# ccalantzis/BRDF

Hardware: AMD Instinct MI355X
Metric: BRDF residual-evals/sec (1 M samples, Ward 3-param), whole job; rel-err vs CPU levmar in `parity` (higher is better)
Workload: dtype f64

## Files before the change

brdf_amd/_lib.py:

```python
from __future__ import annotations

import ctypes as C
import os

_HERE = os.path.dirname(os.path.abspath(__file__))
LIB_PATH = os.environ.get("BRDF_HIP_LIB") or os.path.join(_HERE, "libbrdf_hip.so")

D = C.POINTER(C.c_double)
F = C.POINTER(C.c_float)
I = C.POINTER(C.c_int)
MODEL_FUNC = C.CFUNCTYPE(None, D, D, C.c_int, C.c_int, C.c_void_p)


class ExtraData(C.Structure):
    _fields_ = [("angles", D), ("modelInfo", C.c_int)]


ABI = {
    "dlevmar_dif": (C.c_int, [C.c_void_p, D, D, C.c_int, C.c_int, C.c_int, D, D, D, D, C.c_void_p]),
    "dlevmar_bc_dif": (C.c_int, [C.c_void_p, D, D, C.c_int, C.c_int, D, D, D, C.c_int, D, D, D, D, C.c_void_p]),
    "dlevmar_der": (C.c_int, [C.c_void_p, C.c_void_p, D, D, C.c_int, C.c_int, C.c_int, D, D, D, D, C.c_void_p]),
    "dlevmar_bc_der": (C.c_int, [C.c_void_p, C.c_void_p, D, D, C.c_int, C.c_int, D, D, D, C.c_int, D, D, D, D, C.c_void_p]),
    "dlevmar_stddev": (C.c_double, [D, C.c_int, C.c_int]),
    "dlevmar_corcoef": (C.c_double, [D, C.c_int, C.c_int, C.c_int]),
    "dlevmar_R2": (C.c_double, [C.c_void_p, D, D, C.c_int, C.c_int, C.c_void_p]),
    "dAx_eq_b_LU_noLapack": (C.c_int, [D, D, D, C.c_int]),
    "slevmar_dif": (C.c_int, [C.c_void_p, F, F, C.c_int, C.c_int, C.c_int, F, F, F, F, C.c_void_p]),
    "slevmar_bc_dif": (C.c_int, [C.c_void_p, F, F, C.c_int, C.c_int, F, F, F, C.c_int, F, F, F, F, C.c_void_p]),
    "slevmar_der": (C.c_int, [C.c_void_p, C.c_void_p, F, F, C.c_int, C.c_int, C.c_int, F, F, F, F, C.c_void_p]),
    "slevmar_bc_der": (C.c_int, [C.c_void_p, C.c_void_p, F, F, C.c_int, C.c_int, F, F, F, C.c_int, F, F, F, F, C.c_void_p]),
    "slevmar_chkjac": (None, [C.c_void_p, C.c_void_p, F, C.c_int, C.c_int, C.c_void_p, F]),
    "slevmar_stddev": (C.c_float, [F, C.c_int, C.c_int]),
    "slevmar_corcoef": (C.c_float, [F, C.c_int, C.c_int, C.c_int]),
    "slevmar_R2": (C.c_float, [C.c_void_p, F, F, C.c_int, C.c_int, C.c_void_p]),
    "sAx_eq_b_LU_noLapack": (C.c_int, [F, F, F, C.c_int]),
    "brdf_hip_register_model": (C.c_int, [C.c_void_p]),
    "brdf_hip_unregister_model": (C.c_int, [C.c_void_p]),
    "BRDFFunc_hip": (None, [D, D, C.c_int, C.c_int, C.c_void_p]),
    "BRDFJac_hip": (None, [D, D, C.c_int, C.c_int, C.c_void_p]),
    "dlevmar_chkjac": (None, [C.c_void_p, C.c_void_p, D, C.c_int, C.c_int, C.c_void_p, D]),
    "brdf_hip_fit_dev": (C.c_int, [C.c_int, C.c_int, C.c_void_p, C.c_void_p, C.c_int, D, D, D, D, C.c_int, D, D, D,
                                   C.c_void_p]),
    "brdf_hip_fit_channels_dev": (C.c_int, [C.c_int, C.c_int, C.c_void_p, C.c_void_p, C.c_longlong, C.c_int, C.c_int, D, D, D, D, C.c_int, D,
                                            D, D, C.c_void_p]),
    "brdf_hip_last_channels_stamps": (C.c_int, [C.c_int, C.POINTER(C.c_longlong)]),
    "brdf_hip_last_channels_stats": (C.c_int, [C.c_int, C.POINTER(C.c_int), C.POINTER(C.c_longlong), C.POINTER(C.c_longlong), D]),
    "brdf_hip_fit_batch_dev": (C.c_int, [C.c_int, C.c_int, C.c_void_p, C.c_void_p, C.c_int, C.c_int, C.c_void_p, D, D,
                                         C.c_int, D, C.c_void_p, C.c_void_p, C.c_void_p]),
    "brdf_hip_fit_batch": (C.c_int, [C.c_int, C.c_int, D, D, C.c_int, C.c_int, D, D, D, C.c_int, D, D, I]),
    "brdf_hip_fit_batch_multi": (C.c_int, [C.c_int, C.c_int, D, D, C.c_int, C.c_int, D, D, D, C.c_int, D, D, I, I, C.c_int]),
    "brdf_hip_last_multi_stats": (C.c_int, [C.c_int, I, C.POINTER(C.c_longlong), C.POINTER(C.c_longlong), D]),
    "brdf_hip_fit_stats_batch_dev": (C.c_int, [C.c_int, C.c_int, C.c_void_p, C.c_void_p, C.c_int, C.c_int, C.c_void_p, D, C.c_void_p,
                                               C.c_void_p, C.c_void_p, C.c_void_p]),
    "brdf_hip_fit_stats_batch": (C.c_int, [C.c_int, C.c_int, D, D, C.c_int, C.c_int, D, D, D, D, I]),
    "brdf_hip_model_eval_dev": (C.c_int, [C.c_int, C.c_void_p, C.c_int, D, C.c_void_p, C.c_void_p]),
    "brdf_hip_synth_dev": (C.c_int, [C.c_int, C.c_ulonglong, C.c_longlong, C.c_int, C.c_int, C.c_void_p, C.c_void_p,
                                     C.c_void_p, C.c_void_p]),
    "brdf_hip_cosines_dev": (C.c_int, [C.c_void_p, C.c_void_p, C.c_void_p, C.c_void_p, C.c_longlong, D, C.c_int, D, C.c_int,
                                       C.c_void_p, C.c_void_p]),
    "brdf_hip_led_table": (None, [D]),
    "brdf_hip_fit_capture_dev": (C.c_int, [C.c_int, C.c_void_p, C.c_int, C.c_int, C.c_int, C.c_void_p, C.c_void_p, C.c_void_p,
                                           C.c_void_p, C.c_int, D, D, C.c_int, D, D, D, C.c_int, D, C.c_void_p, D,
                                           C.POINTER(C.c_longlong), C.c_void_p]),
    "brdf_hip_fit_capture_stats_dev": (C.c_int, [C.c_int, C.c_void_p, C.c_int, C.c_int, C.c_int, C.c_void_p, C.c_void_p, C.c_void_p,
                                                 C.c_void_p, C.c_int, D, D, C.c_int, D, D, D, C.c_int, D, C.c_void_p, D,
                                                 C.POINTER(C.c_longlong), C.c_void_p, C.c_void_p, C.c_void_p, C.c_void_p]),
    "brdf_hip_fit_capture_single_dev": (C.c_int, [C.c_int, C.c_void_p, C.c_int, C.c_int, C.c_int, C.c_void_p, C.c_void_p, C.c_void_p,
                                                  C.c_void_p, C.c_int, D, D, C.c_int, D, D, D, C.c_int, D, D, D,
                                                  C.POINTER(C.c_longlong), C.c_void_p]),
    "brdf_hip_device_count": (C.c_int, []),
    "brdf_hip_last_error": (C.c_char_p, []),
    "brdf_hip_last_fit_launches": (C.c_longlong, []),
    "brdf_hip_set_launch_timing": (None, [C.c_int]),
    "brdf_hip_last_fit_kernel_us": (C.c_double, []),
    "brdf_hip_last_channels_kernel_us": (C.c_double, []),
    "brdf_hip_last_fit_stamps": (C.c_int, [C.POINTER(C.c_longlong)]),
    "brdf_hip_last_fit_trace": (C.c_int, [C.POINTER(C.c_longlong), C.c_int]),
    "brdf_hip_last_fit_stats": (C.c_int, [C.POINTER(C.c_longlong), C.POINTER(C.c_longlong), C.POINTER(C.c_longlong),
                                          D]),
}


def load() -> C.CDLL:
    try:
        import torch
    except ImportError:
        pass
    if not os.path.exists(LIB_PATH):
        raise ImportError(
            f"{LIB_PATH} not found: build it with `python -c 'import __graft_entry__ as g; g.build()'` "
            "(or `make -C brdf_amd/csrc`). brdf_amd has no fallback path without its HIP library.")
    lib = C.CDLL(LIB_PATH, mode=C.RTLD_LOCAL)
    for name, (res, args) in ABI.items():
        try:
            fn = getattr(lib, name)
        except AttributeError as exc:
            raise ImportError(f"{LIB_PATH} does not export `{name}` declared in include/brdf_levmar.h") from exc
        fn.restype = res
        fn.argtypes = args
    return lib


lib = load()


def last_error() -> str:
    return (lib.brdf_hip_last_error() or b"").decode()
```

brdf_amd/csrc/capi.hip:

```cpp
#include <algorithm>
#include <cmath>
#include <cstdio>
#include <cstring>
#include <mutex>

#include <cfloat>
#include <vector>

#include "../../include/brdf_levmar.h"
#include "batch_fit.h"
#include "fit_host.h"
#include "fit_stats.h"

namespace brdf {
int generic_fit_run(int method, void (*func)(double *, double *, int, int, void *),
                    void (*jacf)(double *, double *, int, int, void *), double *p, double *x, int m, int n, double *lb,
                    double *ub, double *dscl, int itmax, double *opts, double *info, double *covar, void *adata);
int model_eval_run(int model, const double *d_angles, int n, const double *p, double *d_hx, hipStream_t stream);
int model_jac_run(int model, const double *d_angles, int n, const double *p, double *d_jac, hipStream_t stream);
int chkjac_err_run(const double *fvec, const double *fjac, const double *fvecp, const double *p, int m, int n, double *err);
int r2_run(const double *x, const double *hx, int n, double *r2);
int generic_fit_run_f(int method, void (*func)(float *, float *, int, int, void *), void (*jacf)(float *, float *, int, int, void *),
                      float *p, float *x, int m, int n, float *lb, float *ub, float *dscl, int itmax, float *opts, float *info,
                      float *covar, void *adata);
// ... 382 lines not shown

void BRDFFunc_hip(double *p, double *hx, int m, int n, void *adata) {
  const brdf_extra_data *ed = static_cast<const brdf_extra_data *>(adata);
  if (!p || !hx || !ed || !ed->angles || m != kM || n <= 0) {
    set_error("BRDFFunc_hip(): bad arguments");
    return;
  }
  if (ed->modelInfo < 0 || ed->modelInfo >= MODEL_COUNT) return;
  double *stage = g_stage.get(4 * (size_t)n);
  if (!stage) return;
  double *d_out = stage + 3 * (size_t)n;
  hipError_t e = upload_planes(stage, ed->angles, n, ed->modelInfo);
  if (e != hipSuccess) {
    set_error("BRDFFunc_hip(): host->device copy failed: %s", hipGetErrorString(e));
    return;
  }
  if (model_eval_run(ed->modelInfo, stage, n, p, d_out, nullptr) != 0) return;
  e = hipMemcpy(hx, d_out, sizeof(double) * n, hipMemcpyDeviceToHost);
  if (e != hipSuccess) set_error("BRDFFunc_hip(): device->host copy failed: %s", hipGetErrorString(e));
}

void BRDFJac_hip(double *p, double *jac, int m, int n, void *adata) {
  const brdf_extra_data *ed = static_cast<const brdf_extra_data *>(adata);
  if (!p || !jac || !ed || !ed->angles || m != kM || n <= 0) {
    set_error("BRDFJac_hip(): bad arguments");
    return;
  }
  if (ed->modelInfo < 0 || ed->modelInfo >= MODEL_COUNT) return;
  double *stage = g_stage.get(6 * (size_t)n);
  if (!stage) return;
  double *d_out = stage + 3 * (size_t)n;
  hipError_t e = upload_planes(stage, ed->angles, n, ed->modelInfo);
  if (e != hipSuccess) {
    set_error("BRDFJac_hip(): host->device copy failed: %s", hipGetErrorString(e));
    return;
  }
  if (model_jac_run(ed->modelInfo, stage, n, p, d_out, nullptr) != 0) return;
  e = hipMemcpy(jac, d_out, sizeof(double) * 3 * n, hipMemcpyDeviceToHost);
  if (e != hipSuccess) set_error("BRDFJac_hip(): device->host copy failed: %s", hipGetErrorString(e));
}

void dlevmar_chkjac(void (*func)(double *, double *, int, int, void *), void (*jacf)(double *, double *, int, int, void *),
                    double *p, int m, int n, void *adata, double *err) {
  if (!func || !jacf || !p || !err || m <= 0 || n <= 0) {
    set_error("dlevmar_chkjac(): bad arguments");
    return;
  }
  std::vector<double> fvec(n), fjac((size_t)n * m), pp(m), fvecp(n);
  const double eps = sqrt(DBL_EPSILON);
  (*func)(p, fvec.data(), m, n, adata);
  (*jacf)(p, fjac.data(), m, n, adata);
  for (int j = 0; j < m; ++j) {
    double temp = eps * fabs(p[j]);
    if (temp == 0.0) temp = eps;
    pp[j] = p[j] + temp;
  }
  (*func)(pp.data(), fvecp.data(), m, n, adata);
  (void)chkjac_err_run(fvec.data(), fjac.data(), fvecp.data(), p, m, n, err);
}

int brdf_hip_fit_dev(int method, int model, const double *d_angles, const double *d_x, int n, double *p,
                     const double *lb, const double *ub, const double *dscl, int itmax, const double *opts,
                     double *info, double *covar, void *stream) {
  StreamFitArgs a;
  a.method = (method == BRDF_METHOD_BC_DER) ? 1 : (method == BRDF_METHOD_DER ? 2 : method);
  a.analytic = (method == BRDF_METHOD_BC_DER || method == BRDF_METHOD_DER) ? 1 : 0;
  a.model = model;
  a.d_angles = d_angles;
  a.d_x = d_x;
  a.n = n;
  a.p = p;
  a.lb = lb;
  a.ub = ub;
  a.dscl = dscl;
  a.itmax = itmax;
  a.opts = opts;
  a.info = info;
  a.covar = covar;
  a.stream = static_cast<hipStream_t>(stream);
  return stream_fit_run(a);
}

int brdf_hip_fit_channels_dev(int method, int model, const double *d_angles, const double *d_x, long long x_stride, int n, int channels,
                              double *p, const double *lb, const double *ub, const double *dscl, int itmax, const double *opts,
                              double *info, double *covar, void *stream) {
  if (!d_angles || !d_x || !p || n <= 0 || channels < 1 || channels > 16 || (channels > 1 && x_stride < n)) {
    set_error("brdf_hip_fit_channels_dev(): bad arguments");
    return LM_ERROR;
  }
  if (method < 0 || method > 3 || model < 0 || model >= MODEL_COUNT) {
    set_error("brdf_hip_fit_channels_dev(): unknown method %d or model %d", method, model);
    return LM_ERROR;
  }
  return channels_fit_run(method, model, d_angles, d_x, x_stride, n, channels, p, lb, ub, dscl, itmax, opts, info, covar,
                          static_cast<hipStream_t>(stream));
}

int brdf_hip_last_channels_stamps(int channel, long long *out8) {
  const FitStats st = channels_last_stats(channel);
  for (int i = 0; i < 8; ++i) out8[i] = st.stamps[i];
  return 0;
}

int brdf_hip_last_channels_stats(int channel, int *shared_launch, long long *passes, long long *jac_passes, double *device_us) {
  const FitStats st = channels_last_stats(channel);
  if (shared_launch) *shared_launch = channels_last_shared();
  if (passes) *passes = st.passes;
  if (jac_passes) *jac_passes = st.jac_passes;
  if (device_us) *device_us = st.device_us;
  return 0;
}

int brdf_hip_fit_batch_dev(int method, int model, const double *d_angles, const double *d_x, int S, int n,
                           double *d_p, const double *lb, const double *ub, int itmax, const double *opts,
                           double *d_info, int *d_ret, void *stream) {
  BatchFitArgs a;
  a.method = method;
  a.model = model;
  a.d_angles = d_angles;
  a.d_x = d_x;
  a.S = S;
  a.n = n;
  a.d_p = d_p;
  a.lb = lb;
  a.ub = ub;
  a.itmax = itmax;
  a.opts = opts;
  a.d_info = d_info;
  a.d_ret = d_ret;
  a.stream = static_cast<hipStream_t>(stream);
  return batch_fit_enqueue(a);
}

int brdf_hip_fit_batch(int method, int model, const double *angles, const double *x, int S, int n, double *p,
                       const double *lb, const double *ub, int itmax, const double *opts, double *info, int *ret) {
  if (!angles || !x || !p || S <= 0 || n <= 0) {
    set_error("brdf_hip_fit_batch(): bad arguments");
    return LM_ERROR;
  }
  const size_t sn = (size_t)S * n;
  DevBuf d_angles, d_x, d_p, d_info, d_ret;
  if (d_angles.alloc(3 * sn) || d_x.alloc(sn) || d_p.alloc(3 * (size_t)S) || d_info.alloc(10 * (size_t)S) ||
      d_ret.alloc(((size_t)S + 1) / 2 + 1))
    return LM_ERROR;
  hipError_t e = hipMemcpy(d_angles.ptr, angles, sizeof(double) * 3 * sn, hipMemcpyHostToDevice);
  if (e == hipSuccess) e = hipMemcpy(d_x.ptr, x, sizeof(double) * sn, hipMemcpyHostToDevice);
  if (e == hipSuccess) e = hipMemcpy(d_p.ptr, p, sizeof(double) * 3 * S, hipMemcpyHostToDevice);
  if (e != hipSuccess) {
    set_error("brdf_hip_fit_batch(): host->device copy failed: %s", hipGetErrorString(e));
    return LM_ERROR;
  }
  int *d_ret_i = reinterpret_cast<int *>(d_ret.ptr);
  if (brdf_hip_fit_batch_dev(method, model, d_angles.ptr, d_x.ptr, S, n, d_p.ptr, lb, ub, itmax, opts, d_info.ptr,
                             d_ret_i, nullptr) != 0)
    return LM_ERROR;
  e = hipDeviceSynchronize();
  if (e == hipSuccess) e = hipMemcpy(p, d_p.ptr, sizeof(double) * 3 * S, hipMemcpyDeviceToHost);
  if (e == hipSuccess && info) e = hipMemcpy(info, d_info.ptr, sizeof(double) * 10 * S, hipMemcpyDeviceToHost);
  int *host_ret = ret;
  int *tmp = nullptr;
  if (!host_ret) host_ret = tmp = new int[S];
  if (e == hipSuccess) e = hipMemcpy(host_ret, d_ret_i, sizeof(int) * S, hipMemcpyDeviceToHost);
  int bad = 0;
  if (e == hipSuccess)
    for (int s = 0; s < S; ++s) bad += host_ret[s] < 0;
  delete[] tmp;
  if (e != hipSuccess) {
    set_error("brdf_hip_fit_batch(): %s", hipGetErrorString(e));
    return LM_ERROR;
  }
  return bad;
}

int brdf_hip_fit_stats_batch_dev(int method, int model, const double *d_angles, const double *d_x, int S, int n,
                                 const double *d_p, const double *opts, double *d_covar, double *d_stats, int *d_rank,
                                 void *stream) {
  FitStatsArgs a;
  a.method = method;
  a.model = model;
  a.d_angles = d_angles;
  a.d_x = d_x;
  a.S = S;
  a.n = n;
  a.d_p = d_p;
  a.opts = opts;
  a.d_covar = d_covar;
  a.d_stats = d_stats;
  a.d_rank = d_rank;
  a.stream = static_cast<hipStream_t>(stream);
  return fit_stats_enqueue(a, "brdf_hip_fit_stats_batch_dev");
}

int brdf_hip_fit_stats_batch(int method, int model, const double *angles, const double *x, int S, int n, const double *p,
                             const double *opts, double *covar, double *stats, int *rank) {
  static const char *who = "brdf_hip_fit_stats_batch";
  FitStatsArgs a;
  a.method = method;
  a.model = model;
  a.d_angles = angles;
  a.d_x = x;
  a.S = S;
  a.n = n;
  a.d_p = p;
  a.opts = opts;
  a.d_covar = covar;
  a.d_stats = stats;
  a.d_rank = rank;
  if (fit_stats_check(a, who) != 0) return LM_ERROR;
  const size_t sn = (size_t)S * n;
  DevBuf d_angles, d_x, d_p, d_covar, d_stats, d_rank;
  if (d_angles.alloc(3 * sn) || d_x.alloc(sn) || d_p.alloc(3 * (size_t)S) || (covar && d_covar.alloc(9 * (size_t)S)) ||
      (stats && d_stats.alloc(BRDF_STATS_SZ * (size_t)S)) || (rank && d_rank.alloc(((size_t)S + 1) / 2 + 1)))
    return LM_ERROR;
  hipError_t e = hipMemcpy(d_angles.ptr, angles, sizeof(double) * 3 * sn, hipMemcpyHostToDevice);
  if (e == hipSuccess) e = hipMemcpy(d_x.ptr, x, sizeof(double) * sn, hipMemcpyHostToDevice);
  if (e == hipSuccess) e = hipMemcpy(d_p.ptr, p, sizeof(double) * 3 * S, hipMemcpyHostToDevice);
  if (e != hipSuccess) {
    set_error("%s(): host->device copy failed: %s", who, hipGetErrorString(e));
    return LM_ERROR;
  }
  a.d_angles = d_angles.ptr;
  a.d_x = d_x.ptr;
  a.d_p = d_p.ptr;
  a.d_covar = d_covar.ptr;
  a.d_stats = d_stats.ptr;
  a.d_rank = reinterpret_cast<int *>(d_rank.ptr);
  if (fit_stats_enqueue(a, who) != 0) return LM_ERROR;
  e = hipStreamSynchronize(nullptr);
  if (e == hipSuccess && covar) e = hipMemcpy(covar, d_covar.ptr, sizeof(double) * 9 * S, hipMemcpyDeviceToHost);
  if (e == hipSuccess && stats) e = hipMemcpy(stats, d_stats.ptr, sizeof(double) * BRDF_STATS_SZ * S, hipMemcpyDeviceToHost);
  if (e == hipSuccess && rank) e = hipMemcpy(rank, d_rank.ptr, sizeof(int) * S, hipMemcpyDeviceToHost);
  if (e != hipSuccess) {
    set_error("%s(): %s", who, hipGetErrorString(e));
    return LM_ERROR;
  }
  return 0;
}

int brdf_hip_model_eval_dev(int model, const double *d_angles, int n, const double *p, double *d_hx, void *stream) {
  return model_eval_run(model, d_angles, n, p, d_hx, static_cast<hipStream_t>(stream));
}

int brdf_hip_synth_dev(int model, unsigned long long seed, long long first, int count, int n,
                       const double *d_truth, double *d_angles, double *d_x, void *stream) {
  return synth_enqueue(model, seed, first, count, n, d_truth, d_angles, d_x, static_cast<hipStream_t>(stream));
}

int brdf_hip_cosines_dev(const double *d_vertices, const int *d_faces, const double *d_face_normals, const int *d_surfels,
                         long long S, const double *leds, int L, const double *view_origin, int rv_mode, double *d_angles,
                         void *stream) {
  return cosines_run(d_vertices, d_faces, d_face_normals, d_surfels, S, leds, L, view_origin, rv_mode, d_angles,
                     static_cast<hipStream_t>(stream));
}

void brdf_hip_led_table(double *leds16x3) { led_table(leds16x3); }

int brdf_hip_fit_capture_dev(int model, const unsigned char *d_images, int L, int H, int W, const int *d_pixel_map,
                             const double *d_vertices, const int *d_faces, const double *d_face_normals, int nf,
                             const double *leds, const double *view_origin, int rv_mode, const double *p0, const double *lb,
                             const double *ub, int itmax, const double *opts, double *d_brdf_surfaces, double *avg,
                             long long *n_pixels, void *stream) {
  return capture_fit_run(model, d_images, L, H, W, d_pixel_map, d_vertices, d_faces, d_face_normals, nf, leds, view_origin,
                         rv_mode, p0, lb, ub, itmax, opts, d_brdf_surfaces, avg, n_pixels, static_cast<hipStream_t>(stream));
}

int brdf_hip_fit_capture_stats_dev(int model, const unsigned char *d_images, int L, int H, int W, const int *d_pixel_map,
                                   const double *d_vertices, const int *d_faces, const double *d_face_normals, int nf,
                                   const double *leds, const double *view_origin, int rv_mode, const double *p0,
                                   const double *lb, const double *ub, int itmax, const double *opts, double *d_brdf_surfaces,
                                   double *avg, long long *n_pixels, void *stream, double *d_surface_covar,
                                   double *d_surface_stats, int *d_surface_rank) {
  return capture_fit_run(model, d_images, L, H, W, d_pixel_map, d_vertices, d_faces, d_face_normals, nf, leds, view_origin,
                         rv_mode, p0, lb, ub, itmax, opts, d_brdf_surfaces, avg, n_pixels, static_cast<hipStream_t>(stream),
                         d_surface_covar, d_surface_stats, d_surface_rank);
}

int brdf_hip_fit_capture_single_dev(int model, const unsigned char *d_images, int L, int H, int W, const int *d_pixel_map,
                                    const double *d_vertices, const int *d_faces, const double *d_face_normals, int nf,
                                    const double *leds, const double *view_origin, int rv_mode, const double *p0,
                                    const double *lb, const double *ub, int itmax, const double *opts, double *single_brdf,
                                    double *info, long long *n_faces_used, void *stream) {
  return capture_fit_single_run(model, d_images, L, H, W, d_pixel_map, d_vertices, d_faces, d_face_normals, nf, leds, view_origin,
                                rv_mode, p0, lb, ub, itmax, opts, single_brdf, info, n_faces_used, static_cast<hipStream_t>(stream));
}

int brdf_hip_device_count(void) {
  int c = 0;
  if (hipGetDeviceCount(&c) != hipSuccess) return 0;
  return c;
}

const char *brdf_hip_last_error(void) { return get_error(); }

int brdf_hip_last_fit_stats(long long *passes, long long *jac_passes, long long *eval_passes, double *device_us) {
  const FitStats s = stream_fit_last_stats();
  if (passes) *passes = s.passes;
  if (jac_passes) *jac_passes = s.jac_passes;
  if (eval_passes) *eval_passes = s.eval_passes;
  if (device_us) *device_us = s.device_us;
  return 0;
}

long long brdf_hip_last_fit_launches(void) { return stream_fit_last_stats().launches; }

void brdf_hip_set_launch_timing(int on) { set_launch_timing(on != 0); }
double brdf_hip_last_fit_kernel_us(void) { return stream_fit_last_stats().kernel_us; }
double brdf_hip_last_channels_kernel_us(void) { return channels_last_shared() ? channels_last_stats(0).kernel_us : -1.0; }

int brdf_hip_last_fit_trace(long long *out, int max_rows) { return resident_fit_last_trace(out, max_rows); }

int brdf_hip_last_fit_stamps(long long *out8) {
  const FitStats s = stream_fit_last_stats();
  for (int k = 0; k < 8; ++k) out8[k] = s.stamps[k];
  return 0;
}

}
```

brdf_amd/csrc/fit_host.hip:

```cpp
#include <algorithm>
#include <cstdio>
#include <cstdlib>

#include "fit_host.h"

namespace brdf {

void set_bad_input_error(const char *who, int bad_input, int n, int m) {
  switch (bad_input) {
  case 1: set_error("%s(): cannot solve a problem with fewer measurements [%d] than unknowns [%d]", who, n, m); break;
  case 2: set_error("%s(): at least one lower bound exceeds the upper one", who); break;
  default: set_error("%s(): scaling constants should be positive", who); break;
  }
}

void warn_start_projected(int i, double from, double to) {
  fprintf(stderr, "Warning: component %d of starting point not feasible in dlevmar_bc_dif()! [%g projected to %g]\n", i, from, to);
}

int start_fit_machine(MachineUnion &m, int method, const double *p, int n, const double *lb, const double *ub, const double *dscl, int itmax,
                      const double *opts, bool want_covar, bool analytic, bool fast) {
  if (method == 0) {
    m.dif.start(p, n, itmax, opts, want_covar, 1, dif_chain_candidates());
    if (m.dif.h.req.kind != RQ_DONE) return 0;
    set_bad_input_error("dlevmar_dif", 1, n, kM);
    return kLmError;
  }
  if (method == 2) {
    m.der.start(p, n, itmax, opts, want_covar);
    if (m.der.h.req.kind != RQ_DONE) return 0;
    set_bad_input_error("dlevmar_der", 1, n, kM);
    return kLmError;
  }
  BcMachine<kM> &bc = m.bc;
  bc.start(p, n, lb, ub, dscl, itmax, opts, want_covar, pg_candidates(), bc_spec_jac_enabled() ? 1 : 0);
  bc.c.analytic_jac = analytic ? 1 : 0;
  if (bc.h.req.kind == RQ_DONE) {
    set_bad_input_error("dlevmar_bc_dif", bc.c.bad_input, n, kM);
    return kLmError;
  }
  if (fast || !brdf_fast_path_enabled())
    for (int i = 0; i < kM; ++i)
      if (bc.c.infeasible_mask & (1 << i)) warn_start_projected(i, bc.c.p_start[i], bc.h.p[i]);
  return 0;
}

void mailbox_to_caller(const Mailbox &mb, double *p, double *info, double *covar, FitStats *stats) {
  for (int i = 0; i < kM; ++i) p[i] = mb.p[i];
  if (info)
    for (int i = 0; i < kInfoSz; ++i) info[i] = mb.info[i];
  if (covar)
    for (int i = 0; i < kM * kM; ++i) covar[i] = mb.covar[i];
  stats->passes = mb.passes;
  stats->jac_passes = mb.n_jac;
  stats->eval_passes = mb.n_eval;
  stats->device_us = (double)(mb.t_last - mb.t_first) / 100.0;
  for (int k = 0; k < 8; ++k) stats->stamps[k] = mb.stamps[k];
}

ExchangeKnobs exchange_knobs(int max_replicas, long long default_spin_ticks) {
  ExchangeKnobs k{max_replicas, default_spin_ticks, -1};
  if (const char *e = getenv("BRDF_HIP_RESIDENT_REPLICAS")) k.replicas = std::min(max_replicas, std::max(1, atoi(e)));
  if (const char *e = getenv("BRDF_HIP_RESIDENT_SPIN_MS")) k.spin_ticks = std::max(1LL, atoll(e)) * 100000LL;
  if (const char *e = getenv("BRDF_HIP_RESIDENT_SABOTAGE")) k.sabotage_epoch = atoi(e);
  return k;
}

bool kernel_fits_a_cu(const void *kernel, int threads, std::atomic<int> &cached) {
  int v = cached.load(std::memory_order_relaxed);
  if (v == 0) {
    int per_cu = 0;
    if (hipOccupancyMaxActiveBlocksPerMultiprocessor(&per_cu, kernel, threads, 0) != hipSuccess) per_cu = 0;
    v = per_cu + 1;
    cached.store(v, std::memory_order_relaxed);
  }
  return v > 1;
}

void ResidentWorkspace::release() {
  if (d_block || h_mbox) {
    int cur = -1;
    (void)hipGetDevice(&cur);
    if (device >= 0 && cur != device) (void)hipSetDevice(device);
    (void)hipDeviceSynchronize();
    if (d_block) (void)hipFree(d_block);
    if (h_mbox) (void)hipHostFree(h_mbox);
    if (cur >= 0 && cur != device) (void)hipSetDevice(cur);
  }
  d_block = nullptr;
  h_mbox = d_mbox = nullptr;
  device = -1;
}

int ResidentWorkspace::allocate(size_t bytes, int mailboxes) {
  hipDeviceProp_t prop;
  HIP_OK(hipGetDeviceProperties(&prop, device));
  cus = prop.multiProcessorCount;
  HIP_OK(hipMalloc(&d_block, bytes));
  HIP_OK(hipMemset(d_block, 0, bytes));
  HIP_OK(hipHostMalloc(&h_mbox, sizeof(Mailbox) * (size_t)mailboxes, hipHostMallocMapped | hipHostMallocCoherent));
  HIP_OK(hipHostGetDevicePointer((void **)&d_mbox, h_mbox, 0));
  block_bytes = bytes;
  n_mbox = mailboxes;
  return 0;
}

int ResidentWorkspace::ensure(int dev, size_t bytes, int mailboxes) {
  if (ready(dev)) return 0;
  release();
  device = dev;
  const int r = allocate(bytes, mailboxes);
  if (r != 0) release();
  return r;
}

int ResidentWorkspace::zero_tables(hipStream_t stream) {
  HIP_OK(hipMemsetAsync(d_block, 0, block_bytes, stream));
  return 0;
}

void ResidentWorkspace::launch_unavailable() {
  backoff = std::min(1024, std::max(8, backoff * 2));
  skip = backoff;
  if (const char *e = getenv("BRDF_HIP_RESIDENT_BACKOFF")) skip = std::max(0, atoi(e));
}

int ResidentWorkspace::wait_for_mailboxes(int K, hipStream_t stream, bool *done) {
  auto all_done = [&] {
    for (int k = 0; k < K; ++k)
      if (!*(volatile int *)&h_mbox[k].done) return false;
    return true;
  };
  for (unsigned spins = 0; !all_done(); ++spins)
    if ((spins & 0x3FFu) == 0x3FFu && hipStreamQuery(stream) != hipErrorNotReady) break;
  __atomic_thread_fence(__ATOMIC_ACQUIRE);
  if (!all_done()) {
    HIP_OK(hipStreamSynchronize(stream));
    __atomic_thread_fence(__ATOMIC_ACQUIRE);
  }
  *done = all_done();
  return 0;
}

}
```

brdf_amd/csrc/lm_machine.h:

```cpp
#pragma once

#include <float.h>
#include <math.h>

#if defined(__HIPCC__)
#define LM_HD __host__ __device__ __forceinline__
#else
#define LM_HD inline
#endif

namespace brdf {

constexpr double kEpsilon = 1E-12;
constexpr double kOneThird = 0.3333333334;
constexpr int kLsItMax = 150;
constexpr double kLsPow = 2.1;
constexpr double kInitMu = 1E-03;
#ifndef LM_STAMP
#define LM_STAMP(i) do {} while (0)
#endif

#ifndef LM_PHASE_ENTER
#define LM_PHASE_ENTER(X) true
#endif
#define LM_PHASE(X) if ((ONE_LANE ? lm_uniform(ph) : ph) == X && LM_PHASE_ENTER(X)) do
#define LM_PHASE_END while (0);
#define LM_GATE(X)                                    \
  if (GATED && !heavy && ph == X) {                   \
    req.kind = RQ_YIELD;                              \
    { h.phase = ph; return; }                         \
  }

constexpr double kStopThresh = 1E-17;
constexpr double kDiffDelta = 1E-06;
constexpr int kInfoSz = 10;
constexpr int kLmError = -1;

enum ReqKind : int {
  RQ_DONE = 0,
  RQ_EVAL = 1,
  RQ_SCALED = 2,
  RQ_JAC = 3,
  RQ_DIF_INIT = 4,
  RQ_DIF_JAC = 5,
  RQ_DIF_TRIAL = 6,
  RQ_DIF_UPDATE = 7,
  RQ_EVAL_MULTI = 8,
  RQ_YIELD = 9
};

constexpr int kMaxCand = 8;

template <class Real>
struct LmLimits;
template <>
struct LmLimits<double> {
  static LM_HD double eps() { return DBL_EPSILON; }
  static LM_HD double max() { return DBL_MAX; }
};
template <>
struct LmLimits<float> {
  static LM_HD float eps() { return FLT_EPSILON; }
  static LM_HD float max() { return FLT_MAX; }
};

template <int M, class Real = double>
struct Request {
  int kind;
  int central;
  int sel_hx;
  int sel_j;
  int aux;
  Real p[M];
  Real d[M];
  Real q[M];
  Real dp[M];
  Real dp_l2;
  Real scal;
  int nk;
  int pad_;
  Real pk[kMaxCand][M];
};

template <int M>
struct SumLayout {
  static constexpr int NL = M * (M + 1) / 2;
  static constexpr int JAC = NL + M + 1;
  static constexpr int DIF_JAC = NL + M;
  static constexpr int DIF_TRIAL = 1 + NL + 2 * M;
  static constexpr int MAX = DIF_TRIAL > JAC ? DIF_TRIAL : JAC;
};

LM_HD int lm_uniform(int v) {
#if defined(__HIP_DEVICE_COMPILE__)
  return __builtin_amdgcn_readfirstlane(v);
#else
  return v;
#endif
}

#if defined(__HIP_DEVICE_COMPILE__)
__device__ __forceinline__ double lm_read_lane(double v, int lane) {
  const int lo = __builtin_amdgcn_readlane(__double2loint(v), lane);
  const int hi = __builtin_amdgcn_readlane(__double2hiint(v), lane);
  return __hiloint2double(hi, lo);
}
__device__ __forceinline__ float lm_read_lane(float v, int lane) {
  return __int_as_float(__builtin_amdgcn_readlane(__float_as_int(v), lane));
}
#endif

template <class Real>
LM_HD Real lm_abs(Real v) { return (v >= Real(0.0)) ? v : -v; }
template <class Real>
LM_HD bool lm_finite(Real v) { return (v - v) == Real(0.0); }

template <int M, class Real>
LM_HD int lu_solve(const Real *A, const Real *B, Real *x) {
  constexpr int kUnrollLu = M <= 8 ? 64 : 1;
  Real a[M * M], scale[M];
  int perm[M];
#pragma unroll kUnrollLu
  for (int i = 0; i < M * M; ++i) a[i] = A[i];
#pragma unroll kUnrollLu
  for (int i = 0; i < M; ++i) x[i] = B[i];
#pragma unroll kUnrollLu
  for (int i = 0; i < M; ++i) {
    Real big = Real(0.0);
#pragma unroll kUnrollLu
    for (int j = 0; j < M; ++j) {
      const Real t = lm_abs(a[i * M + j]);
      if (t > big) big = t;
    }
    if (big == Real(0.0)) return 0;
    scale[i] = Real(1.0) / big;
  }
#pragma unroll kUnrollLu
  for (int j = 0; j < M; ++j) {
    int pivot = j;
    Real big = Real(0.0);
#pragma unroll kUnrollLu
    for (int i = 0; i < j; ++i) {
      Real s = a[i * M + j];
#pragma unroll kUnrollLu
      for (int k = 0; k < i; ++k) s -= a[i * M + k] * a[k * M + j];
      a[i * M + j] = s;
    }
#pragma unroll kUnrollLu
    for (int i = j; i < M; ++i) {
      Real s = a[i * M + j];
#pragma unroll kUnrollLu
      for (int k = 0; k < j; ++k) s -= a[i * M + k] * a[k * M + j];
      a[i * M + j] = s;
      const Real t = scale[i] * lm_abs(s);
      if (t >= big) {
        big = t;
        pivot = i;
      }
    }
#pragma unroll kUnrollLu
    for (int r = j + 1; r < M; ++r) {
      if (pivot == r) {
#pragma unroll kUnrollLu
        for (int k = 0; k < M; ++k) {
          const Real t = a[r * M + k];
          a[r * M + k] = a[j * M + k];
          a[j * M + k] = t;
        }
        scale[r] = scale[j];
      }
    }
    perm[j] = pivot;
    if (a[j * M + j] == Real(0.0)) a[j * M + j] = LmLimits<Real>::eps();
    if (j != M - 1) {
      const Real t = Real(1.0) / a[j * M + j];
#pragma unroll kUnrollLu
      for (int i = j + 1; i < M; ++i) a[i * M + j] *= t;
    }
  }
  int first = 0;
#pragma unroll kUnrollLu
  for (int i = 0; i < M; ++i) {
    Real s = x[i];
#pragma unroll kUnrollLu
    for (int r = i + 1; r < M; ++r) {
      if (perm[i] == r) {
        s = x[r];
        x[r] = x[i];
      }
    }
    if (first != 0) {
#pragma unroll kUnrollLu
      for (int jj = 0; jj < i; ++jj)
        if (jj >= first - 1) s -= a[i * M + jj] * x[jj];
    } else if (s != Real(0.0)) {
      first = i + 1;
    }
    x[i] = s;
  }
#pragma unroll kUnrollLu
  for (int i = M - 1; i >= 0; --i) {
    Real s = x[i];
#pragma unroll kUnrollLu
    for (int j = i + 1; j < M; ++j) s -= a[i * M + j] * x[j];
    x[i] = s / a[i * M + i];
  }
  return 1;
}

template <int M, class Real>
LM_HD int lu_covar(const Real *JtJ, Real *C, Real sumsq, int n) {
  for (int l = 0; l < M; ++l) {
    Real rhs[M], col[M];
    for (int i = 0; i < M; ++i) rhs[i] = (i == l) ? Real(1.0) : Real(0.0);
    if (!lu_solve<M>(JtJ, rhs, col)) return 0;
    for (int i = 0; i < M; ++i) C[i * M + l] = col[i];
  }
  const Real fact = sumsq / (Real)(n - M);
  for (int i = 0; i < M * M; ++i) C[i] *= fact;
  return M;
}

template <int M, class Real>
LM_HD void fd_steps(const Real *p, Real delta, Real *d) {
  for (int j = 0; j < M; ++j) {
    Real s = Real(1E-04) * p[j];
    s = lm_abs(s);
    if (s < delta) s = delta;
    d[j] = s;
  }
}

template <int M, class Real>
LM_HD void unpack_lower(const Real *s, Real *jtj) {
  int c = 0;
  for (int i = 0; i < M; ++i)
    for (int j = 0; j <= i; ++j, ++c) {
      jtj[i * M + j] = s[c];
      jtj[j * M + i] = s[c];
    }
}

template <class Real = double>
struct FitOptionsT {
  Real tau, eps1, eps2, eps2sq, eps3, delta;
  int forward;
};

template <class Real>
LM_HD FitOptionsT<Real> make_options(const Real *opts) {
  FitOptionsT<Real> o;
  if (opts) {
    o.tau = opts[0];
    o.eps1 = opts[1];
    o.eps2 = opts[2];
    o.eps2sq = opts[2] * opts[2];
    o.eps3 = opts[3];
    o.delta = opts[4];
  } else {
    o.tau = Real(kInitMu);
    o.eps1 = Real(kStopThresh);
    o.eps2 = Real(kStopThresh);
    o.eps2sq = Real(kStopThresh) * Real(kStopThresh);
    o.eps3 = Real(kStopThresh);
    o.delta = Real(kDiffDelta);
  }
  o.forward = 1;
  if (o.delta < Real(0.0)) {
    o.delta = -o.delta;
    o.forward = 0;
  }
  return o;
}

template <int M, class Real = double>
struct DifMachine {
  enum Phase : int { D_INIT_EVAL = 1, D_ITER_TOP, D_AFTER_JAC, D_GRADIENT, D_SOLVE, D_AFTER_TRIAL, D_AFTER_UPDATE, D_DECIDE, D_REJECT, D_AFTER_MULTI, D_FINISH, D_DONE };
  struct Cold {
    FitOptionsT<Real> o;
    int itmax, n, want_covar, refresh;
    int speculative;
    int multi;
    Real info[kInfoSz], covar[M * M];
    int ret;
  };
  struct CoreInts {
    int phase, k, stop, nu, nfev, njap, nlss, updjac, updp, newjac;
    int sel_hx, sel_j, accepted;
    int chain, single, mcnt;
  };
  struct CoreReals {
    Real p[M], mu, p_e2, jte_inf, p_l2, dp_l2, pdp_e2;
    Real jtj[M * M], jte[M], dp[M];
  };
  struct Core : CoreInts, CoreReals {};
  struct Cool {
    Real init_e2, diag[M], pdp[M];
    Real spec_jtj[M * M], spec_jte[M];
    Real ml2[kMaxCand];
  };
  struct Hot : Core {
    Cool cool;
    Request<M, Real> req;
  };
  static LM_HD void uniform_ints(CoreInts &h) {
    h.phase = lm_uniform(h.phase);
    h.k = lm_uniform(h.k);
    h.stop = lm_uniform(h.stop);
    h.nu = lm_uniform(h.nu);
    h.nfev = lm_uniform(h.nfev);
    h.njap = lm_uniform(h.njap);
    h.nlss = lm_uniform(h.nlss);
    h.updjac = lm_uniform(h.updjac);
    h.updp = lm_uniform(h.updp);
    h.newjac = lm_uniform(h.newjac);
    h.sel_hx = lm_uniform(h.sel_hx);
    h.sel_j = lm_uniform(h.sel_j);
    h.accepted = lm_uniform(h.accepted);
    h.chain = lm_uniform(h.chain);
    h.single = lm_uniform(h.single);
    h.mcnt = lm_uniform(h.mcnt);
  }
  Cold c;
  Hot h;

  LM_HD void start(const Real *p0, int n_, int itmax_, const Real *opts, int want_covar_, int speculative_ = 1, int multi_ = 1) {
    Request<M, Real> &req = h.req;
    Cool &cool = h.cool;
    c.o = make_options(opts);
    c.speculative = speculative_;
    c.multi = (multi_ < 1 || !speculative_) ? 1 : ((multi_ > kMaxCand) ? kMaxCand : multi_);
    h.chain = h.single = h.mcnt = 0;
    for (int j = 0; j < kMaxCand; ++j) cool.ml2[j] = Real(0.0);
    h.accepted = 0;
    c.itmax = itmax_;
    c.n = n_;
    c.want_covar = want_covar_;
    h.k = 0;
    h.stop = 0;
    h.nfev = h.njap = h.nlss = 0;
    h.updjac = 0;
    h.updp = 1;
    h.newjac = 0;
    c.refresh = (M >= 10) ? M : 10;
    h.sel_hx = h.sel_j = 0;
    h.mu = h.jte_inf = h.p_l2 = Real(0.0);
    h.p_e2 = cool.init_e2 = h.pdp_e2 = Real(0.0);
    h.dp_l2 = LmLimits<Real>::max();
    c.ret = kLmError;
    for (int i = 0; i < M; ++i) {
      h.p[i] = p0[i];
      h.jte[i] = cool.diag[i] = h.dp[i] = cool.pdp[i] = Real(0.0);
      cool.spec_jte[i] = Real(0.0);
    }
    for (int i = 0; i < M * M; ++i) h.jtj[i] = cool.spec_jtj[i] = c.covar[i] = Real(0.0);
    for (int i = 0; i < kInfoSz; ++i) c.info[i] = Real(0.0);
    clear_req(h, req);
    if (c.n < M) {
      h.phase = D_DONE;
      req.kind = RQ_DONE;
      return;
    }
    req.kind = RQ_DIF_INIT;
    for (int i = 0; i < M; ++i) req.p[i] = h.p[i];
    h.phase = D_INIT_EVAL;
  }

  static LM_HD void clear_req(const CoreInts &h, Request<M, Real> &req) {
    req.kind = RQ_DONE;
    req.central = 0;
    req.sel_hx = h.sel_hx;
    req.sel_j = h.sel_j;
    req.aux = 0;
    req.dp_l2 = Real(0.0);
    req.scal = Real(1.0);
    req.nk = 0;
    for (int i = 0; i < M; ++i) req.p[i] = req.d[i] = req.q[i] = req.dp[i] = Real(0.0);
  }

  static LM_HD void gradient_stats(CoreReals &h, Cool &cool) {
    h.p_l2 = h.jte_inf = Real(0.0);
    for (int i = 0; i < M; ++i) {
      const Real t = lm_abs(h.jte[i]);
      if (h.jte_inf < t) h.jte_inf = t;
      cool.diag[i] = h.jtj[i * M + i];
      h.p_l2 += h.p[i] * h.p[i];
    }
  }

  template <bool ONE_LANE = false, bool MULTI = false>
  LM_HD void step(const Real *s, Real maxabs) { run<ONE_LANE, MULTI>(c, h, h.cool, h.req, s, maxabs); }

  template <bool ONE_LANE, bool MULTI = false>
  static LM_HD void run(Cold &c, Core &h, Cool &cool, Request<M, Real> &req, const Real *s, Real maxabs) {
    run<ONE_LANE, MULTI>(c, static_cast<CoreInts &>(h), static_cast<CoreReals &>(h), cool, req, s, maxabs);
  }
  template <bool ONE_LANE, bool MULTI = false>
  static LM_HD void run(Cold &c, CoreInts &hi, CoreReals &h, Cool &cool, Request<M, Real> &req, const Real *s, Real ) {
    int ph = ONE_LANE ? lm_uniform(hi.phase) : hi.phase;
    LM_STAMP(0);
    for (;;) {
      if (ONE_LANE) ph = lm_uniform(ph);
      if (ph <= 0 || ph >= D_DONE) {
        req.kind = RQ_DONE;
        { hi.phase = ph; return; }
      }
      LM_PHASE(D_INIT_EVAL) {
        hi.nfev = 1;
        h.p_e2 = s[0];
        cool.init_e2 = h.p_e2;
        if (!lm_finite(h.p_e2)) hi.stop = 7;
        hi.nu = 20;
        ph = D_ITER_TOP;
        break;
      } LM_PHASE_END

      LM_PHASE(D_AFTER_JAC) {
        unpack_lower<M>(s, h.jtj);
        for (int i = 0; i < M; ++i) h.jte[i] = s[SumLayout<M>::NL + i];
        hi.newjac = 0;
        gradient_stats(h, cool);
        ph = D_SOLVE;
        break;
      } LM_PHASE_END

      LM_PHASE(D_AFTER_TRIAL) {
        h.pdp_e2 = s[0];
        if (!lm_finite(h.pdp_e2)) {
          hi.stop = 7;
          ph = D_FINISH;
          break;
        }
        const Real dF = h.p_e2 - h.pdp_e2;
        const bool updated = (hi.updp || dF > 0);
        if (MULTI) hi.chain = updated ? 0 : hi.chain + 1;
        Real dL = Real(0.0);
        for (int i = 0; i < M; ++i) dL += h.dp[i] * (h.mu * h.dp[i] + h.jte[i]);
        hi.accepted = (dL > Real(0.0) && dF > Real(0.0)) ? 1 : 0;
        if (hi.accepted) {
          Real t = (Real(2.0) * dF / dL - Real(1.0));
          t = Real(1.0) - t * t * t;
          h.mu = h.mu * ((t >= Real(kOneThird)) ? t : Real(kOneThird));
        }
        if (updated) {
          ++hi.updjac;
          hi.newjac = 1;
          if (c.speculative) {
            hi.sel_j ^= 1;
            unpack_lower<M>(s + 1, cool.spec_jtj);
            const Real *g = s + 1 + SumLayout<M>::NL + (hi.accepted ? 0 : M);
            for (int i = 0; i < M; ++i) cool.spec_jte[i] = g[i];
          } else {
            clear_req(hi, req);
            req.kind = RQ_DIF_UPDATE;
            req.aux = hi.accepted;
            for (int i = 0; i < M; ++i) {
              req.p[i] = h.p[i];
              req.q[i] = cool.pdp[i];
              req.dp[i] = h.dp[i];
            }
            req.dp_l2 = h.dp_l2;
            ph = D_AFTER_UPDATE;
            { hi.phase = ph; return; }
          }
        }
        LM_STAMP(1);
        ph = D_DECIDE;
        break;
      } LM_PHASE_END

      LM_PHASE(D_AFTER_UPDATE) {
        unpack_lower<M>(s, cool.spec_jtj);
        for (int i = 0; i < M; ++i) cool.spec_jte[i] = s[SumLayout<M>::NL + i];
        ph = D_DECIDE;
        break;
      } LM_PHASE_END

      if constexpr (MULTI)
      LM_PHASE(D_AFTER_MULTI) {
        const int cnt = hi.mcnt;
        int next = D_ITER_TOP;
        for (int j = 0; j < kMaxCand; ++j) {
          if (j >= cnt || !(hi.k < c.itmax)) break;
          const Real e2 = s[j];
          if (lm_finite(e2) && h.p_e2 - e2 > Real(0.0)) {
            hi.single = 1;
            break;
          }
          ++hi.nlss;
          ++hi.nfev;
          h.pdp_e2 = e2;
          h.dp_l2 = cool.ml2[j];
          if (!lm_finite(e2)) {
            hi.stop = 7;
            next = D_FINISH;
            break;
          }
          ++hi.chain;
          h.mu *= hi.nu;
          const int nu2 = (int)((unsigned)hi.nu << 1);
          if (nu2 <= hi.nu) {
            hi.stop = 5;
            next = D_FINISH;
            break;
          }
          hi.nu = nu2;
          ++hi.k;
        }
        ph = next;
        break;
      } LM_PHASE_END

      LM_PHASE(D_DECIDE) {
        if (hi.accepted) {
          hi.nu = 2;
          for (int i = 0; i < M; ++i) h.p[i] = cool.pdp[i];
          if (c.speculative) hi.sel_hx ^= 1;
          h.p_e2 = h.pdp_e2;
          hi.updp = 1;
          ++hi.k;
          ph = D_ITER_TOP;
          break;
        }
        ph = D_REJECT;
        break;
      } LM_PHASE_END

      LM_PHASE(D_REJECT) {
        h.mu *= hi.nu;
        const int nu2 = (int)((unsigned)hi.nu << 1);
        if (nu2 <= hi.nu) {
          hi.stop = 5;
          ph = D_FINISH;
          break;
        }
        hi.nu = nu2;
        for (int i = 0; i < M; ++i) h.jtj[i * M + i] = cool.diag[i];
        ++hi.k;
        ph = D_ITER_TOP;
        break;
      } LM_PHASE_END

      LM_PHASE(D_ITER_TOP) {
        if (!(hi.k < c.itmax && !hi.stop)) {
          ph = D_FINISH;
          break;
        }
        if (h.p_e2 <= c.o.eps3) {
          hi.stop = 6;
          ph = D_FINISH;
          break;
        }
        if ((hi.updp && hi.nu > 16) || hi.updjac == c.refresh) {
          clear_req(hi, req);
          req.kind = RQ_DIF_JAC;
          req.central = !c.o.forward;
          for (int i = 0; i < M; ++i) req.p[i] = h.p[i];
          fd_steps<M>(h.p, c.o.delta, req.d);
          ++hi.njap;
          hi.nfev += c.o.forward ? M : 2 * M;
          hi.nu = 2;
          hi.updjac = 0;
          hi.updp = 0;
          hi.newjac = 1;
          if (MULTI) hi.chain = 0;
          ph = D_AFTER_JAC;
          { hi.phase = ph; return; }
        }
        ph = D_GRADIENT;
        break;
      } LM_PHASE_END

      LM_PHASE(D_GRADIENT) {
        LM_STAMP(5);
        if (hi.newjac) {
          hi.newjac = 0;
          for (int i = 0; i < M * M; ++i) h.jtj[i] = cool.spec_jtj[i];
          for (int i = 0; i < M; ++i) h.jte[i] = cool.spec_jte[i];
          gradient_stats(h, cool);
        }
        ph = D_SOLVE;
        break;
      } LM_PHASE_END

      LM_PHASE(D_SOLVE) {
        LM_STAMP(2);
        if (h.jte_inf <= c.o.eps1) {
          h.dp_l2 = Real(0.0);
          hi.stop = 1;
          ph = D_FINISH;
          break;
        }
        if (hi.k == 0) {
          Real t = -LmLimits<Real>::max();
          for (int i = 0; i < M; ++i)
            if (cool.diag[i] > t) t = cool.diag[i];
          h.mu = c.o.tau * t;
        }
        if (MULTI && c.multi > 1 && hi.updp == 0 && hi.chain >= 1 && !hi.single) {
          Real A[M * M], b[M], pc[M];
          for (int i = 0; i < M * M; ++i) A[i] = h.jtj[i];
          for (int i = 0; i < M; ++i) {
            b[i] = h.jte[i];
            pc[i] = h.p[i];
          }
          Real mu = h.mu;
          int nu = hi.nu, kk = hi.k, cnt = 0;
          const Real pl2 = h.p_l2;
#if defined(__HIP_DEVICE_COMPILE__)
          if (ONE_LANE) {
            const int myj = (int)(__lane_id() & (kMaxCand - 1));
            Real my_mu = mu;
            int limit = 0;
            for (int j = 0; j < kMaxCand; ++j) {
              if (j >= c.multi || !(kk < c.itmax)) break;
              if (j == myj) my_mu = mu;
              limit = j + 1;
              mu *= nu;
              const int nu2 = (int)((unsigned)nu << 1);
              if (nu2 <= nu) break;
              nu = nu2;
              ++kk;
            }
            Real dpj[M], q[M], l2 = Real(0.0);
            for (int i = 0; i < M; ++i) A[i * M + i] = cool.diag[i] + my_mu;
            bool ok = lu_solve<M>(A, b, dpj) != 0;
            for (int i = 0; i < M; ++i) {
              q[i] = pc[i] + dpj[i];
              l2 += dpj[i] * dpj[i];
            }
            ok = ok && !(l2 <= c.o.eps2sq * pl2 || l2 >= (pl2 + c.o.eps2) / (Real(kEpsilon) * Real(kEpsilon)));
            const unsigned good = (unsigned)__builtin_amdgcn_ballot_w64(ok) & 0xFFu;
            for (int j = 0; j < kMaxCand; ++j) {
              if (j >= limit || !(good >> j & 1u)) break;
              for (int i = 0; i < M; ++i) req.pk[j][i] = lm_read_lane(q[i], j);
              cool.ml2[j] = lm_read_lane(l2, j);
              ++cnt;
            }
          } else
#endif
          for (int j = 0; j < kMaxCand; ++j) {
            if (j >= c.multi || !(kk < c.itmax)) break;
            Real dpj[M];
            for (int i = 0; i < M; ++i) A[i * M + i] = cool.diag[i] + mu;
            if (!lu_solve<M>(A, b, dpj)) break;
            Real l2 = Real(0.0);
            for (int i = 0; i < M; ++i) {
              req.pk[j][i] = pc[i] + dpj[i];
              l2 += dpj[i] * dpj[i];
            }
            if (l2 <= c.o.eps2sq * pl2 || l2 >= (pl2 + c.o.eps2) / (Real(kEpsilon) * Real(kEpsilon))) break;
            cool.ml2[j] = l2;
            ++cnt;
            mu *= nu;
            const int nu2 = (int)((unsigned)nu << 1);
            if (nu2 <= nu) break;
            nu = nu2;
            ++kk;
          }
          if (cnt >= 2) {
            hi.mcnt = cnt;
            req.kind = RQ_EVAL_MULTI;
            req.nk = cnt;
            req.scal = Real(1.0);
            ph = D_AFTER_MULTI;
            { hi.phase = ph; return; }
          }
        }
        if (MULTI) hi.single = 0;
        for (int i = 0; i < M; ++i) h.jtj[i * M + i] += h.mu;
        const int solved = lu_solve<M>(h.jtj, h.jte, h.dp);
        LM_STAMP(3);
        ++hi.nlss;
        if (!solved) {
          ph = D_REJECT;
          break;
        }
        h.dp_l2 = Real(0.0);
        for (int i = 0; i < M; ++i) {
          const Real t = h.dp[i];
          cool.pdp[i] = h.p[i] + t;
          h.dp_l2 += t * t;
        }
        if (h.dp_l2 <= c.o.eps2sq * h.p_l2) {
          hi.stop = 2;
          ph = D_FINISH;
          break;
        }
        if (h.dp_l2 >= (h.p_l2 + c.o.eps2) / (Real(kEpsilon) * Real(kEpsilon))) {
          hi.stop = 4;
          ph = D_FINISH;
          break;
        }
        clear_req(hi, req);
        req.kind = RQ_DIF_TRIAL;
        for (int i = 0; i < M; ++i) {
          req.p[i] = h.p[i];
          req.q[i] = cool.pdp[i];
          req.dp[i] = h.dp[i];
        }
        req.dp_l2 = h.dp_l2;
        ++hi.nfev;
        ph = D_AFTER_TRIAL;
        LM_STAMP(4);
        { hi.phase = ph; return; }
      } LM_PHASE_END

      LM_PHASE(D_FINISH) {
        if (hi.k >= c.itmax) hi.stop = 3;
        for (int i = 0; i < M; ++i) h.jtj[i * M + i] = cool.diag[i];
        c.info[0] = cool.init_e2;
        c.info[1] = h.p_e2;
        c.info[2] = h.jte_inf;
        c.info[3] = h.dp_l2;
        Real t = -LmLimits<Real>::max();
        for (int i = 0; i < M; ++i)
          if (t < h.jtj[i * M + i]) t = h.jtj[i * M + i];
        c.info[4] = h.mu / t;
        c.info[5] = (Real)hi.k;
        c.info[6] = (Real)hi.stop;
        c.info[7] = (Real)hi.nfev;
        c.info[8] = (Real)hi.njap;
        c.info[9] = (Real)hi.nlss;
        if (c.want_covar) lu_covar<M>(h.jtj, c.covar, h.p_e2, c.n);
        c.ret = (hi.stop != 4 && hi.stop != 7) ? hi.k : kLmError;
        clear_req(hi, req);
        ph = D_DONE;
        { hi.phase = ph; return; }
      } LM_PHASE_END
    }
  }
};

template <int M, class Real = double>
struct BcMachine {
  enum Phase : int {
    B_INIT_EVAL = 1, B_ITER_TOP, B_AFTER_JAC, B_SOLVE, B_AFTER_LM_EVAL, B_AFTER_LM_NORM, B_LM_JUDGE, B_LS_PROLOGUE,
    B_LS_ISSUE, B_LS_EVAL, B_PG_BEGIN, B_PG_ISSUE, B_PG_EVAL, B_PG_NORM, B_PG_JUDGE, B_PG_MULTI, B_COMMIT,
    B_END_ITER, B_FINISH, B_DONE
  };
  struct Cold {
    FitOptionsT<Real> o;
    int itmax, n, want_covar;
    int has_lb, has_ub, has_dscl;
    Real lb[M], ub[M], dscl[M];
    int infeasible_mask, bad_input;
    int bad_config;
    int analytic_jac;
    int multi;
    int spec_jac;
    Real p_start[M];
    Real info[kInfoSz], covar[M * M];
    int ret;
  };
  struct Core {
    int phase, k, stop, nu, nfev, njev, nlss, gprev;
    int spec_state;
    Real p[M], mu, p_e2, jte_inf, p_l2, dp_l2, pdp_e2;
    Real jtj[M * M], jte[M], dp[M], pdp[M];
    Real t, gdp;
    int ls_first, ls_left;
    int pg_n, pg_single;
  };
  struct Cool {
    Real init_e2, keep_max, diag[M], t0;
    Real sj[SumLayout<M>::JAC];
    Real ls_f0, ls_lambda, ls_plmbda, ls_pfpls, ls_tlmbda, ls_rmnlmb, ls_slp;
  };
  struct Hot : Core {
    Cool cool;
    Request<M, Real> req;
  };
  static LM_HD void uniform_ints(Core &h) {
    h.phase = lm_uniform(h.phase);
    h.k = lm_uniform(h.k);
    h.stop = lm_uniform(h.stop);
    h.nu = lm_uniform(h.nu);
    h.nfev = lm_uniform(h.nfev);
    h.njev = lm_uniform(h.njev);
    h.nlss = lm_uniform(h.nlss);
    h.gprev = lm_uniform(h.gprev);
    h.spec_state = lm_uniform(h.spec_state);
    h.ls_first = lm_uniform(h.ls_first);
    h.ls_left = lm_uniform(h.ls_left);
    h.pg_n = lm_uniform(h.pg_n);
    h.pg_single = lm_uniform(h.pg_single);
  }
  Cold c;
  Hot h;

  LM_HD static Real median3(Real a, Real b, Real c) {
    return (a >= b) ? ((c >= a) ? a : ((c <= b) ? b : c)) : ((c >= b) ? b : ((c <= a) ? a : c));
  }
  static LM_HD void project(const Cold &c, Real *v) {
    const int has_lb = c.has_lb, has_ub = c.has_ub;
    if (!has_lb && !has_ub) return;
    Real lo[M], hi[M];
    for (int i = 0; i < M; ++i) {
      lo[i] = c.lb[i];
      hi[i] = c.ub[i];
    }
    for (int i = M; i-- > 0;) {
      if (has_lb && has_ub)
        v[i] = median3(lo[i], v[i], hi[i]);
      else if (has_ub) {
        if (v[i] > hi[i]) v[i] = hi[i];
      } else {
        if (v[i] < lo[i]) v[i] = lo[i];
      }
    }
  }
  static LM_HD void clear_req(const Core &h, Request<M, Real> &req) {
    req.kind = RQ_DONE;
    req.central = 0;
    req.sel_hx = req.sel_j = req.aux = 0;
    req.dp_l2 = Real(0.0);
    req.scal = Real(1.0);
    for (int i = 0; i < M; ++i) req.p[i] = req.d[i] = req.q[i] = req.dp[i] = Real(0.0);
  }
  static LM_HD void request_eval(const Cold &c, Core &h, Request<M, Real> &req, const Real *v, int kind = RQ_EVAL) {
    req.kind = kind;
    req.scal = Real(1.0);
    if (c.has_dscl) {
      for (int i = 0; i < M; ++i) req.p[i] = v[i] * c.dscl[i];
    } else {
      for (int i = 0; i < M; ++i) req.p[i] = v[i];
    }
    ++h.nfev;
  }
  static LM_HD void request_eval_jac(const Cold &c, Core &h, Request<M, Real> &req, const Real *v) {
    req.kind = RQ_JAC;
    req.scal = Real(1.0);
    req.central = !c.o.forward;
    for (int i = 0; i < M; ++i) req.p[i] = v[i];
    fd_steps<M>(req.p, c.o.delta, req.d);
    ++h.nfev;
    h.spec_state = 1;
  }

  LM_HD void configure(int n_, const Real *lb_, const Real *ub_, const Real *dscl_, int itmax_, const Real *opts,
                       int want_covar_, int multi_ = 1, int spec_jac_ = 0) {
    c.multi = (multi_ < 1) ? 1 : ((multi_ > kMaxCand) ? kMaxCand : multi_);
    c.o = make_options(opts);
    if (opts) {
      c.o.forward = (opts[4] >= Real(0.0));
      c.o.delta = lm_abs(opts[4]);
    }
    c.itmax = itmax_;
    c.n = n_;
    c.want_covar = want_covar_;
    c.has_lb = lb_ != nullptr;
    c.has_ub = ub_ != nullptr;
    c.has_dscl = dscl_ != nullptr;
    c.analytic_jac = 0;
    c.spec_jac = (spec_jac_ && !c.has_dscl) ? 1 : 0;
    for (int i = 0; i < M; ++i) {
      c.lb[i] = c.has_lb ? lb_[i] : -LmLimits<Real>::max();
      c.ub[i] = c.has_ub ? ub_[i] : LmLimits<Real>::max();
      c.dscl[i] = c.has_dscl ? dscl_[i] : Real(1.0);
    }
    c.bad_config = 0;
    if (c.n < M) {
      c.bad_config = 1;
      return;
    }
    if (c.has_lb && c.has_ub)
      for (int i = 0; i < M; ++i)
        if (c.lb[i] > c.ub[i]) {
          c.bad_config = 2;
          return;
        }
    if (c.has_dscl)
      for (int i = M; i-- > 0;)
        if (c.dscl[i] <= Real(0.0)) {
          c.bad_config = 3;
          return;
        }
  }
  LM_HD void begin(const Real *p0) {
    Request<M, Real> &req = h.req;
    Cool &cool = h.cool;
    h.pg_n = h.pg_single = 0;
    h.spec_state = 0;
    h.k = 0;
    h.stop = 0;
    h.nu = 2;
    h.nfev = h.njev = h.nlss = 0;
    h.gprev = 0;
    c.infeasible_mask = 0;
    c.bad_input = c.bad_config;
    h.mu = h.jte_inf = h.p_l2 = h.t = cool.t0 = h.gdp = Real(0.0);
    h.p_e2 = cool.init_e2 = h.pdp_e2 = cool.keep_max = Real(0.0);
    h.dp_l2 = LmLimits<Real>::max();
    cool.ls_f0 = cool.ls_lambda = cool.ls_plmbda = cool.ls_pfpls = cool.ls_tlmbda = cool.ls_rmnlmb = cool.ls_slp = Real(0.0);
    h.ls_first = 1;
    h.ls_left = 0;
    c.ret = kLmError;
    for (int i = 0; i < M; ++i) {
      h.p[i] = p0[i];
      h.jte[i] = cool.diag[i] = h.dp[i] = h.pdp[i] = Real(0.0);
    }
    for (int i = 0; i < M * M; ++i) h.jtj[i] = c.covar[i] = Real(0.0);
    for (int i = 0; i < SumLayout<M>::JAC; ++i) cool.sj[i] = Real(0.0);
    for (int i = 0; i < kInfoSz; ++i) c.info[i] = Real(0.0);
    clear_req(h, req);
    h.phase = B_DONE;
    if (c.bad_input) return;
    for (int i = 0; i < M; ++i) c.p_start[i] = h.p[i];
    project(c, h.p);
    for (int i = 0; i < M; ++i)
      if (c.p_start[i] != h.p[i]) c.infeasible_mask |= (1 << i);
    clear_req(h, req);
    req.kind = RQ_EVAL;
    for (int i = 0; i < M; ++i) req.p[i] = h.p[i];
    if (c.spec_jac) {
      request_eval_jac(c, h, req, h.p);
      h.nfev = 0;
    }
    h.phase = B_INIT_EVAL;
  }
  LM_HD void start(const Real *p0, int n_, const Real *lb_, const Real *ub_, const Real *dscl_,
                   int itmax_, const Real *opts, int want_covar_, int multi_ = 1, int spec_jac_ = 0) {
    configure(n_, lb_, ub_, dscl_, itmax_, opts, want_covar_, multi_, spec_jac_);
    begin(p0);
  }

  template <bool SPECJ = false>
  static LM_HD void accept_trial(Core &h) {
    for (int i = 0; i < M; ++i) h.p[i] = h.pdp[i];
    h.p_e2 = h.pdp_e2;
    if (SPECJ) h.spec_state = (h.spec_state == 1) ? 2 : 0;
  }
  template <bool SPECJ>
  static LM_HD Real candidate_e2(Core &h, Cool &cool, const Real *s) {
    if (SPECJ && h.spec_state == 1) {
      for (int i = 0; i < SumLayout<M>::JAC; ++i) cool.sj[i] = s[i];
      return s[SumLayout<M>::JAC - 1];
    }
    return s[0];
  }

  template <bool ONE_LANE = false, bool MULTI = true, bool GATED = false, bool SPECJ = false>
  LM_HD void step(const Real *s, Real maxabs, bool heavy = true) { run<ONE_LANE, MULTI, GATED, SPECJ>(c, h, h.cool, h.req, s, maxabs, heavy); }

  template <bool ONE_LANE, bool MULTI, bool GATED, bool SPECJ = false>
  static LM_HD void run(Cold &c, Core &h, Cool &cool, Request<M, Real> &req, const Real *s, Real maxabs, bool heavy) {
    constexpr Real alpha = Real(1e-4), beta = Real(0.9), gamma = Real(0.99995), rho = Real(1e-8), tming = Real(1e-18), tini = Real(1.0);
    int ph = ONE_LANE ? lm_uniform(h.phase) : h.phase;
    for (;;) {
      (void)LM_PHASE_ENTER(29);
      if (ONE_LANE) ph = lm_uniform(ph);
      if (ph <= 0 || ph >= B_DONE) {
        req.kind = RQ_DONE;
        { h.phase = ph; return; }
      }
      LM_PHASE(B_INIT_EVAL) {
        h.nfev = 1;
        h.p_e2 = candidate_e2<SPECJ>(h, cool, s);
        if (SPECJ && h.spec_state == 1) h.spec_state = 2;
        cool.init_e2 = h.p_e2;
        if (!lm_finite(h.p_e2)) h.stop = 7;
        if (c.has_dscl)
          for (int i = M; i-- > 0;) {
            h.p[i] /= c.dscl[i];
            if (c.has_ub && c.ub[i] != LmLimits<Real>::max()) c.ub[i] = c.ub[i] / c.dscl[i];
            if (c.has_lb && c.lb[i] != -LmLimits<Real>::max()) c.lb[i] = c.lb[i] / c.dscl[i];
          }
        ph = B_ITER_TOP;
        break;
      } LM_PHASE_END

      LM_GATE(B_AFTER_JAC)
      if (!GATED || heavy)
      LM_PHASE(B_AFTER_JAC) {
        const Real *sv = s;
        if (SPECJ && h.spec_state == 3) sv = cool.sj;
        if (SPECJ) h.spec_state = 0;
        unpack_lower<M>(sv, h.jtj);
        for (int i = 0; i < M; ++i) h.jte[i] = sv[SumLayout<M>::NL + i];
        if (c.has_dscl) {
          for (int i = 0; i < M; ++i) {
            h.jte[i] *= c.dscl[i];
            for (int j = 0; j < M; ++j) h.jtj[i * M + j] *= c.dscl[i] * c.dscl[j];
          }
        }
        int nactive = 0, satisfied = 0;
        h.p_l2 = h.jte_inf = Real(0.0);
        for (int i = 0; i < M; ++i) {
          if (c.has_ub && h.p[i] == c.ub[i]) {
            ++nactive;
            if (h.jte[i] > Real(0.0)) ++satisfied;
          } else if (c.has_lb && h.p[i] == c.lb[i]) {
            ++nactive;
            if (h.jte[i] < Real(0.0)) ++satisfied;
          } else {
            const Real a = lm_abs(h.jte[i]);
            if (h.jte_inf < a) h.jte_inf = a;
// ... 750 lines not shown
```

brdf_amd/csrc/resident_fit.hip:

```cpp
#include <algorithm>
#include <atomic>
#include <cstdio>
#include <cstdlib>
#include <cstring>

#include "resident_fit_impl.h"
#include "fit_host.h"

namespace brdf {

#ifndef BRDF_DEV_WARD_ONLY
ResidentKernels resident_kernels_00(), resident_kernels_01(), resident_kernels_02();
ResidentKernels resident_kernels_10(), resident_kernels_11(), resident_kernels_12();
#endif
ResidentKernels resident_kernels_20(), resident_kernels_21(), resident_kernels_22();

namespace {

ResidentKernels (*const kKernels[MODEL_COUNT][3])() = {
#ifndef BRDF_DEV_WARD_ONLY
    {resident_kernels_00, resident_kernels_01, resident_kernels_02},
    {resident_kernels_10, resident_kernels_11, resident_kernels_12},
#else
    {nullptr, nullptr, nullptr},
    {nullptr, nullptr, nullptr},
#endif
    {resident_kernels_20, resident_kernels_21, resident_kernels_22},
};
std::atomic<int> g_fits_a_cu[MODEL_COUNT][3][2];

struct RWorkspace : ResidentWorkspace {
  static constexpr size_t kMachineBytes = 4096;
  static constexpr size_t off_rows = sizeof(ResidentCtl) + kMachineBytes;
  static constexpr size_t rows_bytes = sizeof(u64) * (kRowsGranules + kGroupsGranules);
  static constexpr size_t trace_bytes = sizeof(long long) * 8 * kRowStride;
  long long h_trace[8 * (kRowStride + 1)] = {0};
  unsigned tag_base = 0;
  FitStats stats{};
  int ensure(int dev) {
    if (ready(dev)) return 0;
    tag_base = 0;
    return ResidentWorkspace::ensure(dev, off_rows + rows_bytes + trace_bytes, 1);
  }
};
thread_local RWorkspace g_rws;

int resident_attempt(const ResidentKernels &k, bool fast, const StreamFitArgs &a, RWorkspace &ws, bool *retry_exact, bool *unavailable) {
  *retry_exact = *unavailable = false;
  const int G = (int)std::min<long long>(ws.cus, std::max<long long>(1, ((long long)a.n + 1023) / 1024));
  MachineUnion scratch;
  if (start_fit_machine(scratch, a.method, a.p, a.n, a.lb, a.ub, a.dscl, a.itmax, a.opts, a.covar != nullptr, a.analytic != 0, fast) != 0)
    return kLmError;
  ws.clear_mailboxes();
  if (ws.tag_base > 0xF0000000u) {
    if (ws.zero_tables(a.stream) != 0) return kLmError;
    ws.tag_base = 0;
  }

  ResidentCtx c;
  c.c0 = a.d_angles;
  c.c1 = a.d_angles + a.n;
  c.c2 = a.d_angles + 2 * (size_t)a.n;
  c.x = a.d_x;
  c.ctl = reinterpret_cast<ResidentCtl *>(ws.d_block);
  c.rows = reinterpret_cast<u64 *>(ws.d_block + RWorkspace::off_rows);
  c.groups = c.rows + kRowsGranules;
  c.launch_id = ws.tag_base + 1u;
  for (int i = 0; i < kM; ++i) {
    c.p0[i] = a.p[i];
    c.lb[i] = a.lb ? a.lb[i] : 0.0;
    c.ub[i] = a.ub ? a.ub[i] : 0.0;
    c.dscl[i] = a.dscl ? a.dscl[i] : 1.0;
  }
  for (int i = 0; i < 5; ++i) c.opts[i] = a.opts ? a.opts[i] : 0.0;
  c.itmax = a.itmax;
  c.has_opts = a.opts != nullptr;
  c.has_lb = a.method == 1 && a.lb != nullptr;
  c.has_ub = a.method == 1 && a.ub != nullptr;
  c.has_dscl = a.method == 1 && a.dscl != nullptr;
  c.want_covar = a.covar != nullptr;
  c.multi = pg_candidates();
  c.chain = dif_chain_candidates();
  c.spec_jac = bc_spec_jac_enabled() ? 1 : 0;
  c.analytic = a.analytic ? 1 : 0;
  c.mbox = ws.d_mbox;
  c.n = a.n;
  c.tag_base = ws.tag_base;
  const ExchangeKnobs knobs = exchange_knobs(kReplicas, kSpinBudgetTicks);
  c.spin_ticks = knobs.spin_ticks;
  c.sabotage_epoch = knobs.sabotage_epoch;
  c.replicas = knobs.replicas;
  c.trace = nullptr;
  c.trace_epoch = -1;
#ifdef BRDF_STAMPS
  c.trace = reinterpret_cast<long long *>(ws.d_block + RWorkspace::off_rows + RWorkspace::rows_bytes);
  c.trace_epoch = 20;
  if (const char *e = getenv("BRDF_HIP_RESIDENT_TRACE_EPOCH")) c.trace_epoch = atoi(e);
#endif

  const ResidentKernelFn kernel = k.single[fast ? kFastPath : kExactPath];
  if (!kernel_fits_a_cu((const void *)kernel, kRThreads, g_fits_a_cu[a.model][a.method][fast ? kFastPath : kExactPath])) {
    *unavailable = true;
    return 0;
  }
  ws.timer.before(a.stream);
  hipLaunchKernelGGL(kernel, dim3(G), dim3(kRThreads), 0, a.stream, c, BatchCtx{});
  HIP_OK(hipGetLastError());
  ws.timer.after(a.stream);
  bool done = false;
  if (ws.wait_for_mailboxes(1, a.stream, &done) != 0) return kLmError;
  if (!done) {
    (void)ws.zero_tables(a.stream);
    ws.tag_base = 0;
    *unavailable = true;
    return 0;
  }
  const Mailbox &mb = *ws.h_mbox;
  ws.tag_base += (unsigned)mb.passes + 2u;
#ifdef BRDF_STAMPS
  (void)hipMemcpy(ws.h_trace, c.trace, RWorkspace::trace_bytes, hipMemcpyDeviceToHost);
  k.take_lm_stamps(ws.h_trace + 8 * kRowStride);
#endif
  if (fast && mb.domain_bad) {
    *retry_exact = true;
    return 0;
  }
  mailbox_to_caller(mb, a.p, a.info, a.covar, &ws.stats);
  ws.stats.launches = 1;
  ws.stats.kernel_us = ws.timer.elapsed_us();
  return mb.ret;
}

int resident_run(const ResidentKernels &k, const StreamFitArgs &a, RWorkspace &ws, bool *unavailable) {
  bool retry = false;
  double keep[kM];
  for (int i = 0; i < kM; ++i) keep[i] = a.p[i];
  if (brdf_fast_path_enabled() || !k.single[kExactPath]) {
    const int ret = resident_attempt(k, true, a, ws, &retry, unavailable);
    if (!retry || *unavailable) return ret;
    for (int i = 0; i < kM; ++i) a.p[i] = keep[i];
  }
  return k.single[kExactPath] ? resident_attempt(k, false, a, ws, &retry, unavailable) : kLmError;
}

}

FitStats resident_fit_last_stats() { return g_rws.stats; }
int resident_fit_last_trace(long long *out, int max_rows) {
  const int rows = std::min(max_rows, kRowStride + 1);
  memcpy(out, g_rws.h_trace, sizeof(long long) * 8 * (size_t)rows);
  return rows;
}

int resident_batch_enqueue(int model, int method, bool fast, const BatchCtx &c, hipStream_t stream) {
  if (!kKernels[model][method]) {
    set_error("resident kernels of model %d / method %d are not in this build", model, method);
    return kLmError;
  }
  const ResidentKernels k = kKernels[model][method]();
  const dim3 grid(c.S), block(kRThreads);
  const ResidentCtx none{};
  if (fast) {
    hipLaunchKernelGGL(k.batched[kFastPath], grid, block, 0, stream, none, c);
    HIP_OK(hipGetLastError());
  }
  if (k.batched[kExactPath]) {
    hipLaunchKernelGGL(k.batched[kExactPath], grid, block, 0, stream, none, c);
    HIP_OK(hipGetLastError());
  }
  return 0;
}

bool resident_fit_try(const StreamFitArgs &a, int *ret) {
  const char *e = getenv("BRDF_HIP_RESIDENT");
  if (e && e[0] == '0') return false;
  int dev = 0;
  if (!kKernels[a.model][a.method] || hipGetDevice(&dev) != hipSuccess) return false;
  RWorkspace &ws = g_rws;
  if (ws.ensure(dev) != 0) return false;
  if ((long long)a.n > (long long)ws.cus * kRTile || ws.cus > kRowStride) return false;
  if (ws.step_aside()) return false;
  bool unavailable = false;
  const int r = resident_run(kKernels[a.model][a.method](), a, ws, &unavailable);
  if (unavailable) {
    static std::atomic<bool> warned{false};
    if (!warned.exchange(true))
      fprintf(stderr, "libbrdf_hip: resident single-launch path unavailable (grid not co-resident?); using the launch chain\n");
    ws.launch_unavailable();
    return false;
  }
  ws.launch_succeeded();
  *ret = r;
  return true;
}

}
```

brdf_amd/csrc/resident_fit_impl.h:

```cpp
#pragma once
#include <type_traits>

#if defined(BRDF_STAMPS)
#include <hip/hip_runtime.h>
static __device__ long long g_rlm_stamps[8];
static __device__ long long g_rlm_last;
#endif
#if defined(BRDF_STAMPS) && defined(__HIP_DEVICE_COMPILE__)
#define LM_STAMP(i) do { if (blockIdx.x == 0) { const long long now_ = clock64(); if ((i) != 0) g_rlm_stamps[i] += now_ - g_rlm_last; g_rlm_last = now_; } } while (0)
#endif
#include "batch_fit.h"
#include "stream_fit.h"

namespace brdf {

constexpr int kRThreads = 512;
constexpr int kRSpt = 8;
constexpr int kRTile = kRThreads * kRSpt;
constexpr int kRCap = kRTile;
constexpr int kRowWords = 2 * kSlots;
constexpr int kRowStride = 256;
constexpr int kRedCols = kRThreads / 4;
constexpr long long kSpinBudgetTicks = 200000000LL;

typedef unsigned long long u64;

struct ResidentCtl {
  unsigned abort;
  unsigned domain_bad;
  unsigned pad[30];
};

struct ResidentCtx {
  const double *c0, *c1, *c2, *x;
  u64 *rows;
  u64 *groups;
  ResidentCtl *ctl;
  unsigned launch_id;
  double p0[kM], opts[5], lb[kM], ub[kM], dscl[kM];
  int itmax, has_opts, has_lb, has_ub, has_dscl, want_covar, multi, analytic;
  int chain;
  int spec_jac;
  Mailbox *mbox;
  int n;
  unsigned tag_base;
  long long spin_ticks;
  int sabotage_epoch;
  int replicas;
  long long *trace;
  int trace_epoch;
};

template <int METHOD>
using RMachine = typename std::conditional<METHOD == 0, DifMachine<kM>, typename std::conditional<METHOD == 1, BcMachine<kM>, DerMachine<kM>>::type>::type;

__device__ __forceinline__ double read_lane(double v, int lane) {
  const int lo = __builtin_amdgcn_readlane(__double2loint(v), lane);
  const int hi = __builtin_amdgcn_readlane(__double2hiint(v), lane);
  return __hiloint2double(hi, lo);
}

__device__ __forceinline__ void acc_normal_eq_fma(const double *j, double e, double *jtj6, double *jte3) {
  jtj6[0] = fma(j[0], j[0], jtj6[0]);
  jtj6[1] = fma(j[0], j[1], jtj6[1]);
  jtj6[2] = fma(j[1], j[1], jtj6[2]);
  jtj6[3] = fma(j[0], j[2], jtj6[3]);
  jtj6[4] = fma(j[1], j[2], jtj6[4]);
  jtj6[5] = fma(j[2], j[2], jtj6[5]);
  jte3[0] = fma(j[0], e, jte3[0]);
  jte3[1] = fma(j[1], e, jte3[1]);
  jte3[2] = fma(j[2], e, jte3[2]);
}
__device__ __forceinline__ double div_by(double x, double d, double r) {
  const double q = x * r;
  return fma(fma(-q, d, x), r, q);
}

#ifdef BRDF_STAMPS
#define RSTAMP(i) do { const long long now_ = clock64(); st_[i] += now_ - last_; last_ = now_; } while (0)
#define RTRACE(ctx_, epoch_, slot_, val_) do { if ((ctx_).trace && (int)(epoch_) == (ctx_).trace_epoch && (threadIdx.x & 63) == 0) (ctx_).trace[blockIdx.x * 8 + (slot_)] = (long long)(val_); } while (0)
#else
#define RSTAMP(i) do {} while (0)
#define RTRACE(ctx_, epoch_, slot_, val_) do {} while (0)
#endif

constexpr int kFc0 = 0, kFx = 1, kFq1 = 2, kFq2 = 3, kFhx = 4, kFwrk = 5, kFtb = 6;
template <int METHOD>
constexpr int sample_fields() { return METHOD == 0 ? 7 : 4; }

template <int METHOD>
struct RegSamples {
  static constexpr bool kUnrolled = true;
  double v[sample_fields<METHOD>()][kRSpt];
  __device__ __forceinline__ double get(int f, int k) const { return v[f][k]; }
  __device__ __forceinline__ void set(int f, int k, double x) { v[f][k] = x; }
};
template <int METHOD>
struct LdsSamples {
  static constexpr bool kUnrolled = false;
  double *base;
  __device__ __forceinline__ double get(int f, int k) const { return base[(f * kRSpt + k) * kWave]; }
  __device__ __forceinline__ void set(int f, int k, double x) { base[(f * kRSpt + k) * kWave] = x; }
};

template <bool UNROLLED, class F>
__device__ __forceinline__ void for_samples(int nk, F &&f) {
  if constexpr (UNROLLED) {
#pragma unroll
    for (int k = 0; k < kRSpt; ++k)
      if (k < nk) f(k);
  } else {
#pragma unroll 2
    for (int k = 0; k < nk; ++k) f(k);
  }
}

template <int NS, bool MAX = true>
__device__ __forceinline__ void worker_reduce(const double *acc, double mx, double *buf, double *out, long long *st_, long long &last_) {
  const int lane = threadIdx.x & (kWave - 1);
  const int wave = threadIdx.x >> 6;
  double v[NS + 1];
#pragma unroll
  for (int k = 0; k < NS; ++k) {
    double t = acc[k];
    t = t + dpp_move<0x111, 0xf, 0xf>(t, 0.0);
    t = t + dpp_move<0x112, 0xf, 0xf>(t, 0.0);
    v[k] = t;
  }
  if constexpr (MAX) {
    double t = mx;
    t = fmax(t, dpp_move<0x111, 0xf, 0xf>(t, 0.0));
    t = fmax(t, dpp_move<0x112, 0xf, 0xf>(t, 0.0));
    v[NS] = t;
  }
  constexpr int NV = NS + (MAX ? 1 : 0);
  if ((threadIdx.x & 3) == 3) {
#pragma unroll
    for (int k = 0; k < NV; ++k) buf[k * kRedCols + (threadIdx.x >> 2)] = v[k];
  }
  __syncthreads();
  RSTAMP(6);
  {
    constexpr int NW = kRThreads / kWave;
    const int k0 = wave, k1 = wave + NW;
    const bool has0 = k0 < NV, has1 = k1 < NV;
    double s0 = 0.0, s1 = 0.0;
    if (has0) {
      const double *src = buf + k0 * kRedCols;
      s0 = (k0 < NS || !MAX) ? src[lane] + src[lane + kWave] : fmax(src[lane], src[lane + kWave]);
    }
    if (has1) {
      const double *src = buf + k1 * kRedCols;
      s1 = (k1 < NS || !MAX) ? src[lane] + src[lane + kWave] : fmax(src[lane], src[lane + kWave]);
    }
    const bool max0 = MAX && has0 && k0 == NS, max1 = MAX && has1 && k1 == NS;
    if (!max0 && !max1) {
      wave_reduce2_to_last<OpSum, OpSum>(s0, s1);
    } else if (max1) {
      wave_reduce2_to_last<OpSum, OpMax>(s0, s1);
    } else {
      wave_reduce2_to_last<OpMax, OpSum>(s0, s1);
    }
    if (lane == kWave - 1) {
      if (has0) out[max0 ? kSums : k0] = s0;
      if (has1) out[max1 ? kSums : k1] = s1;
    }
  }
  __syncthreads();
}

constexpr int kGroup = 16;
constexpr int kMaxGroups = 16;
constexpr int kReplicas = 8;
constexpr size_t kBlockGranules = (size_t)kRowWords * kGroup;
constexpr size_t kRowsGranules = 2 * (size_t)kMaxGroups * kBlockGranules;
constexpr size_t kGroupsGranules = 2 * (size_t)kReplicas * kBlockGranules;

typedef unsigned int u32x4 __attribute__((ext_vector_type(4)));
constexpr int kCacheSc1 = 16;
__device__ __forceinline__ __amdgpu_buffer_rsrc_t table_rsrc(const u64 *p, size_t granules) {
  return __builtin_amdgcn_make_buffer_rsrc(const_cast<u64 *>(p), 0, (int)(granules * sizeof(u64)), 0x00027000);
}
__device__ __forceinline__ void put_cell(__amdgpu_buffer_rsrc_t t, unsigned cell, unsigned tag, double v) {
  const u32x4 d = {(unsigned)__double2loint(v), tag, (unsigned)__double2hiint(v), tag};
  __builtin_amdgcn_raw_buffer_store_b128(d, t, (int)(cell * 16u), 0, kCacheSc1);
}

template <int NS, bool MAX = true>
__device__ __forceinline__ constexpr bool slot_used(int v) { return v < NS || (MAX && v == kSums); }

template <int NS, bool MAX = true, class Ctx>
__device__ __forceinline__ bool gather_block(const Ctx &ctx, __amdgpu_buffer_rsrc_t t, unsigned first, unsigned tag, int ncols,
                                             double (&val)[4], unsigned *polls) {
  const int lane = threadIdx.x & (kWave - 1);
  const int col = lane & 15, r = lane >> 4;
  const long long t0 = (long long)wall_clock64();
  for (unsigned spins = 0;; ++spins) {
    u32x4 d[4];
    bool ready = true;
#pragma unroll
    for (int j = 0; j < 4; ++j) {
      d[j] = u32x4{0u, tag, 0u, tag};
      if ((4 * j < NS) || (MAX && 4 * j <= kSums && kSums < 4 * j + 4)) {
        const int v = 4 * j + r;
        if (slot_used<NS, MAX>(v) && col < ncols) d[j] = __builtin_amdgcn_raw_buffer_load_b128(t, (int)((first + v * kGroup + col) * 16u), 0, kCacheSc1);
      }
    }
#pragma unroll
    for (int j = 0; j < 4; ++j) ready = ready && d[j].y == tag && d[j].w == tag;
    if (__all(ready)) {
#pragma unroll
      for (int j = 0; j < 4; ++j) val[j] = __hiloint2double((int)d[j].z, (int)d[j].x);
      *polls = spins;
      return true;
    }
    if ((spins & 63u) == 63u) {
      if (__hip_atomic_load(&ctx.ctl->abort, __ATOMIC_RELAXED, __HIP_MEMORY_SCOPE_AGENT) == ctx.launch_id ||
          (long long)wall_clock64() - t0 > ctx.spin_ticks) {
        __hip_atomic_store(&ctx.ctl->abort, ctx.launch_id, __ATOMIC_RELAXED, __HIP_MEMORY_SCOPE_AGENT);
        return false;
      }
    }
    __builtin_amdgcn_s_sleep(1);
  }
}

template <int NS, bool MAX>
__device__ __forceinline__ void fold_block(double (&val)[4]) {
  const int r = (int)(threadIdx.x & (kWave - 1)) >> 4;
  double mx = 0.0;
  if constexpr (MAX) mx = row_reduce_to_last<OpMax>(val[kSums / 4]);
#pragma unroll
  for (int j = 0; j < 4; ++j)
    if ((4 * j < NS) || (MAX && j == kSums / 4)) val[j] = row_reduce_to_last<OpSum>(val[j]);
  if (MAX && r == (kSums & 3)) val[kSums / 4] = mx;
}

template <int NS, bool MAX = true, class Ctx>
__device__ __forceinline__ bool control_exchange(const Ctx &ctx, unsigned epoch, double *sums, int *s_abort,
                                                 long long *st_, long long &last_) {
  const int lane = threadIdx.x & (kWave - 1);
  const int col = lane & 15, r = lane >> 4;
  const int G = gridDim.x;
  const int grp = blockIdx.x / kGroup, ngrp = (G + kGroup - 1) / kGroup;
  const int members = min(kGroup, G - grp * kGroup);
  const int leader = grp * kGroup + (grp & 7) % members;
  const unsigned tag = ctx.tag_base + epoch + 1u;
  constexpr unsigned kBlockCells = kSlots * kGroup;
  const __amdgpu_buffer_rsrc_t rows = table_rsrc(ctx.rows, kRowsGranules), groups = table_rsrc(ctx.groups, kGroupsGranules);
  const unsigned my_rows = ((epoch & 1u) * kMaxGroups + grp) * kBlockCells;
  const unsigned my_groups = (epoch & 1u) * kReplicas * kBlockCells;
  const bool withhold = (int)epoch == ctx.sabotage_epoch && blockIdx.x == gridDim.x - 1;
  if (slot_used<NS, MAX>(lane) && lane <= kSums && !withhold) put_cell(rows, my_rows + lane * kGroup + blockIdx.x % kGroup, tag, sums[lane]);

  double val[4];
  unsigned polls = 0;
  if ((int)blockIdx.x == leader) {
    if (!gather_block<NS, MAX>(ctx, rows, my_rows, tag, members, val, &polls)) {
      *s_abort = 1;
      return false;
    }
#ifndef BRDF_TRACE_WORKERS
    RTRACE(ctx, epoch, 6, polls + 1);
#endif
    fold_block<NS, MAX>(val);
#pragma unroll
    for (int j = 0; j < 4; ++j) {
      const double t = dpp_move<0x15F, 0xf, 0xf>(val[j], 0.0);
      const int v = 4 * j + r;
      if (slot_used<NS, MAX>(v) && col < ctx.replicas) put_cell(groups, my_groups + col * kBlockCells + v * kGroup + grp, tag, t);
    }
  }
  RSTAMP(2);
  RTRACE(ctx, epoch, 3, wall_clock64());
  if (!gather_block<NS, MAX>(ctx, groups, my_groups + (blockIdx.x % ctx.replicas) * kBlockCells, tag, ngrp, val, &polls)) {
    *s_abort = 1;
    return false;
  }
  fold_block<NS, MAX>(val);
#pragma unroll
  for (int j = 0; j < 4; ++j) {
    const int v = 4 * j + r;
    if (slot_used<NS, MAX>(v) && col == kGroup - 1) sums[v] = val[j];
  }
  __builtin_amdgcn_fence(__ATOMIC_RELEASE, "wavefront");
  __builtin_amdgcn_wave_barrier();
  RSTAMP(3);
  RTRACE(ctx, epoch, 4, wall_clock64());
#ifndef BRDF_TRACE_WORKERS
  RTRACE(ctx, epoch, 7, polls);
#endif
  return true;
}

template <int MODEL>
__device__ __forceinline__ void build_uniforms_wave(PassUniforms<MODEL> &u, const Request<kM> &r, bool need_base, bool analytic_jac) {
  using Mdl = BrdfModel<MODEL>;
  const int lane = (int)(threadIdx.x & (kWave - 1));
  if (r.kind == RQ_EVAL_MULTI) {
    u.ncand = r.nk;
    u.analytic = analytic_jac ? 1 : 0;
    if (lane < kMaxCand && lane < r.nk) {
      const double pk[kM] = {r.pk[lane][0], r.pk[lane][1], r.pk[lane][2]};
      u.lk[lane] = Mdl::lin(pk);
      u.nk[lane] = Mdl::nl(pk);
    }
    return;
  }
  if ((r.kind == RQ_JAC && !analytic_jac) || r.kind == RQ_DIF_JAC) {
    u.ncand = 0;
    u.analytic = 0;
    u.central = r.central;
    u.scal = r.scal;
    u.dp_l2 = r.dp_l2;
#pragma unroll
    for (int j = 0; j < kM; ++j) u.dp[j] = r.dp[j];
    if (lane < 1 + 2 * kM) {
      const int j = lane == 0 ? 0 : (lane - 1) % kM;
      const bool plus = lane >= 1 && lane <= kM, minus = lane > kM;
      double pp[kM];
#pragma unroll
      for (int i = 0; i < kM; ++i) {
        pp[i] = r.p[i];
        if (i == j && plus) pp[i] = r.p[i] + r.d[i];
        if (i == j && minus) pp[i] = r.p[i] - r.d[i];
      }
      const Lin l = Mdl::lin(pp);
      const Nl nn = Mdl::nl(pp);
      if (lane == 0) {
        u.l0 = l;
        u.n0 = nn;
      } else if (plus) {
        u.lp[j] = l;
        if (j == kM - 1) u.np2 = nn;
        double dj = r.d[0];
#pragma unroll
        for (int i = 1; i < kM; ++i)
          if (i == j) dj = r.d[i];
        u.dinv[j] = (r.central ? 0.5 : 1.0) / dj;
      } else {
        u.lm[j] = l;
        if (j == kM - 1) u.nm2 = nn;
      }
    }
    return;
  }
  u.build(r, need_base, analytic_jac);
}

template <int MODEL, int METHOD, bool FAST, class Store>
__device__ __forceinline__ void sweep_pass(int kind, const PassUniforms<MODEL> &u, Store &st, double *jl, int tid, int nk, int nfull, unsigned okm,
                                           bool pend, const double *dpp, double *acc, double &mx) {
  constexpr bool U = Store::kUnrolled;
  constexpr bool W2 = BrdfModel<MODEL>::prep_planes == 2;
  auto prep = [&](int k) { return Prep{st.get(kFq1, k), W2 ? st.get(kFq2, k) : 0.0}; };
  auto dead = [&](int k) { return k >= nfull && !(okm >> k & 1u); };
  switch (kind) {
  case RQ_EVAL:
    if constexpr (METHOD != 0) {
      const EvalUniforms eu{scalar_copy(u.l0), scalar_copy(u.n0), 1.0};
      for_samples<U>(nk, [&](int k) {
        const double f = model_value<MODEL, FAST>(eu, st.get(kFc0, k), prep(k));
        double e = st.get(kFx, k) - f;
        if (dead(k)) e = 0.0;
        acc[0] = fma(e, e, acc[0]);
        mx = fmax(mx, fabs(e));
      });
    }
    break;
  case RQ_SCALED:
    if constexpr (METHOD != 0) {
      const EvalUniforms eu{scalar_copy(u.l0), scalar_copy(u.n0), scalar_copy(u.scal)};
      for_samples<U>(nk, [&](int k) {
        const double f = model_value<MODEL, FAST>(eu, st.get(kFc0, k), prep(k));
        double t = (st.get(kFx, k) - f) / eu.scal;
        if (dead(k)) t = 0.0;
        acc[0] = fma(t, t, acc[0]);
      });
    }
    break;
  case RQ_EVAL_MULTI:
    if constexpr (METHOD != 2) {
      if (u.ncand == kMaxCand) {
        if constexpr (METHOD == 0) {
          for_samples<U>(nk, [&](int k) {
            const double c0 = st.get(kFc0, k), x = st.get(kFx, k);
            const Prep q = prep(k);
            const bool d = dead(k);
#pragma unroll
            for (int j0 = 0; j0 < kMaxCand; j0 += 4) {
              double e[4];
#pragma unroll
              for (int j = 0; j < 4; ++j) e[j] = x - model_value_k<MODEL, FAST>(u, j0 + j, c0, q);
#pragma unroll
              for (int j = 0; j < 4; ++j) {
                if (d) e[j] = 0.0;
                acc[j0 + j] = fma(e[j], e[j], acc[j0 + j]);
              }
            }
          });
          break;
        }
#pragma unroll
        for (int j0 = 0; j0 < kMaxCand; j0 += 4) {
          Lin l4[4];
          Nl n4[4];
#pragma unroll
          for (int j = 0; j < 4; ++j) {
            l4[j] = scalar_copy(u.lk[j0 + j]);
            n4[j] = scalar_copy(u.nk[j0 + j]);
          }
          for_samples<U>(nk, [&](int k) {
            const double c0 = st.get(kFc0, k), x = st.get(kFx, k);
            const Prep q = prep(k);
            const bool d = dead(k);
            double e[4];
#pragma unroll
            for (int j = 0; j < 4; ++j) e[j] = x - BrdfModel<MODEL>::combine(l4[j], c0, BrdfModel<MODEL>::template shape<FAST>(n4[j], c0, q));
#pragma unroll
            for (int j = 0; j < 4; ++j) {
              if (d) e[j] = 0.0;
              acc[j0 + j] = fma(e[j], e[j], acc[j0 + j]);
            }
          });
        }
        break;
      }
      for_samples<U>(nk, [&](int k) {
        const double c0 = st.get(kFc0, k), x = st.get(kFx, k);
        const Prep q = prep(k);
#pragma unroll
        for (int j = 0; j < kMaxCand; ++j)
          if (j < u.ncand) {
            double e = x - model_value_k<MODEL, FAST>(u, j, c0, q);
            if (dead(k)) e = 0.0;
            acc[j] = fma(e, e, acc[j]);
          }
      });
    }
    break;
  case RQ_JAC:
    if constexpr (METHOD != 0) {
      auto jac = [&](auto jk) {
        constexpr int JK = decltype(jk)::value;
        JacUniforms ju;
        ju.l0 = scalar_copy(u.l0);
        ju.n0 = scalar_copy(u.n0);
        ju.analytic = JK == 2;
        ju.central = JK == 1;
        if (JK == 2) {
          ju.an[0] = scalar_copy(u.an[0]);
          ju.an[1] = scalar_copy(u.an[1]);
        } else {
#pragma unroll
          for (int j = 0; j < kM; ++j) {
            ju.lp[j] = scalar_copy(u.lp[j]);
            ju.dinv[j] = scalar_copy(u.dinv[j]);
            if (JK == 1) ju.lm[j] = scalar_copy(u.lm[j]);
          }
          ju.np2 = scalar_copy(u.np2);
          if (JK == 1) ju.nm2 = scalar_copy(u.nm2);
        }
        for_samples<U>(nk, [&](int k) {
          double f0 = 0.0, j[kM];
          if (JK == 2)
            model_an_row<MODEL, FAST>(ju, st.get(kFc0, k), prep(k), f0, j);
          else if (JK == 1)
            model_fd_row_t<MODEL, FAST, true>(ju, st.get(kFc0, k), prep(k), true, f0, 0.0, false, j);
          else
            model_fd_row_t<MODEL, FAST, false>(ju, st.get(kFc0, k), prep(k), true, f0, 0.0, false, j);
          double e = st.get(kFx, k) - f0;
          if (dead(k)) e = j[0] = j[1] = j[2] = 0.0;
          acc_normal_eq_fma(j, e, acc, acc + kNL);
          acc[kNL + kM] = fma(e, e, acc[kNL + kM]);
        });
      };
      if (u.analytic)
        jac(std::integral_constant<int, 2>{});
      else if (u.central)
        jac(std::integral_constant<int, 1>{});
      else
        jac(std::integral_constant<int, 0>{});
    }
    break;
  case RQ_DIF_INIT:
    if constexpr (METHOD == 0) {
      for_samples<U>(nk, [&](int k) {
        const double h = model_value<MODEL, FAST>(u, st.get(kFc0, k), prep(k));
        st.set(kFhx, k, h);
        double e = st.get(kFx, k) - h;
        if (dead(k)) e = 0.0;
        acc[0] = fma(e, e, acc[0]);
      });
    }
    break;
  case RQ_DIF_JAC:
    if constexpr (METHOD == 0) {
      for_samples<U>(nk, [&](int k) {
        const int s = k * kRThreads + tid;
        const double h = st.get(kFhx, k);
        double f0 = 0.0, j[kM];
        model_fd_row<MODEL, FAST>(u, st.get(kFc0, k), prep(k), false, f0, h, true, j);
        double e = st.get(kFx, k) - h;
        if (dead(k)) e = j[0] = j[1] = j[2] = 0.0;
        jl[s] = j[0];
        jl[kRCap + s] = j[1];
        jl[2 * kRCap + s] = j[2];
        acc_normal_eq_fma(j, e, acc, acc + kNL);
      });
    }
    break;
  case RQ_DIF_TRIAL:
    if constexpr (METHOD == 0) {
      struct TrialUniforms {
        Lin lq;
        Nl nq;
        double dp[kM], dp_l2;
      };
      TrialUniforms tu;
      tu.lq = scalar_copy(u.lq);
      tu.nq = scalar_copy(u.nq);
#pragma unroll
      for (int j = 0; j < kM; ++j) tu.dp[j] = scalar_copy(u.dp[j]);
      tu.dp_l2 = scalar_copy(u.dp_l2);
      const double dpp_s[kM] = {scalar_copy(dpp[0]), scalar_copy(dpp[1]), scalar_copy(dpp[2])};
      const TrialUniforms &u = tu;
      const double *dpp = dpp_s;
      const double rinv = 1.0 / u.dp_l2;
      auto value_q = [&](int k) { return model_value_q<MODEL, FAST>(u, st.get(kFc0, k), prep(k)); };
      auto body = [&](int k, const double w) {
        const int s = k * kRThreads + tid;
        const double h = st.get(kFhx, k), x = st.get(kFx, k);
        double jo[kM] = {jl[s], jl[kRCap + s], jl[2 * kRCap + s]};
        if (pend) {
          const double tp = st.get(kFtb, k);
#pragma unroll
          for (int j = 0; j < kM; ++j) jo[j] = fma(tp, dpp[j], jo[j]);
          jl[s] = jo[0];
          jl[kRCap + s] = jo[1];
          jl[2 * kRCap + s] = jo[2];
        }
        double t = jo[0] * u.dp[0], jn[kM];
        t = fma(jo[1], u.dp[1], t);
        t = fma(jo[2], u.dp[2], t);
        t = div_by(w - h - t, u.dp_l2, rinv);
#pragma unroll
        for (int j = 0; j < kM; ++j) jn[j] = fma(t, u.dp[j], jo[j]);
        double en = x - w, eo = x - h;
        if (dead(k)) en = eo = jn[0] = jn[1] = jn[2] = t = 0.0;
        st.set(kFwrk, k, w);
        st.set(kFtb, k, t);
        acc[0] = fma(en, en, acc[0]);
#pragma unroll
        for (int j = 0; j < kM; ++j) acc[1 + j] = fma(jo[j], t, acc[1 + j]);
        acc[1 + kM] = fma(t, t, acc[1 + kM]);
#pragma unroll
        for (int j = 0; j < kM; ++j) acc[2 + kM + j] = fma(jn[j], en, acc[2 + kM + j]);
        acc[2 + 2 * kM] = fma(t, eo, acc[2 + 2 * kM]);
      };
      for_samples<U>(nk, [&](int k) { body(k, value_q(k)); });
    }
    break;
  default: break;
  }
}

template <int METHOD>
__device__ __forceinline__ void reduce_pass(int kind, const double *acc, double mx, double *red, double *sums, long long *st_, long long &last_) {
  if constexpr (METHOD == 0) {
    switch (kind) {
    case RQ_DIF_JAC: worker_reduce<SumLayout<kM>::DIF_JAC, false>(acc, mx, red, sums, st_, last_); break;
    case RQ_DIF_TRIAL: worker_reduce<kTrialSums, false>(acc, mx, red, sums, st_, last_); break;
    case RQ_EVAL_MULTI: worker_reduce<kMaxCand, false>(acc, mx, red, sums, st_, last_); break;
    default: worker_reduce<1, false>(acc, mx, red, sums, st_, last_); break;
    }
  } else {
    switch (kind) {
    case RQ_JAC: worker_reduce<SumLayout<kM>::JAC, false>(acc, mx, red, sums, st_, last_); break;
    case RQ_EVAL_MULTI: worker_reduce<kMaxCand, false>(acc, mx, red, sums, st_, last_); break;
    default: worker_reduce<1, METHOD == 1>(acc, mx, red, sums, st_, last_); break;
    }
  }
}

template <int MODEL, int METHOD, bool FAST, bool BATCHED>
__global__ __launch_bounds__(kRThreads) void resident_fit_kernel(ResidentCtx ctx, BatchCtx bctx) {
  using Machine = RMachine<METHOD>;
  using Mdl = BrdfModel<MODEL>;
  constexpr int NF = sample_fields<METHOD>();
  constexpr bool kControlFromLds = (METHOD == 0) || (METHOD == 1 && !BATCHED);
  static_assert(sizeof(Machine) % 4 == 0, "machine copied as dwords");
  __shared__ Machine sm;
  __shared__ PassUniforms<MODEL> su;
  __shared__ double red[kSlots * kRedCols];
  __shared__ double sums[kSlots];
  __shared__ double dp_prev[kM + 1];
  __shared__ int s_abort, s_bad;
  __shared__ double cst[kControlFromLds ? NF * kRSpt * kWave : 2];
  constexpr int kJl = (METHOD == 0) ? 3 * kRCap : 2;
  __shared__ double jl[kJl];

  const int tid = threadIdx.x;
  const int wave = __builtin_amdgcn_readfirstlane((int)threadIdx.x >> 6);
  const int G = BATCHED ? 1 : (int)gridDim.x;
  const int n = BATCHED ? bctx.n : ctx.n;
  const int fit = blockIdx.x;
  if constexpr (BATCHED && !FAST) {
    if (bctx.flags[fit] != kNeedsExact) return;
  }

  if (wave == 0) {
    double p0[kM], opts[5], lb[kM], ub[kM], dscl[kM];
    int itmax, has_opts, has_lb, has_ub, has_dscl = 0, want_covar = 0, multi, analytic, chain, spec_jac;
    if constexpr (BATCHED) {
#pragma unroll
      for (int i = 0; i < kM; ++i) {
        p0[i] = bctx.p[(size_t)fit * kM + i];
        lb[i] = bctx.lb[i];
        ub[i] = bctx.ub[i];
        dscl[i] = 1.0;
      }
#pragma unroll
      for (int i = 0; i < 5; ++i) opts[i] = bctx.opts[i];
      itmax = bctx.itmax, has_opts = bctx.has_opts, has_lb = bctx.has_lb, has_ub = bctx.has_ub, multi = bctx.multi, analytic = bctx.analytic;
      chain = bctx.chain, spec_jac = bctx.spec_jac;
    } else {
#pragma unroll
      for (int i = 0; i < kM; ++i) {
        p0[i] = ctx.p0[i];
        lb[i] = ctx.lb[i];
        ub[i] = ctx.ub[i];
        dscl[i] = ctx.dscl[i];
      }
#pragma unroll
      for (int i = 0; i < 5; ++i) opts[i] = ctx.opts[i];
      itmax = ctx.itmax, has_opts = ctx.has_opts, has_lb = ctx.has_lb, has_ub = ctx.has_ub, has_dscl = ctx.has_dscl;
      want_covar = ctx.want_covar, multi = ctx.multi, analytic = ctx.analytic, chain = ctx.chain, spec_jac = ctx.spec_jac;
    }
    const double *po = has_opts ? opts : nullptr;
    if constexpr (METHOD == 0) {
      sm.start(p0, n, itmax, po, want_covar, 1, chain);
    } else if constexpr (METHOD == 1) {
      sm.start(p0, n, has_lb ? lb : nullptr, has_ub ? ub : nullptr, has_dscl ? dscl : nullptr, itmax, po, want_covar, multi, BATCHED ? 0 : spec_jac);
      sm.c.analytic_jac = analytic;
    } else {
      sm.start(p0, n, itmax, po, want_covar);
    }
    (void)analytic, (void)chain, (void)spec_jac;
  }
  if (tid == 0) s_abort = s_bad = 0;
  if (tid <= kM) dp_prev[tid] = 0.0;
  __syncthreads();
  if (wave == 0) {
    if constexpr (METHOD == 1)
      su.build(sm.h.req, true, sm.c.analytic_jac != 0);
    else
      su.build(sm.h.req, true, METHOD == 2);
  }

  int vb = BATCHED ? 0 : (int)blockIdx.x;
  if (!BATCHED && (G & 7) == 0) vb = (blockIdx.x & 7) * (G >> 3) + (blockIdx.x >> 3);
  const int tile = (n + G - 1) / G;
  const int begin = vb * tile;
  const int end = min(n, begin + tile);
  const double *pc0 = BATCHED ? bctx.angles + (size_t)fit * 3 * n : ctx.c0;
  const double *pc1 = BATCHED ? pc0 + n : ctx.c1;
  const double *pc2 = BATCHED ? pc0 + 2 * (size_t)n : ctx.c2;
  const double *px = BATCHED ? bctx.x + (size_t)fit * n : ctx.x;
  const int nk = (tile + kRThreads - 1) / kRThreads;
  const int nfull = max(end - begin, 0) / kRThreads;
  RegSamples<METHOD> rs;
  LdsSamples<METHOD> ls{cst + (tid & (kWave - 1))};
  unsigned okm = 0;
  {
    bool bad = false;
#pragma unroll
    for (int k = 0; k < kRSpt; ++k) {
      const int i = begin + tid + k * kRThreads;
      const bool ok = i < end;
      okm |= ok ? (1u << k) : 0u;
      const int ii = ok ? i : begin;
      const double r0 = pc0[ii];
      const double r1 = Mdl::uses_c1 ? pc1[ii] : 0.0;
      const double r2 = Mdl::uses_c2 ? pc2[ii] : 0.0;
      const Prep q = Mdl::template prepare<FAST>(r0, r1, r2);
      rs.v[kFc0][k] = r0;
      rs.v[kFx][k] = px[ii];
      rs.v[kFq1][k] = q.q1;
      rs.v[kFq2][k] = q.q2;
      if constexpr (METHOD == 0) rs.v[kFhx][k] = rs.v[kFwrk][k] = rs.v[kFtb][k] = 0.0;
      if (FAST && ok && !Mdl::domain_ok(r0, r1, r2)) bad = true;
    }
    if constexpr (BATCHED) {
      if (FAST && bad) s_bad = 1;
    } else {
      if (FAST && bad) __hip_atomic_store(&ctx.ctl->domain_bad, ctx.launch_id, __ATOMIC_RELAXED, __HIP_MEMORY_SCOPE_AGENT);
    }
    if (kControlFromLds && wave == 0) {
#pragma unroll
      for (int f = 0; f < NF; ++f)
#pragma unroll
        for (int k = 0; k < kRSpt; ++k) ls.set(f, k, rs.v[f][k]);
    }
  }
  __syncthreads();

  int cur_sel_hx = 0, cur_sel_j = 0;
  auto decisions = [&](auto &st, bool &pend) {
    pend = false;
    if constexpr (METHOD == 0) {
      pend = sm.h.req.sel_j != cur_sel_j;
      if (pend && sm.h.req.kind != RQ_DIF_TRIAL) pend = false;
      cur_sel_j = sm.h.req.sel_j;
      if (sm.h.req.sel_hx != cur_sel_hx) {
        for_samples<std::remove_reference<decltype(st)>::type::kUnrolled>(nk, [&](int k) { st.set(kFhx, k, st.get(kFwrk, k)); });
        cur_sel_hx = sm.h.req.sel_hx;
      }
    }
  };

  if (wave == 0) {
    long long st_[8] = {0, 0, 0, 0, 0, 0, 0, 0};
    long long last_ = clock64();
    long long n_jac = 0;
    typename Machine::Cold cold0;
    typename std::conditional<METHOD == 0, typename DifMachine<kM>::CoreInts, int>::type ints_regs{};
    if constexpr (METHOD == 0) {
      cold0.itmax = lm_uniform(sm.c.itmax);
      cold0.n = lm_uniform(sm.c.n);
      cold0.want_covar = lm_uniform(sm.c.want_covar);
      cold0.refresh = lm_uniform(sm.c.refresh);
      cold0.speculative = lm_uniform(sm.c.speculative);
      cold0.multi = lm_uniform(sm.c.multi);
      cold0.o.forward = lm_uniform(sm.c.o.forward);
      cold0.o.tau = scalar_copy(sm.c.o.tau);
      cold0.o.eps1 = scalar_copy(sm.c.o.eps1);
      cold0.o.eps2 = scalar_copy(sm.c.o.eps2);
      cold0.o.eps2sq = scalar_copy(sm.c.o.eps2sq);
      cold0.o.eps3 = scalar_copy(sm.c.o.eps3);
      cold0.o.delta = scalar_copy(sm.c.o.delta);
      ints_regs = sm.h;
      Machine::uniform_ints(ints_regs);
    }
    (void)cold0, (void)ints_regs;
    const long long t_first = (long long)wall_clock64();
    unsigned epoch = 0;
    for (;; ++epoch) {
      const int kind = sm.h.req.kind;
      if (kind == RQ_DONE) break;
      if (kind == RQ_JAC || kind == RQ_DIF_JAC) ++n_jac;
      RTRACE(ctx, epoch, 0, wall_clock64());
      {
        bool pend;
        double acc[kSums];
#pragma unroll
        for (int k = 0; k < kSums; ++k) acc[k] = 0.0;
        double mx = 0.0;
        const double dpp[kM] = {dp_prev[0], dp_prev[1], dp_prev[2]};
        if constexpr (kControlFromLds) {
          decisions(ls, pend);
          sweep_pass<MODEL, METHOD, FAST>(kind, su, ls, jl, tid, nk, nfull, okm, pend, dpp, acc, mx);
        } else {
          decisions(rs, pend);
          sweep_pass<MODEL, METHOD, FAST>(kind, su, rs, jl, tid, nk, nfull, okm, pend, dpp, acc, mx);
        }
        RSTAMP(5);
        RTRACE(ctx, epoch, 1, wall_clock64());
        reduce_pass<METHOD>(kind, acc, mx, red, sums, st_, last_);
      }
      RSTAMP(1);
      RTRACE(ctx, epoch, 2, wall_clock64());
      bool alive = true;
      if constexpr (BATCHED && FAST) {
        if (epoch == 0) {
          if (s_bad) {
            if (tid == 0) bctx.flags[fit] = kNeedsExact;
            s_abort = 1;
            alive = false;
          } else if (tid == 0) {
            bctx.flags[fit] = 0;
          }
        }
      }
      if constexpr (!BATCHED) {
       if (gridDim.x > 1) {
        if constexpr (METHOD == 0) {
          switch (kind) {
          case RQ_DIF_JAC: alive = control_exchange<SumLayout<kM>::DIF_JAC, false>(ctx, epoch, sums, &s_abort, st_, last_); break;
          case RQ_DIF_TRIAL: alive = control_exchange<kTrialSums, false>(ctx, epoch, sums, &s_abort, st_, last_); break;
          case RQ_EVAL_MULTI: alive = control_exchange<kMaxCand, false>(ctx, epoch, sums, &s_abort, st_, last_); break;
          default: alive = control_exchange<1, false>(ctx, epoch, sums, &s_abort, st_, last_); break;
          }
        } else {
          switch (kind) {
          case RQ_JAC: alive = control_exchange<SumLayout<kM>::JAC, false>(ctx, epoch, sums, &s_abort, st_, last_); break;
          case RQ_EVAL_MULTI: alive = control_exchange<kMaxCand, false>(ctx, epoch, sums, &s_abort, st_, last_); break;
          default: alive = control_exchange<1, METHOD == 1>(ctx, epoch, sums, &s_abort, st_, last_); break;
          }
        }
       }
      }
      if (!alive) {
        __syncthreads();
        return;
      }
      if (kind == RQ_DIF_TRIAL) {
        if constexpr (METHOD == 0) {
          expand_trial_sums(static_cast<const typename Machine::Core &>(sm.h), sm.h.cool, su.dp, sums);
        }
#pragma unroll
        for (int j = 0; j < kM; ++j) dp_prev[j] = su.dp[j];
        dp_prev[kM] = su.dp_l2;
      }
      {
        if constexpr (METHOD == 0) {
          typename Machine::Cold cc;
          cc.itmax = cold0.itmax, cc.n = cold0.n, cc.want_covar = cold0.want_covar, cc.refresh = cold0.refresh;
          cc.speculative = cold0.speculative, cc.multi = cold0.multi, cc.o = cold0.o;
          for (int i = 0; i < kInfoSz; ++i) cc.info[i] = 0.0;
          for (int i = 0; i < kM * kM; ++i) cc.covar[i] = 0.0;
          cc.ret = kLmError;
          Machine::template run<true, true>(cc, ints_regs, static_cast<typename Machine::CoreReals &>(sm.h), sm.h.cool, sm.h.req, sums, sums[kSums]);
          Machine::uniform_ints(ints_regs);
          if (sm.h.req.kind == RQ_DONE) {
            for (int i = 0; i < kInfoSz; ++i) sm.c.info[i] = cc.info[i];
            for (int i = 0; i < kM * kM; ++i) sm.c.covar[i] = cc.covar[i];
            sm.c.ret = cc.ret;
          }
        } else
        if constexpr (METHOD == 1)
          sm.template step<true, true, false, !BATCHED>(sums, sums[kSums]);
        else
          sm.template step<true>(sums, sums[kSums]);
      }
      RSTAMP(7);
      if (sm.h.req.kind != RQ_DONE) {
        if constexpr (METHOD == 1 && !BATCHED)
          build_uniforms_wave(su, sm.h.req, false, sm.c.analytic_jac != 0);
        else if constexpr (METHOD == 1)
          su.build(sm.h.req, false, sm.c.analytic_jac != 0);
        else
          su.build(sm.h.req, false, METHOD == 2);
      }
      RTRACE(ctx, epoch, 5, wall_clock64());
      __syncthreads();
      RSTAMP(4);
    }
    if constexpr (BATCHED) {
      if (tid == 0) {
        double *po = bctx.p + (size_t)fit * kM;
        for (int i = 0; i < kM; ++i) po[i] = sm.h.p[i];
        if (bctx.info)
          for (int i = 0; i < kInfoSz; ++i) bctx.info[(size_t)fit * kInfoSz + i] = sm.c.info[i];
        if (bctx.ret) bctx.ret[fit] = sm.c.ret;
      }
      return;
    }
    if (blockIdx.x == 0 && tid == 0) {
      Mailbox *mb = ctx.mbox;
      mb->ret = sm.c.ret;
      mb->passes = (int)epoch;
      if constexpr (METHOD == 1)
        mb->infeasible_mask = sm.c.infeasible_mask;
      else
        mb->infeasible_mask = 0;
      mb->domain_bad = __hip_atomic_load(&ctx.ctl->domain_bad, __ATOMIC_RELAXED, __HIP_MEMORY_SCOPE_AGENT) == ctx.launch_id ? 1 : 0;
      mb->n_jac = n_jac;
      mb->n_eval = (long long)epoch - n_jac;
      mb->t_first = t_first;
      mb->t_last = (long long)wall_clock64();
      for (int k = 0; k < 8; ++k) mb->stamps[k] = st_[k];
      for (int i = 0; i < kM; ++i) mb->p[i] = sm.h.p[i];
      for (int i = 0; i < kInfoSz; ++i) mb->info[i] = sm.c.info[i];
      for (int i = 0; i < kM * kM; ++i) mb->covar[i] = sm.c.covar[i];
      __threadfence_system();
      __hip_atomic_store(&mb->done, 1, __ATOMIC_RELEASE, __HIP_MEMORY_SCOPE_SYSTEM);
    }
    return;
  }

  long long wst_[8] = {0, 0, 0, 0, 0, 0, 0, 0}, wlast_ = 0;
#ifdef BRDF_TRACE_WORKERS
  unsigned wepoch = 0;
#endif
  for (;;) {
    const int kind = sm.h.req.kind;
    if (kind == RQ_DONE) break;
    bool pend;
    decisions(rs, pend);
    double acc[kSums];
#pragma unroll
    for (int k = 0; k < kSums; ++k) acc[k] = 0.0;
    double mx = 0.0;
    const double dpp[kM] = {dp_prev[0], dp_prev[1], dp_prev[2]};
    sweep_pass<MODEL, METHOD, FAST>(kind, su, rs, jl, tid, nk, nfull, okm, pend, dpp, acc, mx);
#ifdef BRDF_TRACE_WORKERS
    if constexpr (!BATCHED) {
      if (wave == 4) RTRACE(ctx, wepoch, 6, wall_clock64());
      if (wave == 7) RTRACE(ctx, wepoch, 7, wall_clock64());
      ++wepoch;
    }
#endif
    reduce_pass<METHOD>(kind, acc, mx, red, sums, wst_, wlast_);
    __syncthreads();
    if (s_abort) return;
  }
}

using ResidentKernelFn = void (*)(ResidentCtx, BatchCtx);
constexpr int kFastPath = 0, kExactPath = 1;
struct ResidentKernels {
  ResidentKernelFn single[2], batched[2];
#ifdef BRDF_STAMPS
  void (*take_lm_stamps)(long long *out8);
#endif
};

template <int MODEL, int METHOD, bool FAST, bool BATCHED>
constexpr ResidentKernelFn resident_kernel() {
  if constexpr (FAST || MODEL != MODEL_WARD)
    return resident_fit_kernel<MODEL, METHOD, FAST, BATCHED>;
  else
    return nullptr;
}

#ifdef BRDF_STAMPS
static void take_lm_stamps(long long *out8) {
  const long long zero[8] = {0, 0, 0, 0, 0, 0, 0, 0};
  (void)hipMemcpyFromSymbol(out8, HIP_SYMBOL(g_rlm_stamps), sizeof zero);
  (void)hipMemcpyToSymbol(HIP_SYMBOL(g_rlm_stamps), zero, sizeof zero);
}
#define BRDF_RESIDENT_STAMPS_ENTRY , take_lm_stamps
#else
#define BRDF_RESIDENT_STAMPS_ENTRY
#endif

#define BRDF_RESIDENT_INSTANCE(MODEL_, METHOD_, NAME_)                                                                      \
  ResidentKernels resident_kernels_##NAME_() {                                                                              \
    return {{resident_kernel<MODEL_, METHOD_, true, false>(), resident_kernel<MODEL_, METHOD_, false, false>()},            \
            {resident_kernel<MODEL_, METHOD_, true, true>(), resident_kernel<MODEL_, METHOD_, false, true>()} BRDF_RESIDENT_STAMPS_ENTRY}; \
  }

}
```

brdf_amd/csrc/stream_fit.h:

```cpp
#pragma once

#include "device_common.h"

namespace brdf {

constexpr int kStreamThreads = 512;
constexpr int kStreamMaxBlocks = 512;
constexpr int kStreamGridCap = 256;
constexpr int kStreamWavesPerSimd = 2;

union MachineUnion {
  DifMachine<kM> dif;
  BcMachine<kM> bc;
  DerMachine<kM> der;
  __host__ __device__ MachineUnion() {}
};

struct Mailbox {
  int done;
  int ret;
  int passes;
  int infeasible_mask;
  long long t_first, t_last;
  long long n_jac, n_eval;
  double p[kM];
  double info[kInfoSz];
  double covar[kM * kM];
  int progress;
  int domain_bad;
  long long stamps[8];
};

struct StreamCtx {
  const double *c0, *c1, *c2, *x;
  double *prep[2];
  double *jac[2];
  double *partials;
  Mailbox *mbox;
  int n, nb, method, model;
  int done;
  int domain_bad;
  long long t_first;
  long long n_jac, n_eval;
  long long stamps[8];
#ifdef BRDF_STAMPS
  int dbg[4096 * 4];
#endif
  MachineUnion m[2];
};

struct StreamFitArgs {
  int method, model;
  int analytic = 0;
  const double *d_angles, *d_x;
  int n;
  double *p;
  const double *lb, *ub, *dscl;
  int itmax;
  const double *opts;
  double *info, *covar;
  hipStream_t stream;
};
int stream_fit_run(const StreamFitArgs &a);

struct FitStats {
  long long passes, jac_passes, eval_passes;
  long long launches;
  double device_us;
  double kernel_us;
  long long stamps[8];
};
FitStats stream_fit_last_stats();
bool launch_timing_enabled();
void set_launch_timing(bool on);
struct LaunchTimer {
  hipEvent_t e0 = nullptr, e1 = nullptr;
  int device = -1;
  bool armed = false;
  void drop() {
    if (e0) (void)hipEventDestroy(e0);
    if (e1) (void)hipEventDestroy(e1);
    e0 = e1 = nullptr;
  }
  ~LaunchTimer() { drop(); }
  void before(hipStream_t s) {
    armed = false;
    if (!launch_timing_enabled()) return;
    int dev = -1;
    if (hipGetDevice(&dev) != hipSuccess) return;
    if (dev != device) {
      drop();
      device = dev;
    }
    if (!e0 && (hipEventCreate(&e0) != hipSuccess || hipEventCreate(&e1) != hipSuccess)) {
      drop();
      return;
    }
    armed = hipEventRecord(e0, s) == hipSuccess;
  }
  void after(hipStream_t s) {
    if (armed) armed = hipEventRecord(e1, s) == hipSuccess;
  }
  double elapsed_us() {
    float ms = 0.0f;
    if (!armed || hipEventSynchronize(e1) != hipSuccess || hipEventElapsedTime(&ms, e0, e1) != hipSuccess) return -1.0;
    return 1e3 * (double)ms;
  }
};

bool resident_fit_try(const StreamFitArgs &a, int *ret);
FitStats resident_fit_last_stats();
int resident_fit_last_trace(long long *out, int max_rows);

int channels_fit_run(int method, int model, const double *d_angles, const double *d_x, long long x_stride, int n, int K, double *p,
                     const double *lb, const double *ub, const double *dscl, int itmax, const double *opts, double *info, double *covar,
                     hipStream_t stream);
int channels_last_shared();
FitStats channels_last_stats(int c);

int capture_fit_single_run(int model, const unsigned char *d_images, int L, int H, int W, const int *d_pixel_map,
                           const double *d_vertices, const int *d_faces, const double *d_normals, int nf, const double *leds,
                           const double *view, int rv_mode, const double *p0, const double *lb, const double *ub, int itmax,
                           const double *opts, double *single_brdf, double *info, long long *n_faces_used, hipStream_t stream);
int cosines_run(const double *d_vertices, const int *d_faces, const double *d_normals, const int *d_surfels, long long S,
                const double *leds, int L, const double *view, int rv_mode, double *d_angles, hipStream_t stream);
void led_table(double *out16x3);
int capture_fit_run(int model, const unsigned char *d_images, int L, int H, int W, const int *d_pixel_map,
                    const double *d_vertices, const int *d_faces, const double *d_normals, int nf, const double *leds,
                    const double *view, int rv_mode, const double *p0, const double *lb, const double *ub, int itmax,
                    const double *opts, double *d_brdf_surfaces, double *avg, long long *n_pixels, hipStream_t stream,
                    double *d_surface_covar = nullptr, double *d_surface_stats = nullptr, int *d_surface_rank = nullptr);

bool brdf_fast_path_enabled();
int pg_candidates();
int dif_chain_candidates();
bool bc_spec_jac_enabled();
void set_error(const char *fmt, ...);
const char *get_error();

}
```

brdf_amd/csrc/stream_fit.hip:

```cpp
#include <chrono>
#include <cstdarg>
#include <cstdio>
#include <atomic>
#include <cstdlib>
#include <cstring>
#include <type_traits>

#if defined(BRDF_STAMPS)
#include <hip/hip_runtime.h>
__device__ long long g_lm_stamps[8];
__device__ long long g_lm_last;
#endif
#if defined(BRDF_STAMPS) && defined(__HIP_DEVICE_COMPILE__)
#define LM_STAMP(i) do { if (blockIdx.x == 0) { const long long now_ = clock64(); if ((i) != 0) g_lm_stamps[i] += now_ - g_lm_last; g_lm_last = now_; } } while (0)
#endif
#include "fit_host.h"

namespace brdf {

template <int METHOD>
using MachineOf = typename std::conditional<METHOD == 0, DifMachine<kM>, typename std::conditional<METHOD == 1, BcMachine<kM>, DerMachine<kM>>::type>::type;

template <int METHOD>
__device__ __forceinline__ MachineOf<METHOD> *machine_slot(StreamCtx *ctx, int which) {
// ... 250 lines not shown
    {
      auto rows = [&](auto jk) {
        constexpr int JK = decltype(jk)::value;
#pragma unroll
        for (int k = 0; k < 4; ++k) {
          double f0 = 0.0, j[kM];
          if (JK == 2)
            model_an_row<MODEL, FAST>(u, s0[k], pq[k], f0, j);
          else if (JK == 1)
            model_fd_row_t<MODEL, FAST, true>(u, s0[k], pq[k], true, f0, 0.0, false, j);
          else
            model_fd_row_t<MODEL, FAST, false>(u, s0[k], pq[k], true, f0, 0.0, false, j);
          double e = sx[k] - f0;
          if (!ok[k]) e = j[0] = j[1] = j[2] = 0.0;
          acc_normal_eq(j, e, acc, acc + kNL);
          acc[kNL + kM] += e * e;
        }
      };
      if (u.analytic)
        rows(std::integral_constant<int, 2>{});
      else if (u.central)
        rows(std::integral_constant<int, 1>{});
      else
        rows(std::integral_constant<int, 0>{});
    }
    SWEEP_END
    STAMP();
    block_reduce<SumLayout<kM>::JAC, kStreamThreads>(acc, mx, red, sums);
    break;
  case RQ_DIF_INIT: {
    SWEEP_BEGIN(4)
#pragma unroll
    for (int k = 0; k < 4; ++k) {
      const double f = model_value<MODEL, FAST>(u, s0[k], pq[k]);
      const double e = ok[k] ? sx[k] - f : 0.0;
      acc[0] += e * e;
    }
    SWEEP_END
    STAMP();
    block_reduce<1, kStreamThreads>(acc, mx, red, sums);
    break;
  }
  case RQ_DIF_JAC: {
    double *__restrict__ jb = ctx->jac[sm.h.req.sel_j];
    SWEEP_BEGIN(4)
#pragma unroll
    for (int k = 0; k < 4; ++k) {
      double f0 = 0.0, j[kM];
      model_fd_row<MODEL, FAST>(u, s0[k], pq[k], true, f0, 0.0, false, j);
      double e = sx[k] - f0;
      if (ok[k]) {
        jb[idx[k]] = j[0];
        jb[(size_t)n + idx[k]] = j[1];
        jb[2 * (size_t)n + idx[k]] = j[2];
      } else {
        e = j[0] = j[1] = j[2] = 0.0;
      }
      acc_normal_eq(j, e, acc, acc + kNL);
    }
    SWEEP_END
    STAMP();
    block_reduce<SumLayout<kM>::DIF_JAC, kStreamThreads>(acc, mx, red, sums);
    break;
  }
  case RQ_DIF_TRIAL: {
    const double *__restrict__ jo = ctx->jac[sm.h.req.sel_j];
    double *__restrict__ jn = ctx->jac[sm.h.req.sel_j ^ 1];
    SWEEP_BEGIN(4)
    double h[4], jold[4][kM];
#pragma unroll
    for (int k = 0; k < 4; ++k) {
      jold[k][0] = jo[idx[k]];
      jold[k][1] = jo[(size_t)n + idx[k]];
      jold[k][2] = jo[2 * (size_t)n + idx[k]];
    }
#pragma unroll
    for (int k = 0; k < 4; ++k) {
      const double w = model_value_q<MODEL, FAST>(u, s0[k], pq[k]);
      h[k] = model_value<MODEL, FAST>(u, s0[k], pq[k]);
      double j[kM];
      broyden_row(jold[k], w, h[k], u.dp, u.dp_l2, j);
      double en = sx[k] - w, eo = sx[k] - h[k];
      if (ok[k]) {
        jn[idx[k]] = j[0];
        jn[(size_t)n + idx[k]] = j[1];
        jn[2 * (size_t)n + idx[k]] = j[2];
      } else {
        en = eo = j[0] = j[1] = j[2] = 0.0;
      }
      acc[0] += en * en;
      acc_normal_eq(j, en, acc + 1, acc + 1 + kNL);
      acc[1 + kNL + kM + 0] += j[0] * eo;
      acc[1 + kNL + kM + 1] += j[1] * eo;
      acc[1 + kNL + kM + 2] += j[2] * eo;
    }
    SWEEP_END
    STAMP();
    block_reduce<SumLayout<kM>::DIF_TRIAL, kStreamThreads>(acc, mx, red, sums);
    break;
  }
  default: return;
  }
#undef SWEEP_BEGIN
#undef SWEEP_END

  if (tid < kSlots) outp[tid * kStreamMaxBlocks + blockIdx.x] = sums[tid];
  STAMP();
#ifdef BRDF_STAMPS
  if (blockIdx.x == 0 && tid == 0 && pass > 0 && sti_ == 8)
    for (int k = 0; k < 7; ++k) ctx->stamps[k] += st_[k + 1] - st_[k];
#endif
}

template <int MODEL>
__global__ __launch_bounds__(256) void model_eval_kernel(const double *__restrict__ c0, const double *__restrict__ c1,
                                                         const double *__restrict__ c2, int n, Request<kM> r,
                                                         double *__restrict__ hx) {
  using Mdl = BrdfModel<MODEL>;
  PassUniforms<MODEL> u;
  u.build(r);
  for (int i = blockIdx.x * blockDim.x + threadIdx.x; i < n; i += gridDim.x * blockDim.x)
    hx[i] = model_value<MODEL, false>(u, c0[i], Mdl::template prepare<false>(c0[i], Mdl::uses_c1 ? c1[i] : 0.0, Mdl::uses_c2 ? c2[i] : 0.0));
}

template <int MODEL>
__global__ __launch_bounds__(256) void model_jac_kernel(const double *__restrict__ c0, const double *__restrict__ c1,
                                                        const double *__restrict__ c2, int n, Request<kM> r,
                                                        double *__restrict__ jac) {
  using Mdl = BrdfModel<MODEL>;
  PassUniforms<MODEL> u;
  u.build(r, true, true);
  for (int i = blockIdx.x * blockDim.x + threadIdx.x; i < n; i += gridDim.x * blockDim.x) {
    double f0, j[kM];
    model_an_row<MODEL, false>(u, c0[i], Mdl::template prepare<false>(c0[i], Mdl::uses_c1 ? c1[i] : 0.0, Mdl::uses_c2 ? c2[i] : 0.0), f0, j);
    jac[3 * (size_t)i] = j[0];
    jac[3 * (size_t)i + 1] = j[1];
    jac[3 * (size_t)i + 2] = j[2];
  }
}

static thread_local char g_err[512] = "";
void set_error(const char *fmt, ...) {
  va_list ap;
  va_start(ap, fmt);
  vsnprintf(g_err, sizeof g_err, fmt, ap);
  va_end(ap);
  fprintf(stderr, "libbrdf_hip: %s\n", g_err);
}
const char *get_error() { return g_err; }

namespace {

struct Workspace {
  int device = -1;
  StreamCtx *d_ctx = nullptr;
  StreamCtx *h_ctx = nullptr;
  Mailbox *h_mbox = nullptr;
  Mailbox *d_mbox = nullptr;
  double *d_partials = nullptr;
  double *d_dif = nullptr;
  size_t dif_cap = 0;
  hipStream_t last_stream = nullptr;
  bool used = false;
  FitStats stats{};

  int ensure(int dev) {
    if (device == dev && d_ctx) return 0;
    release();
    device = dev;
    HIP_OK(hipMalloc(&d_ctx, sizeof(StreamCtx)));
    HIP_OK(hipHostMalloc(&h_ctx, sizeof(StreamCtx), hipHostMallocDefault));
    HIP_OK(hipHostMalloc(&h_mbox, sizeof(Mailbox), hipHostMallocMapped | hipHostMallocCoherent));
    HIP_OK(hipHostGetDevicePointer((void **)&d_mbox, h_mbox, 0));
    HIP_OK(hipMalloc(&d_partials, sizeof(double) * 2 * kSlots * kStreamMaxBlocks));
    HIP_OK(hipMemset(d_partials, 0, sizeof(double) * 2 * kSlots * kStreamMaxBlocks));
    return 0;
  }
  int ensure_dif(size_t n) {
    if (dif_cap >= n) return 0;
    if (d_dif) (void)hipFree(d_dif);
    d_dif = nullptr;
    dif_cap = 0;
    HIP_OK(hipMalloc(&d_dif, sizeof(double) * 8 * n));
    dif_cap = n;
    return 0;
  }
  void release() {
    if (d_ctx) (void)hipFree(d_ctx);
    if (h_ctx) (void)hipHostFree(h_ctx);
    if (h_mbox) (void)hipHostFree(h_mbox);
    if (d_partials) (void)hipFree(d_partials);
    if (d_dif) (void)hipFree(d_dif);
    d_ctx = nullptr;
    h_ctx = nullptr;
    h_mbox = nullptr;
    d_mbox = nullptr;
    d_partials = nullptr;
    d_dif = nullptr;
    dif_cap = 0;
  }
  ~Workspace() {
    if (!d_ctx && !d_dif) return;
    int cur = -1;
    (void)hipGetDevice(&cur);
    if (device >= 0 && cur != device) (void)hipSetDevice(device);
    release();
    if (cur >= 0 && device >= 0 && cur != device) (void)hipSetDevice(cur);
  }
};
thread_local Workspace g_ws;

using PassFn = void (*)(StreamCtx *, int);
PassFn pass_kernel(int model, int method, bool fast) {
  static const PassFn table[2][MODEL_COUNT][3] = {
      {{stream_pass<0, 0, false>, stream_pass<0, 1, false>, stream_pass<0, 2, false>},
       {stream_pass<1, 0, false>, stream_pass<1, 1, false>, stream_pass<1, 2, false>},
       {stream_pass<2, 0, false>, stream_pass<2, 1, false>, stream_pass<2, 2, false>}},
      {{stream_pass<0, 0, true>, stream_pass<0, 1, true>, stream_pass<0, 2, true>},
       {stream_pass<1, 0, true>, stream_pass<1, 1, true>, stream_pass<1, 2, true>},
       {stream_pass<2, 0, true>, stream_pass<2, 1, true>, stream_pass<2, 2, true>}},
  };
  return table[fast ? 1 : 0][model][method];
}

int blocks_for(int n) {
  long long nb = ((long long)n + kStreamThreads * 4 - 1) / (kStreamThreads * 4);
  if (nb > kStreamGridCap) nb = kStreamGridCap;
  if (nb >= 8) nb &= ~7LL;
  if (nb < 1) nb = 1;
  return (int)nb;
}

}

static thread_local bool g_last_was_resident = false;
FitStats stream_fit_last_stats() { return g_last_was_resident ? resident_fit_last_stats() : g_ws.stats; }

static int stream_fit_attempt(const StreamFitArgs &a, bool fast, bool *retry_exact) {
  *retry_exact = false;
  Workspace &ws = g_ws;
  StreamCtx &h = *ws.h_ctx;
  HIP_OK(hipStreamSynchronize(a.stream));
  memset(&h, 0, sizeof h);
  h.c0 = a.d_angles;
  h.c1 = a.d_angles + a.n;
  h.c2 = a.d_angles + 2 * (size_t)a.n;
  h.x = a.d_x;
  h.partials = ws.d_partials;
  h.mbox = ws.d_mbox;
  h.n = a.n;
  h.nb = blocks_for(a.n);
  h.method = a.method;
  h.model = a.model;
  if (ws.ensure_dif((size_t)a.n) != 0) return kLmError;
  h.prep[0] = ws.d_dif;
  h.prep[1] = ws.d_dif + (size_t)a.n;
  h.jac[0] = ws.d_dif + 2 * (size_t)a.n;
  h.jac[1] = ws.d_dif + 5 * (size_t)a.n;

  if (start_fit_machine(h.m[0], a.method, a.p, a.n, a.lb, a.ub, a.dscl, a.itmax, a.opts, a.covar != nullptr, a.analytic != 0, fast) != 0)
    return kLmError;

  Mailbox &mb = *ws.h_mbox;
  memset(&mb, 0, sizeof mb);
  HIP_OK(hipMemcpyAsync(ws.d_ctx, &h, sizeof h, hipMemcpyHostToDevice, a.stream));

  const PassFn fn = pass_kernel(a.model, a.method, fast);
  const dim3 grid(h.nb), block(kStreamThreads);
  constexpr int kRunAhead = 6;
  const long long cap = (long long)(a.itmax > 0 ? a.itmax : 1) * 700 + 64;
  volatile int *done = &mb.done;
  volatile int *progress = &mb.progress;
  long long pass = 0;
  const auto t0 = std::chrono::steady_clock::now();
  long long spins = 0;
  while (!*done) {
    if (pass - (long long)*progress < kRunAhead) {
      if (pass >= cap) {
        set_error("pass budget exhausted (%lld launches) without termination", pass);
        (void)hipStreamSynchronize(a.stream);
        return kLmError;
      }
      hipLaunchKernelGGL(fn, grid, block, 0, a.stream, ws.d_ctx, (int)pass);
      ++pass;
      if ((pass & 63) == 0) HIP_OK(hipGetLastError());
    } else if ((++spins & 0xFFFF) == 0) {
      const double sec = std::chrono::duration<double>(std::chrono::steady_clock::now() - t0).count();
      if (sec > 120.0) {
        set_error("device did not finish within 120 s (pass %lld, progress %d)", pass, *progress);
        return kLmError;
      }
      HIP_OK(hipGetLastError());
    }
  }
  __atomic_thread_fence(__ATOMIC_ACQUIRE);
  HIP_OK(hipGetLastError());
  if (fast && mb.domain_bad) {
    *retry_exact = true;
    return 0;
  }

  mailbox_to_caller(mb, a.p, a.info, a.covar, &ws.stats);
  ws.stats.launches = pass;
  ws.stats.kernel_us = -1.0;
#ifdef BRDF_STAMPS
  if (const char *path = getenv("BRDF_HIP_STEP_DUMP")) {
    static StreamCtx tmp;
    (void)hipStreamSynchronize(a.stream);
    (void)hipMemcpy(&tmp, ws.d_ctx, sizeof tmp, hipMemcpyDeviceToHost);
    long long ls[8];
    if (hipMemcpyFromSymbol(ls, HIP_SYMBOL(g_lm_stamps), sizeof ls) == hipSuccess) {
      fprintf(stderr, "lm step sections (cycles, summed over %d passes, cumulative since load): after_trial=%lld top+gradient=%lld lu_solve=%lld rest_of_solve=%lld\n",
              mb.passes, ls[1], ls[2], ls[3], ls[4]);
    }
    if (FILE *f = fopen(path, "a")) {
      for (int i = 1; i < mb.passes && i < 4096; ++i) fprintf(f, "%d %d %d %d\n", a.method, tmp.dbg[i * 4], tmp.dbg[i * 4 + 1], tmp.dbg[i * 4 + 2]);
      fclose(f);
    }
  }
#endif
  return mb.ret;
}

int pg_candidates() {
  const char *e = getenv("BRDF_HIP_PG_MULTI");
  const int k = e ? atoi(e) : kMaxCand;
  return k < 1 ? 1 : (k > kMaxCand ? kMaxCand : k);
}

static std::atomic<int> g_launch_timing{0};
bool launch_timing_enabled() { return g_launch_timing.load(std::memory_order_relaxed) != 0; }
void set_launch_timing(bool on) { g_launch_timing.store(on ? 1 : 0, std::memory_order_relaxed); }

int dif_chain_candidates() {
  const char *e = getenv("BRDF_HIP_DIF_CHAIN");
  const int k = e ? atoi(e) : kMaxCand;
  return k < 1 ? 1 : (k > kMaxCand ? kMaxCand : k);
}

bool bc_spec_jac_enabled() {
  const char *e = getenv("BRDF_HIP_SPEC_JAC");
  return !(e && e[0] == '0');
}

bool brdf_fast_path_enabled() {
  const char *e = getenv("BRDF_HIP_EXACT_POW");
  return !(e && e[0] == '1');
}

int stream_fit_run(const StreamFitArgs &a) {
  if (a.model < 0 || a.model >= MODEL_COUNT) {
    set_error("unknown BRDF model %d (0 Phong, 1 Blinn-Phong, 2 Ward)", a.model);
    return kLmError;
  }
  if (a.method != 0 && a.method != 1 && a.method != 2) {
    set_error("unknown method %d (0 dlevmar_dif, 1 dlevmar_bc_dif / bc_der, 2 dlevmar_der)", a.method);
    return kLmError;
  }
  if (!a.p || !a.d_angles || a.n <= 0) {
    set_error("null parameter vector / sample planes, or n <= 0");
    return kLmError;
  }
  if (!a.d_x) {
    set_error("x == NULL (zero measurement vector) is not supported on the device path");
    return kLmError;
  }
  (void)hipGetLastError();
  int dev = 0;
  HIP_OK(hipGetDevice(&dev));
  Workspace &ws = g_ws;
  if (ws.ensure(dev) != 0) return kLmError;
  if (ws.used && ws.last_stream != a.stream) HIP_OK(hipStreamSynchronize(ws.last_stream));
  ws.last_stream = a.stream;
  ws.used = true;

  double p_keep[kM];
  for (int i = 0; i < kM; ++i) p_keep[i] = a.p[i];
  {
    int pret = 0;
    if (resident_fit_try(a, &pret)) {
      g_last_was_resident = true;
      return pret;
    }
    for (int i = 0; i < kM; ++i) a.p[i] = p_keep[i];
    g_last_was_resident = false;
  }
  bool retry = false;
  int ret = stream_fit_attempt(a, brdf_fast_path_enabled(), &retry);
  if (retry) {
    for (int i = 0; i < kM; ++i) a.p[i] = p_keep[i];
    ret = stream_fit_attempt(a, false, &retry);
  }
  return ret;
}

int model_jac_run(int model, const double *d_angles, int n, const double *p, double *d_jac, hipStream_t stream) {
  if (model < 0 || model >= MODEL_COUNT || !d_angles || !d_jac || !p || n <= 0) {
    set_error("model_jac: bad arguments");
    return kLmError;
  }
  (void)hipGetLastError();
  Request<kM> r;
  memset(&r, 0, sizeof r);
  r.kind = RQ_JAC;
  r.scal = 1.0;
  for (int i = 0; i < kM; ++i) r.p[i] = p[i];
  int blocks = (n + 255) / 256;
  if (blocks > 2048) blocks = 2048;
  const double *c0 = d_angles, *c1 = d_angles + n, *c2 = d_angles + 2 * (size_t)n;
  switch (model) {
  case 0: hipLaunchKernelGGL(model_jac_kernel<0>, dim3(blocks), dim3(256), 0, stream, c0, c1, c2, n, r, d_jac); break;
  case 1: hipLaunchKernelGGL(model_jac_kernel<1>, dim3(blocks), dim3(256), 0, stream, c0, c1, c2, n, r, d_jac); break;
  default: hipLaunchKernelGGL(model_jac_kernel<2>, dim3(blocks), dim3(256), 0, stream, c0, c1, c2, n, r, d_jac); break;
  }
  HIP_OK(hipGetLastError());
  return 0;
}

int model_eval_run(int model, const double *d_angles, int n, const double *p, double *d_hx, hipStream_t stream) {
  if (model < 0 || model >= MODEL_COUNT || !d_angles || !d_hx || !p || n <= 0) {
    set_error("model_eval: bad arguments");
    return kLmError;
  }
  (void)hipGetLastError();
  Request<kM> r;
  memset(&r, 0, sizeof r);
  r.kind = RQ_EVAL;
  r.scal = 1.0;
  for (int i = 0; i < kM; ++i) r.p[i] = p[i];
  int blocks = (n + 255) / 256;
  if (blocks > 2048) blocks = 2048;
  const double *c0 = d_angles, *c1 = d_angles + n, *c2 = d_angles + 2 * (size_t)n;
  switch (model) {
  case 0: hipLaunchKernelGGL(model_eval_kernel<0>, dim3(blocks), dim3(256), 0, stream, c0, c1, c2, n, r, d_hx); break;
  case 1: hipLaunchKernelGGL(model_eval_kernel<1>, dim3(blocks), dim3(256), 0, stream, c0, c1, c2, n, r, d_hx); break;
  default: hipLaunchKernelGGL(model_eval_kernel<2>, dim3(blocks), dim3(256), 0, stream, c0, c1, c2, n, r, d_hx); break;
  }
  HIP_OK(hipGetLastError());
  return 0;
}

}
```

brdf_amd/fit.py:

```python
from __future__ import annotations

import ctypes as C
from dataclasses import dataclass

import numpy as np

from ._lib import D, ExtraData, last_error, lib

MODEL_PHONG, MODEL_BLINN_PHONG, MODEL_WARD = 0, 1, 2
METHOD_DIF, METHOD_BC_DIF, METHOD_BC_DER, METHOD_DER = 0, 1, 2, 3


@dataclass
class FitResult:
    ret: int
    p: np.ndarray
    info: np.ndarray
    covar: np.ndarray | None = None


def _require(cond: bool, what: str) -> None:
    if not cond:
        raise ValueError(what)

# ... 66 lines not shown
    lba, uba, dsa = _f64(lb, 3), _f64(ub, 3), _f64(dscl, 3)
    oa = _f64(opts, 5) if opts is not None else None
    with torch.cuda.device(angles.device):
        rc = lib.brdf_hip_fit_channels_dev(method, model, angles.data_ptr(), x.data_ptr(), n, n, K, _dptr(p), _dptr(lba), _dptr(uba),
                                           _dptr(dsa), itmax, _dptr(oa), _dptr(info), _dptr(covar), _stream_handle(torch))
    out = []
    for c in range(K):
        failed = info[c, 6] in (4, 7) or (rc != 0 and info[c, 6] == 0)
        out.append(FitResult(-1 if failed else int(info[c, 5]), p[c].copy(), info[c].copy(), None if covar is None else covar[c].reshape(3, 3).copy()))
    return out


def last_channels_stats(channels: int = 3):
    shared = C.c_int(0)
    per = []
    for c in range(channels):
        passes, jac, us = C.c_longlong(0), C.c_longlong(0), C.c_double(0.0)
        lib.brdf_hip_last_channels_stats(c, C.byref(shared), C.byref(passes), C.byref(jac), C.byref(us))
        per.append({"passes": passes.value, "jac_passes": jac.value, "device_us": us.value})
    return {"shared_launch": bool(shared.value), "channels": per, "kernel_us": lib.brdf_hip_last_channels_kernel_us()}


def fit_batch(method: int, model: int, angles, x, p0, *, lb=None, ub=None, itmax=100, opts=None):
    import torch
    _require(angles.is_cuda and x.is_cuda and p0.is_cuda and angles.device == x.device == p0.device, "bad argument: " 'angles.is_cuda and x.is_cuda and p0.is_cuda and angles.device == x.device == p0.device')
    _require(angles.dtype == torch.float64 and x.dtype == torch.float64 and p0.dtype == torch.float64, "bad argument: " 'angles.dtype == torch.float64 and x.dtype == torch.float64 and p0.dtype == torch.float64')
    S, n = x.shape
    _require(tuple(angles.shape) == (S, 3, n) and tuple(p0.shape) == (S, 3), "bad argument: " 'tuple(angles.shape) == (S, 3, n) and tuple(p0.shape) == (S, 3)')
    angles = angles.contiguous()
    x = x.contiguous()
    p = p0.contiguous()
    info = torch.zeros((S, 10), dtype=torch.float64, device=x.device)
    ret = torch.zeros((S,), dtype=torch.int32, device=x.device)
    lb_a, ub_a, op_a = _f64(lb, 3), _f64(ub, 3), _f64(opts, 5)
    with torch.cuda.device(x.device):
        rc = lib.brdf_hip_fit_batch_dev(method, model, angles.data_ptr(), x.data_ptr(), S, n, p.data_ptr(), _dptr(lb_a),
                                        _dptr(ub_a), itmax, _dptr(op_a), info.data_ptr(), ret.data_ptr(),
                                        _stream_handle(torch))
    if rc != 0:
        raise RuntimeError(f"brdf_hip_fit_batch_dev failed: {last_error()}")
    return p, info, ret


@dataclass
class FitStats:
    covar: object
    stats: object
    rank: object


def fit_stats_batch(method: int, model: int, angles, x, p, *, opts=None) -> FitStats:
    op_a = _f64(opts, 5)
    if isinstance(x, np.ndarray):
        angles = np.ascontiguousarray(angles, dtype=np.float64)
        x = np.ascontiguousarray(x, dtype=np.float64)
        p = np.ascontiguousarray(p, dtype=np.float64)
        _require(x.ndim == 2, "x must be [S, n]")
        S, n = x.shape
        _require(angles.shape == (S, 3, n) and p.shape == (S, 3), "angles must be [S, 3, n], p [S, 3]")
        covar, stats, rank = np.zeros((S, 3, 3)), np.zeros((S, 8)), np.zeros(S, dtype=np.int32)
        rc = lib.brdf_hip_fit_stats_batch(method, model, _dptr(angles), _dptr(x), S, n, _dptr(p), _dptr(op_a), _dptr(covar),
                                          _dptr(stats), rank.ctypes.data_as(C.POINTER(C.c_int)))
        if rc != 0:
            raise RuntimeError(f"brdf_hip_fit_stats_batch failed: {last_error()}")
        return FitStats(covar, stats, rank)
    import torch
    _require(angles.is_cuda and x.is_cuda and p.is_cuda and angles.device == x.device == p.device, "angles, x, p: CUDA tensors on one device")
    _require(angles.dtype == torch.float64 and x.dtype == torch.float64 and p.dtype == torch.float64, "angles, x, p: float64")
    _require(x.dim() == 2, "x must be [S, n]")
    S, n = x.shape
    _require(tuple(angles.shape) == (S, 3, n) and tuple(p.shape) == (S, 3), "angles must be [S, 3, n], p [S, 3]")
    angles, x, p = angles.contiguous(), x.contiguous(), p.contiguous()
    covar = torch.zeros((S, 3, 3), dtype=torch.float64, device=x.device)
    stats = torch.zeros((S, 8), dtype=torch.float64, device=x.device)
    rank = torch.zeros((S,), dtype=torch.int32, device=x.device)
    with torch.cuda.device(x.device):
        rc = lib.brdf_hip_fit_stats_batch_dev(method, model, angles.data_ptr(), x.data_ptr(), S, n, p.data_ptr(), _dptr(op_a),
                                              covar.data_ptr(), stats.data_ptr(), rank.data_ptr(), _stream_handle(torch))
    if rc != 0:
        raise RuntimeError(f"brdf_hip_fit_stats_batch_dev failed: {last_error()}")
    return FitStats(covar, stats, rank)


def fit_batch_multi(method: int, model: int, angles, x, p0, *, devices=None, lb=None, ub=None, itmax=100, opts=None):
    angles = np.ascontiguousarray(angles, dtype=np.float64)
    x = np.ascontiguousarray(x, dtype=np.float64)
    _require(x.ndim == 2, "x must be [S, n]")
    S, n = x.shape
    _require(angles.shape == (S, 3, n), "angles must be [S, 3, n]")
    p = np.array(p0, dtype=np.float64, order="C").reshape(-1)
    _require(p.size == 3 * S, "p0 must be [S, 3]")
    p = p.reshape(S, 3)
    info = np.zeros((S, 10))
    ret = np.zeros(S, dtype=np.int32)
    lb_a, ub_a, op_a = _f64(lb, 3), _f64(ub, 3), _f64(opts, 5)
    dev_list, ndev = None, 0
    if devices is not None:
        devices = [int(d) for d in devices]
        dev_list, ndev = (C.c_int * max(1, len(devices)))(*devices), len(devices)
    rc = lib.brdf_hip_fit_batch_multi(method, model, _dptr(angles), _dptr(x), S, n, _dptr(p), _dptr(lb_a), _dptr(ub_a), itmax,
                                      _dptr(op_a), _dptr(info), ret.ctypes.data_as(C.POINTER(C.c_int)), dev_list, ndev)
    if rc < 0:
        raise RuntimeError(f"brdf_hip_fit_batch_multi failed: {last_error()}")
    return p, info, ret


def last_multi_stats() -> list:
    out = []
    dev, first, count, ms = C.c_int(0), C.c_longlong(0), C.c_longlong(0), (C.c_double * 3)()
    while lib.brdf_hip_last_multi_stats(len(out), C.byref(dev), C.byref(first), C.byref(count), ms) == 0:
        out.append({"device": dev.value, "first": first.value, "count": count.value, "upload_ms": ms[0], "fit_ms": ms[1],
                    "download_ms": ms[2]})
    return out


def model_eval(model: int, angles, p):
    import torch
    _require(angles.is_cuda and angles.dtype == torch.float64 and angles.numel() % 3 == 0, "bad argument: " 'angles.is_cuda and angles.dtype == torch.float64 and angles.numel() % 3 == 0')
    angles = angles.contiguous()
    n = angles.numel() // 3
    hx = torch.empty(n, dtype=torch.float64, device=angles.device)
    pa = _f64(p, 3)
    with torch.cuda.device(angles.device):
        rc = lib.brdf_hip_model_eval_dev(model, angles.data_ptr(), n, _dptr(pa), hx.data_ptr(), _stream_handle(torch))
    if rc != 0:
        raise RuntimeError(f"brdf_hip_model_eval_dev failed: {last_error()}")
    return hx


def led_table() -> np.ndarray:
    out = np.zeros(48)
    lib.brdf_hip_led_table(_dptr(out))
    return out.reshape(16, 3)


def _check_indices(idx, upper: int, what: str, lower: int = 0) -> None:
    if idx.numel() == 0:
        return
    lo, hi = int(idx.min()), int(idx.max())
    _require(lo >= lower and hi < upper, f"{what} (range [{lo}, {hi}], allowed [{lower}, {upper}))")


def cosines(vertices, faces, face_normals, leds, view_origin, *, surfels=None, rv_mode: int = 0, validate: bool = True):
    import torch
    vertices, faces, face_normals = vertices.contiguous(), faces.contiguous(), face_normals.contiguous()
    _require(vertices.is_cuda and faces.is_cuda and face_normals.is_cuda, "bad argument: " 'vertices.is_cuda and faces.is_cuda and face_normals.is_cuda')
    _require(vertices.dtype == torch.float64 and face_normals.dtype == torch.float64 and faces.dtype == torch.int32, "bad argument: " 'vertices.dtype == torch.float64 and face_normals.dtype == torch.float64 and faces.dtype == torch.int32')
    _require(vertices.shape[-1] == 3 and faces.shape[-1] == 3 and tuple(face_normals.shape) == (faces.shape[0], 3), "bad argument: " 'vertices.shape[-1] == 3 and faces.shape[-1] == 3 and tuple(face_normals.shape) == (faces.shape[0], 3)')
    if validate:
        _check_indices(faces, vertices.shape[0], "face index outside the vertex array")
    if surfels is not None:
        surfels = surfels.contiguous()
        _require(surfels.is_cuda and surfels.dtype == torch.int32, "bad argument: " 'surfels.is_cuda and surfels.dtype == torch.int32')
        if validate:
            _check_indices(surfels, faces.shape[0], "surfel index outside the face array")
    S = int(surfels.numel()) if surfels is not None else int(faces.shape[0])
    la = np.ascontiguousarray(leds, dtype=np.float64).reshape(-1, 3)
    L = la.shape[0]
    va = _f64(view_origin, 3)
    out = torch.empty((S, 3, L), dtype=torch.float64, device=vertices.device)
    with torch.cuda.device(vertices.device):
        rc = lib.brdf_hip_cosines_dev(vertices.data_ptr(), faces.data_ptr(), face_normals.data_ptr(),
                                      surfels.data_ptr() if surfels is not None else None, S, _dptr(la), L, _dptr(va), rv_mode,
                                      out.data_ptr(), _stream_handle(torch))
    if rc != 0:
        raise RuntimeError(f"brdf_hip_cosines_dev failed: {last_error()}")
    return out


def fit_capture(model: int, images, pixel_map, vertices, faces, face_normals, leds, view_origin, *, rv_mode: int = 0,
                p0=(0.5, 1.0, 1.0), lb=(0.0, 0.0, 0.0), ub=(100.0, 100.0, 100.0), itmax: int = 100, opts=None, brdf_surfaces=None,
                validate: bool = True, want_stats: bool = False, surface_stats: FitStats | None = None):
    import torch
    images, pixel_map = images.contiguous(), pixel_map.contiguous()
    vertices, faces, face_normals = vertices.contiguous(), faces.contiguous(), face_normals.contiguous()
    _require(images.is_cuda and pixel_map.is_cuda and vertices.is_cuda and faces.is_cuda and face_normals.is_cuda, "bad argument: " 'images.is_cuda and pixel_map.is_cuda and vertices.is_cuda and faces.is_cuda and face_normals.is_cuda')
    _require(images.dtype == torch.uint8 and pixel_map.dtype == torch.int32 and faces.dtype == torch.int32, "bad argument: " 'images.dtype == torch.uint8 and pixel_map.dtype == torch.int32 and faces.dtype == torch.int32')
    _require(vertices.dtype == torch.float64 and face_normals.dtype == torch.float64, "bad argument: " 'vertices.dtype == torch.float64 and face_normals.dtype == torch.float64')
    _require(images.dim() == 4 and images.shape[3] == 3 and tuple(pixel_map.shape) == tuple(images.shape[1:3]), "bad argument: " 'images.dim() == 4 and images.shape[3] == 3 and tuple(pixel_map.shape) == tuple(images.shape[1:3])')
    _require(tuple(face_normals.shape) == (faces.shape[0], 3) and vertices.shape[-1] == 3, "bad argument: " 'tuple(face_normals.shape) == (faces.shape[0], 3) and vertices.shape[-1] == 3')
    if validate:
        _check_indices(pixel_map, faces.shape[0], "pixel map names a face that does not exist", lower=-1)
        _check_indices(faces, vertices.shape[0], "face index outside the vertex array")
    L, H, W = int(images.shape[0]), int(images.shape[1]), int(images.shape[2])
    nf = int(faces.shape[0])
    if brdf_surfaces is None:
        brdf_surfaces = torch.zeros((nf, 3, 3), dtype=torch.float64, device=images.device)
    la = np.ascontiguousarray(leds, dtype=np.float64).reshape(-1, 3)
    _require(la.shape[0] == L, "bad argument: " 'la.shape[0] == L')
    va, pa, lba, uba = _f64(view_origin, 3), _f64(p0, 3), _f64(lb, 3), _f64(ub, 3)
    oa = _f64(opts, 5) if opts is not None else None
    avg = np.zeros(3)
    npx = C.c_longlong(0)
    args = (model, images.data_ptr(), L, H, W, pixel_map.data_ptr(), vertices.data_ptr(), faces.data_ptr(), face_normals.data_ptr(),
            nf, _dptr(la), _dptr(va), rv_mode, _dptr(pa), _dptr(lba), _dptr(uba), itmax, _dptr(oa) if oa is not None else None,
            brdf_surfaces.data_ptr(), _dptr(avg), C.byref(npx))
    if not want_stats:
        with torch.cuda.device(images.device):
            rc = lib.brdf_hip_fit_capture_dev(*args, _stream_handle(torch))
        if rc != 0:
            raise RuntimeError(f"brdf_hip_fit_capture_dev failed: {last_error()}")
        return brdf_surfaces, avg, npx.value
    st = surface_stats
    if st is None:
        st = FitStats(torch.zeros((nf, 3, 3, 3), dtype=torch.float64, device=images.device),
                      torch.zeros((nf, 3, 8), dtype=torch.float64, device=images.device),
                      torch.zeros((nf, 3), dtype=torch.int32, device=images.device))
    _require(tuple(st.covar.shape) == (nf, 3, 3, 3) and tuple(st.stats.shape) == (nf, 3, 8) and tuple(st.rank.shape) == (nf, 3),
             "surface_stats: covar [nf,3,3,3], stats [nf,3,8], rank [nf,3]")
    _require(st.covar.dtype == torch.float64 and st.stats.dtype == torch.float64 and st.rank.dtype == torch.int32,
             "surface_stats: float64 covar and stats, int32 rank")
    _require(st.covar.is_contiguous() and st.stats.is_contiguous() and st.rank.is_contiguous() and st.covar.is_cuda and st.stats.is_cuda
             and st.rank.is_cuda, "surface_stats: contiguous CUDA tensors")
    with torch.cuda.device(images.device):
        rc = lib.brdf_hip_fit_capture_stats_dev(*args, _stream_handle(torch), st.covar.data_ptr(), st.stats.data_ptr(), st.rank.data_ptr())
    if rc != 0:
        raise RuntimeError(f"brdf_hip_fit_capture_stats_dev failed: {last_error()}")
    return brdf_surfaces, avg, npx.value, st


def fit_capture_single(model: int, images, pixel_map, vertices, faces, face_normals, leds, view_origin, *, rv_mode: int = 0,
                       p0=(0.0, 0.0, 0.0), lb=(0.0, 0.0, 0.0), ub=(100.0, 100.0, 100.0), itmax: int = 2000,
                       opts=(1e-3, 1e-15, 1e-10, 1e-50, 1.0), validate: bool = True):
    import torch
    images, pixel_map = images.contiguous(), pixel_map.contiguous()
    vertices, faces, face_normals = vertices.contiguous(), faces.contiguous(), face_normals.contiguous()
    _require(images.is_cuda and pixel_map.is_cuda and vertices.is_cuda and faces.is_cuda and face_normals.is_cuda, "bad argument: " 'images.is_cuda and pixel_map.is_cuda and vertices.is_cuda and faces.is_cuda and face_normals.is_cuda')
    _require(images.dtype == torch.uint8 and pixel_map.dtype == torch.int32 and faces.dtype == torch.int32, "bad argument: " 'images.dtype == torch.uint8 and pixel_map.dtype == torch.int32 and faces.dtype == torch.int32')
    _require(vertices.dtype == torch.float64 and face_normals.dtype == torch.float64, "bad argument: " 'vertices.dtype == torch.float64 and face_normals.dtype == torch.float64')
    _require(images.dim() == 4 and images.shape[3] == 3 and tuple(pixel_map.shape) == tuple(images.shape[1:3]), "bad argument: " 'images.dim() == 4 and images.shape[3] == 3 and tuple(pixel_map.shape) == tuple(images.shape[1:3])')
    _require(tuple(face_normals.shape) == (faces.shape[0], 3) and vertices.shape[-1] == 3, "bad argument: " 'tuple(face_normals.shape) == (faces.shape[0], 3) and vertices.shape[-1] == 3')
    if validate:
        _check_indices(pixel_map, faces.shape[0], "pixel map names a face that does not exist", lower=-1)
        _check_indices(faces, vertices.shape[0], "face index outside the vertex array")
    L, H, W = int(images.shape[0]), int(images.shape[1]), int(images.shape[2])
    nf = int(faces.shape[0])
    la = np.ascontiguousarray(leds, dtype=np.float64).reshape(-1, 3)
    _require(la.shape[0] == L, "bad argument: " 'la.shape[0] == L')
    va, pa, lba, uba, oa = _f64(view_origin, 3), _f64(p0, 3), _f64(lb, 3), _f64(ub, 3), _f64(opts, 5)
    out, info = np.zeros(9), np.zeros(30)
    nfu = C.c_longlong(0)
    with torch.cuda.device(images.device):
        rc = lib.brdf_hip_fit_capture_single_dev(model, images.data_ptr(), L, H, W, pixel_map.data_ptr(), vertices.data_ptr(),
                                                 faces.data_ptr(), face_normals.data_ptr(), nf, _dptr(la), _dptr(va), rv_mode,
                                                 _dptr(pa), _dptr(lba), _dptr(uba), itmax, _dptr(oa), _dptr(out), _dptr(info),
                                                 C.byref(nfu), _stream_handle(torch))
    if rc != 0:
        raise RuntimeError(f"brdf_hip_fit_capture_single_dev failed: {last_error()}")
    return out.reshape(3, 3), info.reshape(3, 10), nfu.value


def host_dlevmar(method: int, model: int, angles: np.ndarray, x: np.ndarray, p0, *, lb=None, ub=None, dscl=None,
                 itmax=100, opts=None, want_covar=False) -> FitResult:
    angles = np.ascontiguousarray(angles, dtype=np.float64).reshape(-1)
    x = np.ascontiguousarray(x, dtype=np.float64)
    n = x.size
    p = _f64(p0, 3).copy()
    info = np.zeros(10)
    covar = np.zeros(9) if want_covar else None
    ed = ExtraData(_dptr(angles), model)
    func = C.cast(lib.BRDFFunc_hip, C.c_void_p)
    lb_a, ub_a, ds_a, op_a = _f64(lb, 3), _f64(ub, 3), _f64(dscl, 3), _f64(opts, 5)
    if method == METHOD_DIF:
        ret = lib.dlevmar_dif(func, _dptr(p), _dptr(x), 3, n, itmax, _dptr(op_a), _dptr(info), None, _dptr(covar),
                              C.byref(ed))
    elif method == METHOD_DER:
        ret = lib.dlevmar_der(func, C.cast(lib.BRDFJac_hip, C.c_void_p), _dptr(p), _dptr(x), 3, n, itmax, _dptr(op_a), _dptr(info),
                              None, _dptr(covar), C.byref(ed))
    elif method == METHOD_BC_DER:
        ret = lib.dlevmar_bc_der(func, C.cast(lib.BRDFJac_hip, C.c_void_p), _dptr(p), _dptr(x), 3, n, _dptr(lb_a), _dptr(ub_a),
                                 _dptr(ds_a), itmax, _dptr(op_a), _dptr(info), None, _dptr(covar), C.byref(ed))
    else:
        ret = lib.dlevmar_bc_dif(func, _dptr(p), _dptr(x), 3, n, _dptr(lb_a), _dptr(ub_a), _dptr(ds_a), itmax,
                                 _dptr(op_a), _dptr(info), None, _dptr(covar), C.byref(ed))
    return FitResult(ret, p, info, None if covar is None else covar.reshape(3, 3))


def model_jacobian(model: int, angles: np.ndarray, p) -> np.ndarray:
    a = np.ascontiguousarray(angles, dtype=np.float64).reshape(-1)
    n = a.size // 3
    jac = np.zeros(3 * n)
    pa = _f64(p, 3).copy()
    ed = ExtraData(_dptr(a), model)
    lib.BRDFJac_hip(_dptr(pa), _dptr(jac), 3, n, C.byref(ed))
    return jac.reshape(n, 3)


def chkjac(model: int, angles: np.ndarray, p) -> np.ndarray:
    a = np.ascontiguousarray(angles, dtype=np.float64).reshape(-1)
    n = a.size // 3
    err = np.zeros(n)
    pa = _f64(p, 3).copy()
    ed = ExtraData(_dptr(a), model)
    lib.dlevmar_chkjac(C.cast(lib.BRDFFunc_hip, C.c_void_p), C.cast(lib.BRDFJac_hip, C.c_void_p), _dptr(pa), 3, n, C.byref(ed),
                       _dptr(err))
    return err


def last_fit_stats() -> dict:
    a, b, c = C.c_longlong(0), C.c_longlong(0), C.c_longlong(0)
    us = C.c_double(0.0)
    lib.brdf_hip_last_fit_stats(C.byref(a), C.byref(b), C.byref(c), C.byref(us))
    return {"passes": a.value, "jac_passes": b.value, "eval_passes": c.value, "device_us": us.value,
            "launches": lib.brdf_hip_last_fit_launches(), "kernel_us": lib.brdf_hip_last_fit_kernel_us()}


def set_launch_timing(on: bool) -> None:
    lib.brdf_hip_set_launch_timing(1 if on else 0)
```

include/brdf_levmar.h:

```cpp
#ifndef BRDF_LEVMAR_H
#define BRDF_LEVMAR_H

#ifdef __cplusplus
extern "C" {
#endif

#define LM_DIF_WORKSZ(npar, nmeas) (4 * (nmeas) + 4 * (npar) + (nmeas) * (npar) + (npar) * (npar))
#define LM_BC_DIF_WORKSZ(npar, nmeas) (2 * (nmeas) + 4 * (npar) + (nmeas) * (npar) + (npar) * (npar))
#define LM_DER_WORKSZ(npar, nmeas) (2 * (nmeas) + 4 * (npar) + (nmeas) * (npar) + (npar) * (npar))
#define LM_BC_DER_WORKSZ(npar, nmeas) (2 * (nmeas) + 4 * (npar) + (nmeas) * (npar) + (npar) * (npar))
#define LM_VERSION "2.6 (November 2011)"
#define LM_OPTS_SZ 5
#define LM_INFO_SZ 10
#define LM_ERROR (-1)
#define LM_INIT_MU 1E-03
#define LM_STOP_THRESH 1E-17
#define LM_DIFF_DELTA 1E-06

struct brdf_extra_data {
  double *angles;
  int modelInfo;
};

enum { BRDF_MODEL_PHONG = 0, BRDF_MODEL_BLINN_PHONG = 1, BRDF_MODEL_WARD = 2 };
enum { BRDF_METHOD_DIF = 0, BRDF_METHOD_BC_DIF = 1,
       BRDF_METHOD_BC_DER = 2,
       BRDF_METHOD_DER = 3      };


int dlevmar_dif(void (*func)(double *p, double *hx, int m, int n, void *adata), double *p, double *x,
                int m, int n, int itmax, double *opts, double *info, double *work, double *covar,
                void *adata);

int dlevmar_bc_dif(void (*func)(double *p, double *hx, int m, int n, void *adata), double *p, double *x,
                   int m, int n, double *lb, double *ub, double *dscl, int itmax, double *opts,
                   double *info, double *work, double *covar, void *adata);

int dlevmar_der(void (*func)(double *p, double *hx, int m, int n, void *adata),
                void (*jacf)(double *p, double *j, int m, int n, void *adata), double *p, double *x, int m, int n,
                int itmax, double *opts, double *info, double *work, double *covar, void *adata);

int dlevmar_bc_der(void (*func)(double *p, double *hx, int m, int n, void *adata),
                   void (*jacf)(double *p, double *j, int m, int n, void *adata), double *p, double *x, int m, int n,
                   double *lb, double *ub, double *dscl, int itmax, double *opts, double *info, double *work,
                   double *covar, void *adata);

double dlevmar_stddev(double *covar, int m, int i);
double dlevmar_corcoef(double *covar, int m, int i, int j);

double dlevmar_R2(void (*func)(double *p, double *hx, int m, int n, void *adata), double *p, double *x, int m, int n,
                  void *adata);

int dAx_eq_b_LU_noLapack(double *A, double *B, double *x, int m);

int slevmar_der(void (*func)(float *p, float *hx, int m, int n, void *adata), void (*jacf)(float *p, float *j, int m, int n, void *adata),
                float *p, float *x, int m, int n, int itmax, float *opts, float *info, float *work, float *covar, void *adata);
int slevmar_dif(void (*func)(float *p, float *hx, int m, int n, void *adata), float *p, float *x, int m, int n, int itmax, float *opts,
                float *info, float *work, float *covar, void *adata);
int slevmar_bc_der(void (*func)(float *p, float *hx, int m, int n, void *adata), void (*jacf)(float *p, float *j, int m, int n, void *adata),
                   float *p, float *x, int m, int n, float *lb, float *ub, float *dscl, int itmax, float *opts, float *info, float *work,
                   float *covar, void *adata);
int slevmar_bc_dif(void (*func)(float *p, float *hx, int m, int n, void *adata), float *p, float *x, int m, int n, float *lb, float *ub,
                   float *dscl, int itmax, float *opts, float *info, float *work, float *covar, void *adata);
void slevmar_chkjac(void (*func)(float *p, float *hx, int m, int n, void *adata), void (*jacf)(float *p, float *j, int m, int n, void *adata),
                    float *p, int m, int n, void *adata, float *err);
float slevmar_stddev(float *covar, int m, int i);
float slevmar_corcoef(float *covar, int m, int i, int j);
float slevmar_R2(void (*func)(float *p, float *hx, int m, int n, void *adata), float *p, float *x, int m, int n, void *adata);
int sAx_eq_b_LU_noLapack(float *A, float *B, float *x, int m);

int brdf_hip_register_model(void (*func)(double *p, double *hx, int m, int n, void *adata));
int brdf_hip_unregister_model(void (*func)(double *p, double *hx, int m, int n, void *adata));

void BRDFFunc_hip(double *p, double *hx, int m, int n, void *adata);

void BRDFJac_hip(double *p, double *jac, int m, int n, void *adata);

void dlevmar_chkjac(void (*func)(double *p, double *hx, int m, int n, void *adata),
                    void (*jacf)(double *p, double *j, int m, int n, void *adata), double *p, int m, int n, void *adata,
                    double *err);


int brdf_hip_fit_dev(int method, int model, const double *d_angles, const double *d_x, int n, double *p,
                     const double *lb, const double *ub, const double *dscl, int itmax,
                     const double *opts, double *info, double *covar, void *stream);

int brdf_hip_fit_channels_dev(int method, int model, const double *d_angles, const double *d_x, long long x_stride, int n, int channels,
                              double *p, const double *lb, const double *ub, const double *dscl, int itmax, const double *opts,
                              double *info, double *covar, void *stream);
int brdf_hip_last_channels_stats(int channel, int *shared_launch, long long *passes, long long *jac_passes, double *device_us);
int brdf_hip_last_channels_stamps(int channel, long long *out8);

int brdf_hip_fit_batch_dev(int method, int model, const double *d_angles, const double *d_x, int S, int n,
                           double *d_p, const double *lb, const double *ub, int itmax,
                           const double *opts, double *d_info, int *d_ret, void *stream);

int brdf_hip_fit_batch(int method, int model, const double *angles, const double *x, int S, int n,
                       double *p, const double *lb, const double *ub, int itmax, const double *opts,
                       double *info, int *ret);

int brdf_hip_fit_batch_multi(int method, int model, const double *angles, const double *x, int S, int n, double *p,
                             const double *lb, const double *ub, int itmax, const double *opts, double *info, int *ret,
                             const int *devices, int ndev);
int brdf_hip_last_multi_stats(int shard, int *device, long long *first, long long *count, double *ms3);

#define BRDF_STATS_SZ 8
int brdf_hip_fit_stats_batch_dev(int method, int model, const double *d_angles, const double *d_x, int S, int n,
                                 const double *d_p, const double *opts, double *d_covar, double *d_stats, int *d_rank,
                                 void *stream);
int brdf_hip_fit_stats_batch(int method, int model, const double *angles, const double *x, int S, int n, const double *p,
                             const double *opts, double *covar, double *stats, int *rank);

int brdf_hip_model_eval_dev(int model, const double *d_angles, int n, const double *p, double *d_hx,
                            void *stream);

int brdf_hip_synth_dev(int model, unsigned long long seed, long long first, int count, int n,
                       const double *d_truth, double *d_angles, double *d_x, void *stream);

int brdf_hip_cosines_dev(const double *d_vertices, const int *d_faces, const double *d_face_normals, const int *d_surfels,
                         long long S, const double *leds, int L, const double *view_origin, int rv_mode, double *d_angles,
                         void *stream);
void brdf_hip_led_table(double *leds16x3);

int brdf_hip_fit_capture_dev(int model, const unsigned char *d_images, int L, int H, int W, const int *d_pixel_map,
                             const double *d_vertices, const int *d_faces, const double *d_face_normals, int nf,
                             const double *leds, const double *view_origin, int rv_mode, const double *p0, const double *lb,
                             const double *ub, int itmax, const double *opts, double *d_brdf_surfaces, double *avg,
                             long long *n_pixels, void *stream);

int brdf_hip_fit_capture_stats_dev(int model, const unsigned char *d_images, int L, int H, int W, const int *d_pixel_map,
                                   const double *d_vertices, const int *d_faces, const double *d_face_normals, int nf,
                                   const double *leds, const double *view_origin, int rv_mode, const double *p0,
                                   const double *lb, const double *ub, int itmax, const double *opts, double *d_brdf_surfaces,
                                   double *avg, long long *n_pixels, void *stream, double *d_surface_covar,
                                   double *d_surface_stats, int *d_surface_rank);

int brdf_hip_fit_capture_single_dev(int model, const unsigned char *d_images, int L, int H, int W, const int *d_pixel_map,
                                    const double *d_vertices, const int *d_faces, const double *d_face_normals, int nf,
                                    const double *leds, const double *view_origin, int rv_mode, const double *p0,
                                    const double *lb, const double *ub, int itmax, const double *opts, double *single_brdf,
                                    double *info, long long *n_faces_used, void *stream);

int brdf_hip_device_count(void);
const char *brdf_hip_last_error(void);
int brdf_hip_last_fit_stats(long long *passes, long long *jac_passes, long long *eval_passes,
                            double *device_us);

long long brdf_hip_last_fit_launches(void);
void brdf_hip_set_launch_timing(int on);
double brdf_hip_last_fit_kernel_us(void);
double brdf_hip_last_channels_kernel_us(void);

int brdf_hip_last_fit_stamps(long long *out8);
int brdf_hip_last_fit_trace(long long *out, int max_rows);

#ifdef __cplusplus
}
#endif
#endif
```

Baseline: 131.3 billion.

## Fuse trial evaluation with Jacobian refresh to skip a grid exchange

In the resident single-fit dif-LM kernel, when the next trial is due to trigger a Jacobian refresh, the trial residual evaluation and the finite-difference Jacobian pass are requested together. The two sweeps then share a single cross-block control exchange, with the trial error carried in an extra sum slot. The initial evaluation is fused with the first Jacobian the same way. This cuts the number of grid-wide synchronisations per iteration. In exchange the Jacobian is computed speculatively even when the trial is rejected, and the state machine and tag bookkeeping become more complex. The feature is on by default, with an env var to disable it.

```diff
diff --git a/brdf_amd/_lib.py b/brdf_amd/_lib.py
--- a/brdf_amd/_lib.py
+++ b/brdf_amd/_lib.py
@@ -71,6 +71,7 @@
     "brdf_hip_device_count": (C.c_int, []),
     "brdf_hip_last_error": (C.c_char_p, []),
     "brdf_hip_last_fit_launches": (C.c_longlong, []),
+    "brdf_hip_last_fit_exchanges": (C.c_longlong, []),
     "brdf_hip_set_launch_timing": (None, [C.c_int]),
     "brdf_hip_last_fit_kernel_us": (C.c_double, []),
     "brdf_hip_last_channels_kernel_us": (C.c_double, []),
diff --git a/brdf_amd/csrc/capi.hip b/brdf_amd/csrc/capi.hip
--- a/brdf_amd/csrc/capi.hip
+++ b/brdf_amd/csrc/capi.hip
@@ -708,6 +708,7 @@
 }
 
 long long brdf_hip_last_fit_launches(void) { return stream_fit_last_stats().launches; }
+long long brdf_hip_last_fit_exchanges(void) { return stream_fit_last_stats().exchanges; }
 
 void brdf_hip_set_launch_timing(int on) { set_launch_timing(on != 0); }
 double brdf_hip_last_fit_kernel_us(void) { return stream_fit_last_stats().kernel_us; }
diff --git a/brdf_amd/csrc/fit_host.hip b/brdf_amd/csrc/fit_host.hip
--- a/brdf_amd/csrc/fit_host.hip
+++ b/brdf_amd/csrc/fit_host.hip
@@ -52,6 +52,7 @@
   if (covar)
     for (int i = 0; i < kM * kM; ++i) covar[i] = mb.covar[i];
   stats->passes = mb.passes;
+  stats->exchanges = mb.passes;
   stats->jac_passes = mb.n_jac;
   stats->eval_passes = mb.n_eval;
   stats->device_us = (double)(mb.t_last - mb.t_first) / 100.0;
diff --git a/brdf_amd/csrc/lm_machine.h b/brdf_amd/csrc/lm_machine.h
--- a/brdf_amd/csrc/lm_machine.h
+++ b/brdf_amd/csrc/lm_machine.h
@@ -46,7 +46,8 @@
   RQ_DIF_TRIAL = 6,
   RQ_DIF_UPDATE = 7,
   RQ_EVAL_MULTI = 8,
-  RQ_YIELD = 9
+  RQ_YIELD = 9,
+  RQ_DIF_EVAL_JAC = 10
 };
 
 constexpr int kMaxCand = 8;
@@ -275,12 +276,13 @@
 
 template <int M, class Real = double>
 struct DifMachine {
-  enum Phase : int { D_INIT_EVAL = 1, D_ITER_TOP, D_AFTER_JAC, D_GRADIENT, D_SOLVE, D_AFTER_TRIAL, D_AFTER_UPDATE, D_DECIDE, D_REJECT, D_AFTER_MULTI, D_FINISH, D_DONE };
+  enum Phase : int { D_INIT_EVAL = 1, D_ITER_TOP, D_AFTER_JAC, D_GRADIENT, D_SOLVE, D_AFTER_TRIAL, D_AFTER_UPDATE, D_DECIDE, D_REJECT, D_AFTER_MULTI, D_FINISH, D_AFTER_FTRIAL, D_DONE };
   struct Cold {
     FitOptionsT<Real> o;
     int itmax, n, want_covar, refresh;
     int speculative;
     int multi;
+    int fuse_refresh;
     Real info[kInfoSz], covar[M * M];
     int ret;
   };
@@ -324,11 +326,13 @@
   Cold c;
   Hot h;
 
-  LM_HD void start(const Real *p0, int n_, int itmax_, const Real *opts, int want_covar_, int speculative_ = 1, int multi_ = 1) {
+  LM_HD void start(const Real *p0, int n_, int itmax_, const Real *opts, int want_covar_, int speculative_ = 1, int multi_ = 1,
+                   int fuse_refresh_ = 0) {
     Request<M, Real> &req = h.req;
     Cool &cool = h.cool;
     c.o = make_options(opts);
     c.speculative = speculative_;
+    c.fuse_refresh = fuse_refresh_ ? 1 : 0;
     c.multi = (multi_ < 1 || !speculative_) ? 1 : ((multi_ > kMaxCand) ? kMaxCand : multi_);
     h.chain = h.single = h.mcnt = 0;
     for (int j = 0; j < kMaxCand; ++j) cool.ml2[j] = Real(0.0);
@@ -363,7 +367,13 @@
     }
     req.kind = RQ_DIF_INIT;
     for (int i = 0; i < M; ++i) req.p[i] = h.p[i];
+    if (c.fuse_refresh) request_eval_jac(c, req);
     h.phase = D_INIT_EVAL;
+  }
+  static LM_HD void request_eval_jac(const Cold &c, Request<M, Real> &req) {
+    req.kind = RQ_DIF_EVAL_JAC;
+    req.central = !c.o.forward;
+    fd_steps<M>(req.p, c.o.delta, req.d);
   }
 
   static LM_HD void clear_req(const CoreInts &h, Request<M, Real> &req) {
@@ -388,16 +398,17 @@
     }
   }
 
-  template <bool ONE_LANE = false, bool MULTI = false>
-  LM_HD void step(const Real *s, Real maxabs) { run<ONE_LANE, MULTI>(c, h, h.cool, h.req, s, maxabs); }
-
-  template <bool ONE_LANE, bool MULTI = false>
+  template <bool ONE_LANE = false, bool MULTI = false, bool FUSE = false>
+  LM_HD void step(const Real *s, Real maxabs) { run<ONE_LANE, MULTI, FUSE>(c, h, h.cool, h.req, s, maxabs); }
+
+  template <bool ONE_LANE, bool MULTI = false, bool FUSE = false>
   static LM_HD void run(Cold &c, Core &h, Cool &cool, Request<M, Real> &req, const Real *s, Real maxabs) {
-    run<ONE_LANE, MULTI>(c, static_cast<CoreInts &>(h), static_cast<CoreReals &>(h), cool, req, s, maxabs);
-  }
-  template <bool ONE_LANE, bool MULTI = false>
+    run<ONE_LANE, MULTI, FUSE>(c, static_cast<CoreInts &>(h), static_cast<CoreReals &>(h), cool, req, s, maxabs);
+  }
+  template <bool ONE_LANE, bool MULTI = false, bool FUSE = false>
   static LM_HD void run(Cold &c, CoreInts &hi, CoreReals &h, Cool &cool, Request<M, Real> &req, const Real *s, Real ) {
     int ph = ONE_LANE ? lm_uniform(hi.phase) : hi.phase;
+    int fz = 0;
     LM_STAMP(0);
     for (;;) {
       if (ONE_LANE) ph = lm_uniform(ph);
@@ -408,6 +419,10 @@
       LM_PHASE(D_INIT_EVAL) {
         hi.nfev = 1;
         h.p_e2 = s[0];
+        if (FUSE && c.fuse_refresh) {
+          h.p_e2 = s[SumLayout<M>::DIF_JAC];
+          fz = 1;
+        }
         cool.init_e2 = h.p_e2;
         if (!lm_finite(h.p_e2)) hi.stop = 7;
         hi.nu = 20;
@@ -469,6 +484,31 @@
         break;
       } LM_PHASE_END
 
+      if constexpr (FUSE)
+      LM_PHASE(D_AFTER_FTRIAL) {
+        h.pdp_e2 = s[SumLayout<M>::DIF_JAC];
+        if (!lm_finite(h.pdp_e2)) {
+          hi.stop = 7;
+          ph = D_FINISH;
+          break;
+        }
+        const Real dF = h.p_e2 - h.pdp_e2;
+        if (MULTI) hi.chain = 0;
+        Real dL = Real(0.0);
+        for (int i = 0; i < M; ++i) dL += h.dp[i] * (h.mu * h.dp[i] + h.jte[i]);
+        hi.accepted = (dL > Real(0.0) && dF > Real(0.0)) ? 1 : 0;
+        if (hi.accepted) {
+          Real t = (Real(2.0) * dF / dL - Real(1.0));
+          t = Real(1.0) - t * t * t;
+          h.mu = h.mu * ((t >= Real(kOneThird)) ? t : Real(kOneThird));
+        }
+        ++hi.updjac;
+        hi.newjac = 1;
+        fz = hi.accepted ? 1 : 2;
+        ph = D_DECIDE;
+        break;
+      } LM_PHASE_END
+
       LM_PHASE(D_AFTER_UPDATE) {
         unpack_lower<M>(s, cool.spec_jtj);
         for (int i = 0; i < M; ++i) cool.spec_jte[i] = s[SumLayout<M>::NL + i];
@@ -515,7 +555,7 @@
         if (hi.accepted) {
           hi.nu = 2;
           for (int i = 0; i < M; ++i) h.p[i] = cool.pdp[i];
-          if (c.speculative) hi.sel_hx ^= 1;
+          if (c.speculative && !(FUSE && fz == 1)) hi.sel_hx ^= 1;
           h.p_e2 = h.pdp_e2;
           hi.updp = 1;
           ++hi.k;
@@ -552,18 +592,29 @@
           break;
         }
         if ((hi.updp && hi.nu > 16) || hi.updjac == c.refresh) {
+          ++hi.njap;
+          hi.nfev += c.o.forward ? M : 2 * M;
+          hi.nu = 2;
+          hi.updjac = 0;
+          hi.updp = 0;
+          if (MULTI) hi.chain = 0;
+          if (FUSE && fz == 1) {
+            fz = 0;
+            unpack_lower<M>(s, h.jtj);
+            for (int i = 0; i < M; ++i) h.jte[i] = s[SumLayout<M>::NL + i];
+            hi.newjac = 0;
+            gradient_stats(h, cool);
+            ph = D_SOLVE;
+            break;
+          }
           clear_req(hi, req);
           req.kind = RQ_DIF_JAC;
           req.central = !c.o.forward;
           for (int i = 0; i < M; ++i) req.p[i] = h.p[i];
           fd_steps<M>(h.p, c.o.delta, req.d);
-          ++hi.njap;
-          hi.nfev += c.o.forward ? M : 2 * M;
-          hi.nu = 2;
-          hi.updjac = 0;
-          hi.updp = 0;
+          if (FUSE && fz == 2) req.kind = RQ_DIF_EVAL_JAC;
+          fz = 0;
           hi.newjac = 1;
-          if (MULTI) hi.chain = 0;
           ph = D_AFTER_JAC;
           { hi.phase = ph; return; }
         }
@@ -693,6 +744,13 @@
           break;
         }
         clear_req(hi, req);
+        if (FUSE && c.fuse_refresh && hi.updp && hi.updjac + 1 == c.refresh) {
+          for (int i = 0; i < M; ++i) req.p[i] = cool.pdp[i];
+          request_eval_jac(c, req);
+          ++hi.nfev;
+          ph = D_AFTER_FTRIAL;
+          { hi.phase = ph; return; }
+        }
         req.kind = RQ_DIF_TRIAL;
         for (int i = 0; i < M; ++i) {
           req.p[i] = h.p[i];
diff --git a/brdf_amd/csrc/resident_fit.hip b/brdf_amd/csrc/resident_fit.hip
--- a/brdf_amd/csrc/resident_fit.hip
+++ b/brdf_amd/csrc/resident_fit.hip
@@ -81,6 +81,7 @@
   c.want_covar = a.covar != nullptr;
   c.multi = pg_candidates();
   c.chain = dif_chain_candidates();
+  c.fuse = dif_fuse_enabled() ? 1 : 0;
   c.spec_jac = bc_spec_jac_enabled() ? 1 : 0;
   c.analytic = a.analytic ? 1 : 0;
   c.mbox = ws.d_mbox;
@@ -116,7 +117,7 @@
     return 0;
   }
   const Mailbox &mb = *ws.h_mbox;
-  ws.tag_base += (unsigned)mb.passes + 2u;
+  ws.tag_base += (unsigned)mb.exchanges + 2u;
 #ifdef BRDF_STAMPS
   (void)hipMemcpy(ws.h_trace, c.trace, RWorkspace::trace_bytes, hipMemcpyDeviceToHost);
   k.take_lm_stamps(ws.h_trace + 8 * kRowStride);
@@ -127,6 +128,7 @@
   }
   mailbox_to_caller(mb, a.p, a.info, a.covar, &ws.stats);
   ws.stats.launches = 1;
+  ws.stats.exchanges = mb.exchanges;
   ws.stats.kernel_us = ws.timer.elapsed_us();
   return mb.ret;
 }
diff --git a/brdf_amd/csrc/resident_fit_impl.h b/brdf_amd/csrc/resident_fit_impl.h
--- a/brdf_amd/csrc/resident_fit_impl.h
+++ b/brdf_amd/csrc/resident_fit_impl.h
@@ -40,6 +40,7 @@
   double p0[kM], opts[5], lb[kM], ub[kM], dscl[kM];
   int itmax, has_opts, has_lb, has_ub, has_dscl, want_covar, multi, analytic;
   int chain;
+  int fuse;
   int spec_jac;
   Mailbox *mbox;
   int n;
@@ -589,12 +590,14 @@
   using Mdl = BrdfModel<MODEL>;
   constexpr int NF = sample_fields<METHOD>();
   constexpr bool kControlFromLds = (METHOD == 0) || (METHOD == 1 && !BATCHED);
+  constexpr bool kFuse = METHOD == 0 && !BATCHED;
   static_assert(sizeof(Machine) % 4 == 0, "machine copied as dwords");
   __shared__ Machine sm;
   __shared__ PassUniforms<MODEL> su;
   __shared__ double red[kSlots * kRedCols];
   __shared__ double sums[kSlots];
   __shared__ double dp_prev[kM + 1];
+  __shared__ double fuse_e2;
   __shared__ int s_abort, s_bad;
   __shared__ double cst[kControlFromLds ? NF * kRSpt * kWave : 2];
   constexpr int kJl = (METHOD == 0) ? 3 * kRCap : 2;
@@ -611,7 +614,7 @@
 
   if (wave == 0) {
     double p0[kM], opts[5], lb[kM], ub[kM], dscl[kM];
-    int itmax, has_opts, has_lb, has_ub, has_dscl = 0, want_covar = 0, multi, analytic, chain, spec_jac;
+    int itmax, has_opts, has_lb, has_ub, has_dscl = 0, want_covar = 0, multi, analytic, chain, spec_jac, fuse = 0;
     if constexpr (BATCHED) {
 #pragma unroll
       for (int i = 0; i < kM; ++i) {
@@ -636,17 +639,19 @@
       for (int i = 0; i < 5; ++i) opts[i] = ctx.opts[i];
       itmax = ctx.itmax, has_opts = ctx.has_opts, has_lb = ctx.has_lb, has_ub = ctx.has_ub, has_dscl = ctx.has_dscl;
       want_covar = ctx.want_covar, multi = ctx.multi, analytic = ctx.analytic, chain = ctx.chain, spec_jac = ctx.spec_jac;
+      fuse = ctx.fuse;
     }
     const double *po = has_opts ? opts : nullptr;
     if constexpr (METHOD == 0) {
-      sm.start(p0, n, itmax, po, want_covar, 1, chain);
+      sm.start(p0, n, itmax, po, want_covar, 1, chain, kFuse ? fuse : 0);
+      if (kFuse && sm.h.req.kind == RQ_DIF_EVAL_JAC) sm.h.req.kind = RQ_DIF_INIT;
     } else if constexpr (METHOD == 1) {
       sm.start(p0, n, has_lb ? lb : nullptr, has_ub ? ub : nullptr, has_dscl ? dscl : nullptr, itmax, po, want_covar, multi, BATCHED ? 0 : spec_jac);
       sm.c.analytic_jac = analytic;
     } else {
       sm.start(p0, n, itmax, po, want_covar);
     }
-    (void)analytic, (void)chain, (void)spec_jac;
+    (void)analytic, (void)chain, (void)spec_jac, (void)fuse;
   }
   if (tid == 0) s_abort = s_bad = 0;
   if (tid <= kM) dp_prev[tid] = 0.0;
@@ -732,6 +737,7 @@
       cold0.refresh = lm_uniform(sm.c.refresh);
       cold0.speculative = lm_uniform(sm.c.speculative);
       cold0.multi = lm_uniform(sm.c.multi);
+      cold0.fuse_refresh = lm_uniform(sm.c.fuse_refresh);
       cold0.o.forward = lm_uniform(sm.c.o.forward);
       cold0.o.tau = scalar_copy(sm.c.o.tau);
       cold0.o.eps1 = scalar_copy(sm.c.o.eps1);
@@ -744,10 +750,14 @@
     }
     (void)cold0, (void)ints_regs;
     const long long t_first = (long long)wall_clock64();
-    unsigned epoch = 0;
-    for (;; ++epoch) {
+    unsigned epoch = 0, sweeps = 0;
+    int fuse_half = 0;
+    if constexpr (kFuse) fuse_half = (cold0.fuse_refresh && sm.h.req.kind == RQ_DIF_INIT) ? 1 : 0;
+    (void)fuse_half;
+    for (;;) {
       const int kind = sm.h.req.kind;
       if (kind == RQ_DONE) break;
+      ++sweeps;
       if (kind == RQ_JAC || kind == RQ_DIF_JAC) ++n_jac;
       RTRACE(ctx, epoch, 0, wall_clock64());
       {
@@ -770,6 +780,18 @@
       }
       RSTAMP(1);
       RTRACE(ctx, epoch, 2, wall_clock64());
+      if constexpr (kFuse) {
+        if (fuse_half == 1) {
+          fuse_e2 = sums[0];
+          sm.h.req.kind = RQ_DIF_JAC;
+          su.build(sm.h.req, false, false);
+          fuse_half = 2;
+          __syncthreads();
+          RSTAMP(4);
+          continue;
+        }
+        if (fuse_half == 2) sums[SumLayout<kM>::DIF_JAC] = fuse_e2;
+      }
       bool alive = true;
       if constexpr (BATCHED && FAST) {
         if (epoch == 0) {
@@ -786,7 +808,12 @@
        if (gridDim.x > 1) {
         if constexpr (METHOD == 0) {
           switch (kind) {
-          case RQ_DIF_JAC: alive = control_exchange<SumLayout<kM>::DIF_JAC, false>(ctx, epoch, sums, &s_abort, st_, last_); break;
+          case RQ_DIF_JAC:
+            if (kFuse && fuse_half == 2)
+              alive = control_exchange<SumLayout<kM>::DIF_JAC + 1, false>(ctx, epoch, sums, &s_abort, st_, last_);
+            else
+              alive = control_exchange<SumLayout<kM>::DIF_JAC, false>(ctx, epoch, sums, &s_abort, st_, last_);
+            break;
           case RQ_DIF_TRIAL: alive = control_exchange<kTrialSums, false>(ctx, epoch, sums, &s_abort, st_, last_); break;
           case RQ_EVAL_MULTI: alive = control_exchange<kMaxCand, false>(ctx, epoch, sums, &s_abort, st_, last_); break;
           default: alive = control_exchange<1, false>(ctx, epoch, sums, &s_abort, st_, last_); break;
@@ -820,8 +847,16 @@
           for (int i = 0; i < kInfoSz; ++i) cc.info[i] = 0.0;
           for (int i = 0; i < kM * kM; ++i) cc.covar[i] = 0.0;
           cc.ret = kLmError;
-          Machine::template run<true, true>(cc, ints_regs, static_cast<typename Machine::CoreReals &>(sm.h), sm.h.cool, sm.h.req, sums, sums[kSums]);
+          cc.fuse_refresh = cold0.fuse_refresh;
+          Machine::template run<true, true, kFuse>(cc, ints_regs, static_cast<typename Machine::CoreReals &>(sm.h), sm.h.cool, sm.h.req, sums, sums[kSums]);
           Machine::uniform_ints(ints_regs);
+          if constexpr (kFuse) {
+            fuse_half = 0;
+            if (sm.h.req.kind == RQ_DIF_EVAL_JAC) {
+              sm.h.req.kind = RQ_DIF_INIT;
+              fuse_half = 1;
+            }
+          }
           if (sm.h.req.kind == RQ_DONE) {
             for (int i = 0; i < kInfoSz; ++i) sm.c.info[i] = cc.info[i];
             for (int i = 0; i < kM * kM; ++i) sm.c.covar[i] = cc.covar[i];
@@ -845,6 +880,7 @@
       RTRACE(ctx, epoch, 5, wall_clock64());
       __syncthreads();
       RSTAMP(4);
+      ++epoch;
     }
     if constexpr (BATCHED) {
       if (tid == 0) {
@@ -859,14 +895,15 @@
     if (blockIdx.x == 0 && tid == 0) {
       Mailbox *mb = ctx.mbox;
       mb->ret = sm.c.ret;
-      mb->passes = (int)epoch;
+      mb->passes = (int)sweeps;
+      mb->exchanges = (int)epoch;
       if constexpr (METHOD == 1)
         mb->infeasible_mask = sm.c.infeasible_mask;
       else
         mb->infeasible_mask = 0;
       mb->domain_bad = __hip_atomic_load(&ctx.ctl->domain_bad, __ATOMIC_RELAXED, __HIP_MEMORY_SCOPE_AGENT) == ctx.launch_id ? 1 : 0;
       mb->n_jac = n_jac;
-      mb->n_eval = (long long)epoch - n_jac;
+      mb->n_eval = (long long)sweeps - n_jac;
       mb->t_first = t_first;
       mb->t_last = (long long)wall_clock64();
       for (int k = 0; k < 8; ++k) mb->stamps[k] = st_[k];
diff --git a/brdf_amd/csrc/stream_fit.h b/brdf_amd/csrc/stream_fit.h
--- a/brdf_amd/csrc/stream_fit.h
+++ b/brdf_amd/csrc/stream_fit.h
@@ -29,6 +29,7 @@
   int progress;
   int domain_bad;
   long long stamps[8];
+  int exchanges;
 };
 
 struct StreamCtx {
@@ -65,6 +66,7 @@
 
 struct FitStats {
   long long passes, jac_passes, eval_passes;
+  long long exchanges;
   long long launches;
   double device_us;
   double kernel_us;
@@ -134,6 +136,7 @@
 bool brdf_fast_path_enabled();
 int pg_candidates();
 int dif_chain_candidates();
+bool dif_fuse_enabled();
 bool bc_spec_jac_enabled();
 void set_error(const char *fmt, ...);
 const char *get_error();
diff --git a/brdf_amd/csrc/stream_fit.hip b/brdf_amd/csrc/stream_fit.hip
--- a/brdf_amd/csrc/stream_fit.hip
+++ b/brdf_amd/csrc/stream_fit.hip
@@ -576,6 +576,7 @@
 
   mailbox_to_caller(mb, a.p, a.info, a.covar, &ws.stats);
   ws.stats.launches = pass;
+  ws.stats.exchanges = ws.stats.passes;
   ws.stats.kernel_us = -1.0;
 #ifdef BRDF_STAMPS
   if (const char *path = getenv("BRDF_HIP_STEP_DUMP")) {
@@ -610,6 +611,11 @@
   const char *e = getenv("BRDF_HIP_DIF_CHAIN");
   const int k = e ? atoi(e) : kMaxCand;
   return k < 1 ? 1 : (k > kMaxCand ? kMaxCand : k);
+}
+
+bool dif_fuse_enabled() {
+  const char *e = getenv("BRDF_HIP_DIF_FUSE");
+  return !(e && e[0] == '0');
 }
 
 bool bc_spec_jac_enabled() {
diff --git a/brdf_amd/fit.py b/brdf_amd/fit.py
--- a/brdf_amd/fit.py
+++ b/brdf_amd/fit.py
@@ -392,7 +392,8 @@
     us = C.c_double(0.0)
     lib.brdf_hip_last_fit_stats(C.byref(a), C.byref(b), C.byref(c), C.byref(us))
     return {"passes": a.value, "jac_passes": b.value, "eval_passes": c.value, "device_us": us.value,
-            "launches": lib.brdf_hip_last_fit_launches(), "kernel_us": lib.brdf_hip_last_fit_kernel_us()}
+            "launches": lib.brdf_hip_last_fit_launches(), "kernel_us": lib.brdf_hip_last_fit_kernel_us(),
+            "exchanges": lib.brdf_hip_last_fit_exchanges()}
 
 
 def set_launch_timing(on: bool) -> None:
diff --git a/include/brdf_levmar.h b/include/brdf_levmar.h
--- a/include/brdf_levmar.h
+++ b/include/brdf_levmar.h
@@ -147,6 +147,7 @@
                             double *device_us);
 
 long long brdf_hip_last_fit_launches(void);
+long long brdf_hip_last_fit_exchanges(void);
 void brdf_hip_set_launch_timing(int on);
 double brdf_hip_last_fit_kernel_us(void);
 double brdf_hip_last_channels_kernel_us(void);
```

Result: slower. 129.3 billion (-1.5%).
